# jcribeiro98/V-GAN

Measured on AMD Instinct MI355X. Metric: V-GAN train steps/sec (batch=1024, d=784), higher is better.
Workload: dtype f32; MMD contractions of `value`: split-bf16 x3 on the bf16 MFMA with fp32 accumulation (centred operand); the same step with the fp32 MFMA is timed in `fp32_mode`; 1 GPU; configs[2]: MNIST-pixels-as-features stand-in, d=784, batch=1024 (VGAN_no_kl step); global_batch=1024, features=784, latent=49, rows_per_gpu=1024, parallelism=dp1 (row-sharded Gram, replicated front), hip_graph=True, generator=collapsed, chain_association=depth, mmd_precision=bf16x3, gram_tile=64

## Files before the change

include/vgan_hip.h:

```cpp
#ifndef VGAN_HIP_H
#define VGAN_HIP_H

#include <stdint.h>

#ifdef __cplusplus
extern "C" {
#endif

#define VGAN_OK 0
#define VGAN_ERR_ARG 1
#define VGAN_ERR_HIP 2

#define VGAN_ABI_VERSION 11

typedef void* vgan_stream_t;

int vgan_abi_version(void);
const char* vgan_last_error(void);

int vgan_linear_forward(const float* x, int ldx, int x_nslabs, int64_t x_slab_stride, const float* W,
                        int ldw, const float* b, float* y, int ldy, int n, int in, int out,
                        vgan_stream_t stream);
int vgan_linear_backward_input(const float* dy, int lddy, const float* W, int ldw,
                               float* dx, int lddx, int n, int in, int out, vgan_stream_t stream);
int vgan_linear_backward_params(const float* dy, int lddy, const float* x, int ldx, int x_nslabs,
                                int64_t x_slab_stride, float* dW, int lddw, float* db, int n, int in,
                                int out, int splits, int64_t slab_stride, vgan_stream_t stream);
struct vgan_xx_job;
int vgan_linear_backward_params_xx_supported(int n, int in, int out);
int vgan_linear_backward_params_xx(const float* dy, int lddy, const float* x, int ldx, float* dW, int lddw, int n, int in,
                                   int out, const struct vgan_xx_job* xx, vgan_stream_t stream);
int64_t vgan_linear_backward_params_ksplit_ws_bytes(int in, int out, int parts);
int vgan_linear_backward_params_ksplit(const float* dy, int lddy, const float* x, int ldx, float* dW, int lddw, int n, int in,
                                       int out, int parts, void* ws, int64_t ws_bytes, vgan_stream_t stream);
enum vgan_linear_forward_path_code {
    VGAN_LINEAR_FORWARD_T64_V4 = 0,
    VGAN_LINEAR_FORWARD_T64_V1 = 1,
    VGAN_LINEAR_FORWARD_T64_V4_SLABS = 2,
    VGAN_LINEAR_FORWARD_T64_V1_SLABS = 3,
    VGAN_LINEAR_FORWARD_KS4_V4 = 4,
    VGAN_LINEAR_FORWARD_KS4_V1 = 5,
    VGAN_LINEAR_FORWARD_KS16_V4 = 6,
    VGAN_LINEAR_FORWARD_PATHS = 7
};
enum vgan_linear_backward_input_path_code {
    VGAN_LINEAR_BACKWARD_INPUT_T64_V4 = 0,
    VGAN_LINEAR_BACKWARD_INPUT_T64_V1 = 1,
    VGAN_LINEAR_BACKWARD_INPUT_KS4_V4 = 2,
    VGAN_LINEAR_BACKWARD_INPUT_KS4_V1 = 3,
    VGAN_LINEAR_BACKWARD_INPUT_PATHS = 4
};
enum vgan_linear_backward_params_path_code {
    VGAN_LINEAR_BACKWARD_PARAMS_T64_V4 = 0,
    VGAN_LINEAR_BACKWARD_PARAMS_T64_V1 = 1,
    VGAN_LINEAR_BACKWARD_PARAMS_T64_V4_SLABS = 2,
    VGAN_LINEAR_BACKWARD_PARAMS_T64_V1_SLABS = 3,
    VGAN_LINEAR_BACKWARD_PARAMS_KS4_V4 = 4,
    VGAN_LINEAR_BACKWARD_PARAMS_KS4_V1 = 5,
    VGAN_LINEAR_BACKWARD_PARAMS_KS16_V4 = 6,
    VGAN_LINEAR_BACKWARD_PARAMS_PATHS = 7
};
int vgan_linear_forward_path(const float* x, int ldx, int x_nslabs, int64_t x_slab_stride, const float* W, int ldw,
                             const float* b, const float* y, int ldy, int n, int in, int out);
int vgan_linear_backward_input_path(const float* dy, int lddy, const float* W, int ldw, const float* dx, int lddx, int n,
                                    int in, int out);
int vgan_linear_backward_params_path(const float* dy, int lddy, const float* x, int ldx, int x_nslabs, int64_t x_slab_stride,
                                     const float* dW, int lddw, const float* db, int n, int in, int out, int splits,
                                     int64_t slab_stride);
int vgan_reduce_slabs(const float* src, int64_t slab_stride, int nslabs, float* dst, int64_t count,
                      vgan_stream_t stream);

typedef struct vgan_logits_chain {
    const float* za;
    const float* At4;
    int32_t ldza, ldat, e0, pad;
} vgan_logits_chain;
int vgan_mask_project_forward(const float* logits, int ldl, const float* data, int ldd,
                              const int32_t* rows, const uint64_t* row_cursor, int row_batches,
                              int row_stride, int row_offset, float* S, float* U, float* Zx, float* Zy,
                              int ldz, float* sqx, float* sqy, int n, int d, const float* center,
                              int norm_split, const vgan_logits_chain* chain, vgan_stream_t stream);
int vgan_col_mean(const float* data, int ldd, int rows, int d, float* out, vgan_stream_t stream);
int vgan_gather_rows(const float* data, int ldd, const int32_t* rows, const uint64_t* row_cursor,
                     int row_batches, int row_stride, int row_offset, float* out, int ldo,
                     float* sq, int n, int d, vgan_stream_t stream);
int vgan_gather_rows_split(const float* data, int ldd, const int32_t* rows, const uint64_t* row_cursor,
                           int row_batches, int row_stride, int row_offset, const float* center, float* out,
                           int ldo, float* sq, int norm_split, uint16_t* Zh, uint16_t* Zl, int kp, int n, int d,
                           vgan_stream_t stream);
int vgan_mask_backward(const float* gU, int ldg, int nslabs, int64_t slab_stride, const float* S,
                       int lds, const uint64_t* colkey, float pen_weight, int row_offset,
                       float* dlogits, int ldo, int n, int d, vgan_stream_t stream);
int vgan_colmax_chunks(int n);
int vgan_colmax(const float* S, int lds, int from_softmax, int row_offset, uint64_t* part,
                uint64_t* colkey, int n, int d, vgan_stream_t stream);
int vgan_colmax_partial(const float* S, int lds, int from_softmax, int row_offset, uint64_t* part,
                        int n, int d, vgan_stream_t stream);
int vgan_mask_from_softmax(const float* S, int lds, float* U, int ldu, int n, int d, vgan_stream_t stream);
int vgan_upper_softmax_forward(const float* logits, int ldl, float* S, float* U, int n, int d,
                               vgan_stream_t stream);

#define VGAN_TILE 64
#define VGAN_TILE_INTS 8
#define VGAN_TF_SLOT_MASK 3
#define VGAN_TF_TWICE 4
#define VGAN_TF_STORE 8
#define VGAN_TF_MIRROR 16
#define VGAN_TF_NEG 32

int vgan_mmd_build_tiles(int n, int grad_mode, int rank, int world, int tile, int32_t* out, int cap);
int vgan_mmd_order_tiles(int32_t* tiles, int count, int tile);

int vgan_mmd_gram(const float* Z, int ldz, const float* sq, int n, int p, const float* bw,
                  const int32_t* tiles, int ntiles, int calibrate,
                  float* Wg, int ldw, int wrow0, float* partial, vgan_stream_t stream);
#define VGAN_RBF_MAX_KERNELS 8
int vgan_mmd_gram_general(const float* Z, int ldz, const float* sq, int n, int p, const float* bw,
                          const int32_t* tiles, int ntiles, const float* multipliers, int n_kernels,
                          float* Wg, int ldw, int wrow0, float* partial, vgan_stream_t stream);
int vgan_mmd_gram_colmax(const float* Z, int ldz, const float* sq, int n, int p, const float* bw,
                         const int32_t* tiles, int ntiles, float* Wg, int ldw, int wrow0, float* partial,
                         const float* S, int lds, int from_softmax, int row_offset, uint64_t* colpart,
                         int nrows, int d, vgan_stream_t stream);
int vgan_mmd_reduce(const float* partial, const int32_t* tiles, int ntiles, double* stats,
                    int zero_first, vgan_stream_t stream);
int vgan_mmd_set_bandwidth(const double* stats, int n, float* bw, vgan_stream_t stream);
int vgan_mmd_loss(const double* stats, const uint64_t* colkey, int n, int d, float weight,
                  float* loss, float* loss_accum, float accum_scale, uint64_t* step_counter,
                  vgan_stream_t stream);
int vgan_mmd_finalize(const float* partial, const int32_t* tiles, int ntiles, const uint64_t* colpart,
                      int chunks, uint64_t* colkey, int n, int d, float weight, double* stats,
                      float* loss, float* loss_accum, float accum_scale, uint64_t* step_counter,
                      vgan_stream_t stream);
typedef struct vgan_finalize_job {
    const float* partial;
    const int32_t* tiles;
    const uint64_t* colpart;
    uint64_t* colkey;
    double* stats;
    float* loss;
    float* loss_accum;
    uint64_t* step_counter;
    int32_t ntiles, chunks, n, d;
    float weight, accum_scale;
    int32_t mode, ntiles_main;
} vgan_finalize_job;
int vgan_mmd_backward(const float* Wg, int ldw, const float* Z, int ldz, int wrow0, int nr,
                      int ncols, int p, const float* mul, int ldmul, const float* mul_shift, float* out,
                      int ldo, int splits, int64_t slab_stride, const vgan_finalize_job* finalize,
                      vgan_stream_t stream);
int vgan_mmd_bf3_prepare(const float* Z, int ldz, int rows, int p, uint16_t* Zh, uint16_t* Zl, int kp,
                         uint16_t* ZTh, uint16_t* ZTl, int kn, vgan_stream_t stream);
int64_t vgan_mmd_gram_bf3_tail_ws_bytes(void);
int vgan_mmd_gram_bf3(const uint16_t* Zh, const uint16_t* Zl, int kp, const float* sq, int n, const float* bw,
                      const int32_t* tiles, int ntiles, int tile, uint16_t* Wh, uint16_t* Wl, int ldw,
                      int wrow0, float* partial, const float* S, int lds, int from_softmax, int row_offset,
                      uint64_t* colpart, int nrows, int d, void* tail_ws, int64_t tail_ws_bytes,
                      float* rs_part, int ldrs, vgan_stream_t stream);
int vgan_mmd_backward_bf3_tile(int nr, int p, int splits, int tile);
int vgan_mmd_backward_bf3(const uint16_t* Wh, const uint16_t* Wl, int ldw, const uint16_t* ZTh,
                          const uint16_t* ZTl, int kn, int kp, const float* Z, int ldz, int wrow0, int nr,
                          int p, const float* mul, int ldmul, const float* mul_shift, float* out, int ldo,
                          int splits, int64_t slab_stride, int tile, const vgan_finalize_job* finalize,
                          vgan_stream_t stream);
int vgan_mmd_backward_bf3_rm(const uint16_t* Wh, const uint16_t* Wl, int ldw, int kn, const uint16_t* Zh,
                             const uint16_t* Zl, int kp, int zrows, const float* Z, int ldz, int wrow0, int nr,
                             int p, const float* mul, int ldmul, const float* mul_shift, float* out, int ldo,
                             int splits, int64_t slab_stride, int tile, const vgan_finalize_job* finalize,
                             const float* rs_part, int ldrs, vgan_stream_t stream);
int vgan_mmd_backward_bf3_rm_xx(const uint16_t* Wh, const uint16_t* Wl, int ldw, int kn, const uint16_t* Zh,
                                const uint16_t* Zl, int kp, int zrows, const float* Z, int ldz, int wrow0, int nr,
                                int p, const float* mul, int ldmul, const float* mul_shift, float* out, int ldo,
                                int splits, int64_t slab_stride, const vgan_finalize_job* finalize,
                                const struct vgan_xx_job* xx, vgan_stream_t stream);
typedef struct vgan_bwd_rebuild {
    const float* data;
    const int32_t* xrow;
    const float* S;
    const float* center;
    int32_t ldd, lds;
} vgan_bwd_rebuild;
int vgan_mmd_backward_bf3_rm_rebuild(const uint16_t* Wh, const uint16_t* Wl, int ldw, int kn, const uint16_t* Zh,
                                     const uint16_t* Zl, int kp, int zrows, int nr, int p,
                                     const vgan_bwd_rebuild* rebuild, float* out, int ldo, int splits,
                                     int64_t slab_stride, const vgan_finalize_job* finalize,
                                     const struct vgan_xx_job* xx, vgan_stream_t stream);
#define VGAN_GEMM_MAX_GROUP 4
// ... 407 lines not shown
```

v-gan_amd/csrc/linear.hip:

```cpp
#include "gemm_core.hpp"
#include "mmd_xx.hpp"

namespace vgan {

constexpr int LBM = 64, LBN = 64, LBK = 32;

template <int VEC, bool XSL>
__global__ __launch_bounds__(kBlock, 2) void linear_fwd_kernel(const float* __restrict__ x, int ldx, const float* __restrict__ W,
                                                              int ldw, const float* __restrict__ b, float* __restrict__ y,
                                                              int ldy, int n, int in, int out, int x_nslabs, long x_slab_stride) {
    using G = GemmTile<LBM, LBN, LBK, KC, KC, VEC, XSL ? 1 : 0>;
    __shared__ __attribute__((aligned(16))) float lds[G::kLdsFloats];
    const int m0 = blockIdx.y * LBM, n0 = blockIdx.x * LBN;
    const int col = n0 + G::sub_col(0);
    const float bias = (b != nullptr) ? b[min(col, out - 1)] : 0.f;
    f32x16 acc[G::WM][G::WN];
    zero_acc(acc);
    G::template run<false>(x, ldx, W, ldw, m0, n0, n, out, in, lds, nullptr, acc, x_nslabs, x_slab_stride);
#pragma unroll
    for (int r = 0; r < 16; ++r) {
        const int row = m0 + G::sub_row(0, r);
        if (row < n && col < out) y[(long)row * ldy + col] = acc[0][0][r] + bias;
    }
}

template <int VEC>
__global__ __launch_bounds__(kBlock, 2) void linear_bwd_input_kernel(const float* __restrict__ dy, int lddy,
                                                                    const float* __restrict__ W, int ldw, float* __restrict__ dx,
                                                                    int lddx, int n, int in, int out) {
    using G = GemmTile<LBM, LBN, LBK, KC, MC, VEC>;
    __shared__ __attribute__((aligned(16))) float lds[G::kLdsFloats];
    const int m0 = blockIdx.y * LBM, n0 = blockIdx.x * LBN;
    f32x16 acc[G::WM][G::WN];
    zero_acc(acc);
    G::template run<false>(dy, lddy, W, ldw, m0, n0, n, in, out, lds, nullptr, acc);
    const int col = n0 + G::sub_col(0);
#pragma unroll
    for (int r = 0; r < 16; ++r) {
        const int row = m0 + G::sub_row(0, r);
        if (row < n && col < in) dx[(long)row * lddx + col] = acc[0][0][r];
    }
}

template <int VEC, bool XSL>
__global__ __launch_bounds__(kBlock, 2) void linear_bwd_params_kernel(const float* __restrict__ dy, int lddy,
                                                                     const float* __restrict__ x, int ldx, float* __restrict__ dW,
                                                                     int lddw, float* __restrict__ db, int n, int in, int out,
                                                                     int kchunk, long slab_stride, int x_nslabs, long x_slab_stride) {
    using G = GemmTile<LBM, LBN, LBK, MC, MC, VEC, XSL ? 2 : 0>;
    __shared__ __attribute__((aligned(16))) float lds[G::kLdsFloats];
    __shared__ float side[LBM];
    const int m0 = blockIdx.y * LBM, n0 = blockIdx.x * LBN;
    const int k0 = blockIdx.z * kchunk;
    const int klen = min(kchunk, n - k0);
    dy += (long)k0 * lddy;
    x += (long)k0 * ldx;
    dW += blockIdx.z * slab_stride;
    if (db != nullptr) db += blockIdx.z * slab_stride;
    n = klen;
    f32x16 acc[G::WM][G::WN];
    zero_acc(acc);
    const bool do_bias = (db != nullptr) && (blockIdx.x == 0);
    if (klen <= 0) {
        if (threadIdx.x < LBM) side[threadIdx.x] = 0.f;
        __syncthreads();
    } else if (do_bias)
        G::template run<true>(dy, lddy, x, ldx, m0, n0, out, in, n, lds, side, acc, x_nslabs, x_slab_stride);
    else
        G::template run<false>(dy, lddy, x, ldx, m0, n0, out, in, n, lds, side, acc, x_nslabs, x_slab_stride);
    const int col = n0 + G::sub_col(0);
#pragma unroll
    for (int r = 0; r < 16; ++r) {
        const int row = m0 + G::sub_row(0, r);
        if (row < out && col < in) dW[(long)row * lddw + col] = acc[0][0][r];
    }
    if (do_bias && threadIdx.x < LBM && m0 + threadIdx.x < out) db[m0 + threadIdx.x] = side[threadIdx.x];
}

constexpr int KSBK = 128;
template <int VEC, int NW>
__global__ __launch_bounds__(64 * NW, NW == 4 ? 2 : 1) void linear_fwd_ks_kernel(const float* __restrict__ x, int ldx,
                                                                               const float* __restrict__ W, int ldw,
                                                                               const float* __restrict__ b, float* __restrict__ y,
                                                                               int ldy, int n, int in, int out) {
    using G = GemmTileKS<KSBK, KC, KC, VEC, NW>;
    __shared__ __attribute__((aligned(16))) float lds[G::kLdsFloats];
    const int m0 = blockIdx.y * 32, n0 = blockIdx.x * 32;
    const int col = n0 + G::col_of();
    const float bias = (b != nullptr) ? b[min(col, out - 1)] : 0.f;
    float o[G::NR];
    G::run(x, ldx, W, ldw, m0, n0, n, out, in, lds, o);
#pragma unroll
    for (int rr = 0; rr < G::NR; ++rr) {
        const int row = m0 + G::row_of(rr);
        if (row < n && col < out) y[(long)row * ldy + col] = o[rr] + bias;
    }
}
template <int VEC>
__global__ __launch_bounds__(kBlock, 2) void linear_bwd_input_ks_kernel(const float* __restrict__ dy, int lddy,
                                                                       const float* __restrict__ W, int ldw, float* __restrict__ dx,
                                                                       int lddx, int n, int in, int out, int in_staged) {
    using G = GemmTileKS<KSBK, KC, MC, VEC>;
    __shared__ __attribute__((aligned(16))) float lds[G::kLdsFloats];
    const int m0 = blockIdx.y * 32, n0 = blockIdx.x * 32;
    float o[G::NR];
    G::run(dy, lddy, W, ldw, m0, n0, n, in_staged, out, lds, o);
    const int col = n0 + G::col_of();
#pragma unroll
    for (int rr = 0; rr < G::NR; ++rr) {
        const int row = m0 + G::row_of(rr);
        if (row < n && col < in) dx[(long)row * lddx + col] = o[rr];
    }
}
template <int VEC, int NW>
__global__ __launch_bounds__(64 * NW, NW == 4 ? 2 : 1) void linear_bwd_params_ks_kernel(const float* __restrict__ dy, int lddy,
                                                                                      const float* __restrict__ x, int ldx,
                                                                                      float* __restrict__ dW, int lddw, int n, int in,
                                                                                      int out) {
    using G = GemmTileKS<KSBK, MC, MC, VEC, NW>;
    __shared__ __attribute__((aligned(16))) float lds[G::kLdsFloats];
    const int m0 = blockIdx.y * 32, n0 = blockIdx.x * 32;
    float o[G::NR];
    G::run(dy, lddy, x, ldx, m0, n0, out, in, n, lds, o);
    const int col = n0 + G::col_of();
#pragma unroll
    for (int rr = 0; rr < G::NR; ++rr) {
        const int row = m0 + G::row_of(rr);
        if (row < out && col < in) dW[(long)row * lddw + col] = o[rr];
    }
}
__global__ __launch_bounds__(1024, 1) void linear_bwd_params_ks_split_kernel(const float* __restrict__ dy, int lddy,
                                                                            const float* __restrict__ x, int ldx, float* __restrict__ dW,
                                                                            int lddw, int n, int in, int out, int kchunk, KSplitWs ws) {
    using G = GemmTileKS<KSBK, MC, MC, 4, 16>;
    __shared__ __attribute__((aligned(16))) float lds[G::kLdsFloats];
    const int m0 = blockIdx.y * 32, n0 = blockIdx.x * 32;
    const int part = blockIdx.z, parts = gridDim.z;
    const int k0 = part * kchunk, klen = min(kchunk, n - k0);
    float o[G::NR];
    if (klen > 0) {
        G::run(dy + (long)k0 * lddy, lddy, x + (long)k0 * ldx, ldx, m0, n0, out, in, klen, lds, o);
    } else {
#pragma unroll
        for (int rr = 0; rr < G::NR; ++rr) o[rr] = 0.f;
    }
    const int tile = blockIdx.y * gridDim.x + blockIdx.x;
    if (!ksplit_finish<G::NR, G::NTH>(o, ws, tile, tile * parts * kKSplitSlabBytes, part, parts, lds)) return;
    const int col = n0 + G::col_of();
#pragma unroll
    for (int rr = 0; rr < G::NR; ++rr) {
        const int row = m0 + G::row_of(rr);
        if (row < out && col < in) dW[(long)row * lddw + col] = o[rr];
    }
}
__global__ __launch_bounds__(1024, 1) void linear_bwd_params_ks_xx_kernel(const float* __restrict__ dy, int lddy, const float* __restrict__ x,
                                                                         int ldx, float* __restrict__ dW, int lddw, int n, int in, int out,
                                                                         int gx, int ptiles, XXJob xx) {
    using G = GemmTileKS<KSBK, MC, MC, 4, 16>;
    constexpr int kBytes = G::kLdsFloats * 4 > GemmBF3<64>::kLdsBytes ? G::kLdsFloats * 4 : GemmBF3<64>::kLdsBytes;
    __shared__ __attribute__((aligned(16))) char raw[kBytes];
    __shared__ float xx_red[4];
    if ((int)blockIdx.x >= ptiles) {
        xx_tile_body(xx, blockIdx.x - ptiles, raw, xx_red);
        return;
    }
    float* lds = reinterpret_cast<float*>(raw);
    const int m0 = (blockIdx.x / gx) * 32, n0 = (blockIdx.x % gx) * 32;
    float o[G::NR];
    G::run(dy, lddy, x, ldx, m0, n0, out, in, n, lds, o);
    const int col = n0 + G::col_of();
#pragma unroll
    for (int rr = 0; rr < G::NR; ++rr) {
        const int row = m0 + G::row_of(rr);
        if (row < out && col < in) dW[(long)row * lddw + col] = o[rr];
    }
}

static inline bool use_ks(int rows, int cols, int k) {
    const long tiles64 = (long)((rows + 63) / 64) * ((cols + 63) / 64);
    return tiles64 <= 32 && k >= 128;
}

static inline bool use_ks_params(int rows, int cols, int k) {
    const long tiles64 = (long)((rows + 63) / 64) * ((cols + 63) / 64);
    return use_ks(rows, cols, k) || (tiles64 <= 512 && k >= 2048);
}

static inline dim3 grid_for(int rows, int cols) { return dim3((cols + LBN - 1) / LBN, (rows + LBM - 1) / LBM, 1); }

}

using namespace vgan;

#define VGAN_PLAN_CHECK(cond)                                                       \
    do {                                                                            \
        if (!(cond)) {                                                              \
            ::vgan::set_error("%s:%d: bad argument: %s", __FILE__, __LINE__, #cond); \
            return -VGAN_ERR_ARG;                                                   \
        }                                                                           \
    } while (0)

static int linear_forward_plan(const float* x, int ldx, int x_nslabs, int64_t x_slab_stride, const float* W, int ldw, const float* y,
                               int ldy, int n, int in, int out) {
    VGAN_PLAN_CHECK(x && W && y && n > 0 && in > 0 && out > 0 && ldx >= in && ldw >= in && ldy >= out && x_nslabs >= 1);
    const bool vec = (in % 4 == 0) && (ldx % 4 == 0) && (ldw % 4 == 0) && aligned16(x) && aligned16(W) && (x_slab_stride % 4 == 0);
    if (x_nslabs == 1 && use_ks(n, out, in))
        return vec && in >= 512 ? VGAN_LINEAR_FORWARD_KS16_V4 : vec ? VGAN_LINEAR_FORWARD_KS4_V4 : VGAN_LINEAR_FORWARD_KS4_V1;
    if (x_nslabs > 1) return vec ? VGAN_LINEAR_FORWARD_T64_V4_SLABS : VGAN_LINEAR_FORWARD_T64_V1_SLABS;
    return vec ? VGAN_LINEAR_FORWARD_T64_V4 : VGAN_LINEAR_FORWARD_T64_V1;
}

extern "C" int vgan_linear_forward_path(const float* x, int ldx, int x_nslabs, int64_t x_slab_stride, const float* W, int ldw,
                                        const float* b, const float* y, int ldy, int n, int in, int out) {
    (void)b;
    return linear_forward_plan(x, ldx, x_nslabs, x_slab_stride, W, ldw, y, ldy, n, in, out);
}

extern "C" int vgan_linear_forward(const float* x, int ldx, int x_nslabs, int64_t x_slab_stride, const float* W, int ldw,
                                   const float* b, float* y, int ldy, int n, int in, int out, vgan_stream_t stream) {
    const int path = linear_forward_plan(x, ldx, x_nslabs, x_slab_stride, W, ldw, y, ldy, n, in, out);
    if (path < 0) return VGAN_ERR_ARG;
    hipStream_t s = (hipStream_t)stream;
    const long xs = (long)x_slab_stride;
    const dim3 g((out + 31) / 32, (n + 31) / 32);
#define VGAN_FWD(V, S) hipLaunchKernelGGL((linear_fwd_kernel<V, S>), grid_for(n, out), dim3(kBlock), 0, s, x, ldx, W, ldw, b, y, ldy, n, in, out, x_nslabs, xs)
#define VGAN_FWD_KS(V, NW) hipLaunchKernelGGL((linear_fwd_ks_kernel<V, NW>), g, dim3(64 * NW), 0, s, x, ldx, W, ldw, b, y, ldy, n, in, out)
    switch (path) {
        case VGAN_LINEAR_FORWARD_KS16_V4: VGAN_FWD_KS(4, 16); break;
        case VGAN_LINEAR_FORWARD_KS4_V4: VGAN_FWD_KS(4, 4); break;
        case VGAN_LINEAR_FORWARD_KS4_V1: VGAN_FWD_KS(1, 4); break;
        case VGAN_LINEAR_FORWARD_T64_V4_SLABS: VGAN_FWD(4, true); break;
        case VGAN_LINEAR_FORWARD_T64_V1_SLABS: VGAN_FWD(1, true); break;
        case VGAN_LINEAR_FORWARD_T64_V4: VGAN_FWD(4, false); break;
        default: VGAN_FWD(1, false); break;
    }
#undef VGAN_FWD
#undef VGAN_FWD_KS
    VGAN_CHECK_LAUNCH();
    return VGAN_OK;
}

static int linear_backward_input_plan(const float* dy, int lddy, const float* W, int ldw, const float* dx, int lddx, int n, int in,
                                      int out) {
    VGAN_PLAN_CHECK(dy && W && dx && n > 0 && in > 0 && out > 0 && lddy >= out && ldw >= in && lddx >= in);
    const bool vec_but_in = (out % 4 == 0) && (lddy % 4 == 0) && (ldw % 4 == 0) && aligned16(dy) && aligned16(W);
    const bool vec = vec_but_in && (in % 4 == 0);
    if (use_ks(n, in, out)) {
        const int in4 = (in + 3) / 4 * 4;
        return vec_but_in && ldw >= in4 ? VGAN_LINEAR_BACKWARD_INPUT_KS4_V4 : VGAN_LINEAR_BACKWARD_INPUT_KS4_V1;
    }
    return vec ? VGAN_LINEAR_BACKWARD_INPUT_T64_V4 : VGAN_LINEAR_BACKWARD_INPUT_T64_V1;
}

extern "C" int vgan_linear_backward_input_path(const float* dy, int lddy, const float* W, int ldw, const float* dx, int lddx, int n,
                                               int in, int out) {
    return linear_backward_input_plan(dy, lddy, W, ldw, dx, lddx, n, in, out);
}

extern "C" int vgan_linear_backward_input(const float* dy, int lddy, const float* W, int ldw, float* dx, int lddx, int n, int in,
                                          int out, vgan_stream_t stream) {
    const int path = linear_backward_input_plan(dy, lddy, W, ldw, dx, lddx, n, in, out);
    if (path < 0) return VGAN_ERR_ARG;
    hipStream_t s = (hipStream_t)stream;
    const dim3 g((in + 31) / 32, (n + 31) / 32);
    const int in4 = (in + 3) / 4 * 4;
    switch (path) {
        case VGAN_LINEAR_BACKWARD_INPUT_KS4_V4:
            hipLaunchKernelGGL(linear_bwd_input_ks_kernel<4>, g, dim3(kBlock), 0, s, dy, lddy, W, ldw, dx, lddx, n, in, out, in4);
            break;
        case VGAN_LINEAR_BACKWARD_INPUT_KS4_V1:
            hipLaunchKernelGGL(linear_bwd_input_ks_kernel<1>, g, dim3(kBlock), 0, s, dy, lddy, W, ldw, dx, lddx, n, in, out, in);
            break;
        case VGAN_LINEAR_BACKWARD_INPUT_T64_V4:
            hipLaunchKernelGGL(linear_bwd_input_kernel<4>, grid_for(n, in), dim3(kBlock), 0, s, dy, lddy, W, ldw, dx, lddx, n, in, out);
            break;
        default:
            hipLaunchKernelGGL(linear_bwd_input_kernel<1>, grid_for(n, in), dim3(kBlock), 0, s, dy, lddy, W, ldw, dx, lddx, n, in, out);
            break;
    }
    VGAN_CHECK_LAUNCH();
    return VGAN_OK;
}

static int linear_backward_params_plan(const float* dy, int lddy, const float* x, int ldx, int x_nslabs, int64_t x_slab_stride,
                                       const float* dW, int lddw, const float* db, int n, int in, int out, int splits,
                                       int64_t slab_stride) {
    VGAN_PLAN_CHECK(dy && x && dW && n > 0 && in > 0 && out > 0 && lddy >= out && ldx >= in && lddw >= in && x_nslabs >= 1);
    VGAN_PLAN_CHECK(splits >= 1 && splits <= 64 && (splits == 1 || slab_stride > 0));
    const bool vec = (out % 4 == 0) && (lddy % 4 == 0) && (in % 4 == 0) && (ldx % 4 == 0) && aligned16(dy) && aligned16(x) &&
                     (x_slab_stride % 4 == 0);
    if (splits == 1 && x_nslabs == 1 && db == nullptr && use_ks_params(out, in, n))
        return vec && n >= 256 ? VGAN_LINEAR_BACKWARD_PARAMS_KS16_V4 : vec ? VGAN_LINEAR_BACKWARD_PARAMS_KS4_V4 : VGAN_LINEAR_BACKWARD_PARAMS_KS4_V1;
    if (x_nslabs > 1) return vec ? VGAN_LINEAR_BACKWARD_PARAMS_T64_V4_SLABS : VGAN_LINEAR_BACKWARD_PARAMS_T64_V1_SLABS;
    return vec ? VGAN_LINEAR_BACKWARD_PARAMS_T64_V4 : VGAN_LINEAR_BACKWARD_PARAMS_T64_V1;
}

extern "C" int vgan_linear_backward_params_path(const float* dy, int lddy, const float* x, int ldx, int x_nslabs, int64_t x_slab_stride,
                                                const float* dW, int lddw, const float* db, int n, int in, int out, int splits,
                                                int64_t slab_stride) {
    return linear_backward_params_plan(dy, lddy, x, ldx, x_nslabs, x_slab_stride, dW, lddw, db, n, in, out, splits, slab_stride);
}

extern "C" int vgan_linear_backward_params(const float* dy, int lddy, const float* x, int ldx, int x_nslabs, int64_t x_slab_stride,
                                           float* dW, int lddw, float* db, int n, int in, int out, int splits, int64_t slab_stride,
                                           vgan_stream_t stream) {
    const int path = linear_backward_params_plan(dy, lddy, x, ldx, x_nslabs, x_slab_stride, dW, lddw, db, n, in, out, splits, slab_stride);
    if (path < 0) return VGAN_ERR_ARG;
    hipStream_t s = (hipStream_t)stream;
    int kchunk = (n + splits - 1) / splits;
    kchunk = (kchunk + 3) / 4 * 4;
    dim3 grid = grid_for(out, in);
    grid.z = splits;
    const long xs = (long)x_slab_stride;
    const dim3 g((in + 31) / 32, (out + 31) / 32);
#define VGAN_BWP(V, S) hipLaunchKernelGGL((linear_bwd_params_kernel<V, S>), grid, dim3(kBlock), 0, s, dy, lddy, x, ldx, dW, lddw, db, n, in, out, kchunk, (long)slab_stride, x_nslabs, xs)
#define VGAN_BWP_KS(V, NW) hipLaunchKernelGGL((linear_bwd_params_ks_kernel<V, NW>), g, dim3(64 * NW), 0, s, dy, lddy, x, ldx, dW, lddw, n, in, out)
    switch (path) {
        case VGAN_LINEAR_BACKWARD_PARAMS_KS16_V4: VGAN_BWP_KS(4, 16); break;
        case VGAN_LINEAR_BACKWARD_PARAMS_KS4_V4: VGAN_BWP_KS(4, 4); break;
        case VGAN_LINEAR_BACKWARD_PARAMS_KS4_V1: VGAN_BWP_KS(1, 4); break;
        case VGAN_LINEAR_BACKWARD_PARAMS_T64_V4_SLABS: VGAN_BWP(4, true); break;
        case VGAN_LINEAR_BACKWARD_PARAMS_T64_V1_SLABS: VGAN_BWP(1, true); break;
        case VGAN_LINEAR_BACKWARD_PARAMS_T64_V4: VGAN_BWP(4, false); break;
        default: VGAN_BWP(1, false); break;
    }
#undef VGAN_BWP
#undef VGAN_BWP_KS
    VGAN_CHECK_LAUNCH();
    return VGAN_OK;
}

extern "C" int64_t vgan_linear_backward_params_ksplit_ws_bytes(int in, int out, int parts) {
    if (in <= 0 || out <= 0 || parts <= 1 || parts > kKSplitMaxParts) return 0;
    const long tiles = (long)((in + 31) / 32) * ((out + 31) / 32);
    return ksplit_ticket_bytes(tiles) + tiles * parts * kKSplitSlabBytes;
}

extern "C" int vgan_linear_backward_params_ksplit(const float* dy, int lddy, const float* x, int ldx, float* dW, int lddw, int n, int in,
                                                  int out, int parts, void* ws, int64_t ws_bytes, vgan_stream_t stream) {
    VGAN_CHECK_ARG(parts >= 1 && parts <= kKSplitMaxParts);
    if (parts == 1) return vgan_linear_backward_params(dy, lddy, x, ldx, 1, 0, dW, lddw, nullptr, n, in, out, 1, 0, stream);
    VGAN_CHECK_ARG(dy && x && dW && n > 0 && in > 0 && out > 0 && lddy >= out && ldx >= in && lddw >= in);
    VGAN_CHECK_ARG((out % 4 == 0) && (lddy % 4 == 0) && (in % 4 == 0) && (ldx % 4 == 0) && aligned16(dy) && aligned16(x));
    const int64_t need = vgan_linear_backward_params_ksplit_ws_bytes(in, out, parts);
    VGAN_CHECK_ARG(ws != nullptr && aligned16(ws) && ws_bytes >= need && need < (1ll << 31));
    const int gx = (in + 31) / 32, gy = (out + 31) / 32;
    VGAN_CHECK_ARG(gy <= 65535);
    const long tb = ksplit_ticket_bytes((long)gx * gy);
    const KSplitWs k{reinterpret_cast<float*>(static_cast<char*>(ws) + tb), static_cast<int*>(ws), (int)(need - tb)};
    hipLaunchKernelGGL(linear_bwd_params_ks_split_kernel, dim3(gx, gy, parts), dim3(1024), 0, (hipStream_t)stream, dy, lddy, x, ldx, dW, lddw, n,
                       in, out, ksplit_kchunk(n, parts, KSBK), k);
    VGAN_CHECK_LAUNCH();
    return VGAN_OK;
}

extern "C" int vgan_linear_backward_params_xx_supported(int n, int in, int out) {
    return (n >= 256 && in > 0 && out > 0 && in % 4 == 0 && out % 4 == 0 && use_ks(out, in, n)) ? 1 : 0;
}

extern "C" int vgan_linear_backward_params_xx(const float* dy, int lddy, const float* x, int ldx, float* dW, int lddw, int n, int in,
                                              int out, const vgan_xx_job* xxjob, vgan_stream_t stream) {
    VGAN_CHECK_ARG(dy && x && dW && xxjob && n > 0 && in > 0 && out > 0 && lddy >= out && ldx >= in && lddw >= in);
    const vgan_xx_job& j = *xxjob;
    VGAN_CHECK_ARG(j.Dh && j.Dl && j.dsq && j.tiles && j.bw && j.partial && j.ntiles > 0 && j.ldd % 64 == 0 && aligned16(j.Dh) && aligned16(j.Dl) &&
                   (reinterpret_cast<uintptr_t>(j.partial) & 15) == 0);
    VGAN_CHECK_ARG((out % 4 == 0) && (lddy % 4 == 0) && (in % 4 == 0) && (ldx % 4 == 0) && aligned16(dy) && aligned16(x) && n >= 256 &&
                   use_ks(out, in, n));
    const int gx = (in + 31) / 32, gy = (out + 31) / 32;
    const XXJob xx{j.Dh, j.Dl, j.dsq, nullptr, nullptr, reinterpret_cast<const TileDesc*>(j.tiles), j.bw, j.partial, j.ldd, 1, 0, j.ntiles, 0};
    hipLaunchKernelGGL(linear_bwd_params_ks_xx_kernel, dim3(gx * gy + j.ntiles), dim3(1024), 0, (hipStream_t)stream, dy, lddy, x, ldx, dW, lddw, n,
                       in, out, gx, gx * gy, xx);
    VGAN_CHECK_LAUNCH();
    return VGAN_OK;
}
```

v-gan_amd/csrc/rows.hip:

```cpp
#include "mmd_xx.hpp"
#include "vgan_common.hpp"

namespace vgan {

constexpr int kRowsPerBlock = kBlock / kWave;

struct RowSel {
    const int* rows;
    const unsigned long long* cursor;
    int row_batches, row_stride, row_offset;
    __device__ __forceinline__ long operator()(int i) const {
        if (rows == nullptr) return (long)(row_offset + i);
        const long b = cursor ? (long)(cursor[0] % (unsigned long long)row_batches) : 0l;
        return (long)rows[b * row_stride + row_offset + i];
    }
};


template <bool PROJECT>
__global__ __launch_bounds__(kBlock) void mask_forward_kernel(const float* __restrict__ logits, int ldl, const float* __restrict__ data,
                                                             int ldd, RowSel rows, float* __restrict__ S,
                                                             float* __restrict__ U, float* __restrict__ Zx, float* __restrict__ Zy,
                                                             int ldz, float* __restrict__ sqx, float* __restrict__ sqy, int n, int d,
                                                             const float* __restrict__ center, int norm_split) {
    const int lane = threadIdx.x & 63;
    const int i = blockIdx.x * kRowsPerBlock + (threadIdx.x >> 6);
    if (i >= n) return;
    const float* x = logits + (long)i * ldl;
    float m = -INFINITY;
    for (int j = lane; j < d; j += 64) m = fmaxf(m, x[j]);
    m = wave_max(m);
    float sum = 0.f;
    for (int j = lane; j < d; j += 64) sum += expf(x[j] - m);
    sum = wave_sum(sum);
    const float tau = 1.0f / (float)d;
    const float* xr = nullptr;
    float *zx = nullptr, *zy = nullptr;
    if constexpr (PROJECT) {
        const long src = rows(i);
        xr = data + src * ldd;
        zx = Zx ? Zx + (long)i * ldz : nullptr;
        zy = Zy + (long)i * ldz;
    }
    float nx = 0.f, ny = 0.f;
    for (int j = lane; j < d; j += 64) {
        const float s = expf(x[j] - m) / sum;
        const float u = s < tau ? s : 1.0f;
        S[(long)i * d + j] = s;
        if (U) U[(long)i * d + j] = u;
        if constexpr (PROJECT) {
            const float c = center ? center[j] : 0.f;
            const float xv = xr[j] - c;
            const float yv = project_centred(u, xr[j], c);
            if (zx) zx[j] = xv;
            zy[j] = yv;
            const float xn = norm_split ? split_value(xv) : xv, yn = norm_split ? split_value(yv) : yv;
            nx = fmaf(xn, xn, nx);
            ny = fmaf(yn, yn, ny);
        }
    }
    if constexpr (PROJECT) {
        nx = wave_sum(nx);
        ny = wave_sum(ny);
        if (lane == 0) {
            if (sqx) sqx[i] = nx;
            sqy[i] = ny;
        }
    }
}


struct LogitsChain {
    const float* za;
    const float* At4;
    int ldza, ldat, e0;
};
constexpr int kChainK = 16;
__host__ __device__ constexpr int chain_pitch(int d) { return ((d + 3) / 4) * 4 + 4; }

template <int NT>
__device__ __forceinline__ void chain_logits(const LogitsChain& ch, float* __restrict__ lds_at, int d, int row, bool row_ok, float4 (&v)[NT]) {
    const int lane = threadIdx.x & 63, nq = d >> 2, pitch = chain_pitch(d);
#pragma unroll
    for (int t = 0; t < NT; ++t) v[t] = make_float4(0.f, 0.f, 0.f, 0.f);
    const float* zr = ch.za + (long)(row_ok ? row : 0) * ch.ldza;
    for (int kc = 0; kc < ch.e0; kc += kChainK) {
        __syncthreads();
        for (int idx = threadIdx.x; idx < d * (kChainK / 4); idx += blockDim.x) {
            const int col = idx / (kChainK / 4), kq = idx % (kChainK / 4), k = kc + 4 * kq;
            const float4 a = k < ch.e0 ? *reinterpret_cast<const float4*>(ch.At4 + (long)col * ch.ldat + k) : make_float4(0.f, 0.f, 0.f, 0.f);
            lds_at[(4 * kq + 0) * pitch + col] = a.x;
            lds_at[(4 * kq + 1) * pitch + col] = a.y;
            lds_at[(4 * kq + 2) * pitch + col] = a.z;
            lds_at[(4 * kq + 3) * pitch + col] = a.w;
        }
        __syncthreads();
        const int kw = min(kChainK, ch.e0 - kc);
        for (int k = 0; k < kw; ++k) {
            const float z = zr[kc + k];
#pragma unroll
            for (int t = 0; t < NT; ++t) {
                const int q = min(lane + 64 * t, nq - 1);
                const float4 a = *reinterpret_cast<const float4*>(lds_at + k * pitch + 4 * q);
                v[t].x = fmaf(z, a.x, v[t].x);
                v[t].y = fmaf(z, a.y, v[t].y);
                v[t].z = fmaf(z, a.z, v[t].z);
                v[t].w = fmaf(z, a.w, v[t].w);
            }
        }
    }
#pragma unroll
    for (int t = 0; t < NT; ++t)
        if (lane + 64 * t >= nq) v[t] = make_float4(-INFINITY, -INFINITY, -INFINITY, -INFINITY);
}

template <int NT, bool CHAIN>
__global__ __launch_bounds__(kBlock) void mask_forward_vec_kernel(const float* __restrict__ logits, int ldl, const float* __restrict__ data,
                                                                 int ldd, RowSel rows, float* __restrict__ S, float* __restrict__ U,
                                                                 float* __restrict__ Zx, float* __restrict__ Zy, int ldz,
                                                                 float* __restrict__ sqx, float* __restrict__ sqy, int n, int d,
                                                                 const float* __restrict__ center, int norm_split, LogitsChain ch) {
    extern __shared__ __attribute__((aligned(16))) float chain_lds[];
    const int lane = threadIdx.x & 63;
    const int i = blockIdx.x * kRowsPerBlock + (threadIdx.x >> 6);
    const int nq = d >> 2;
    float4 v[NT], xv[NT], cv[NT];
    if constexpr (CHAIN) chain_logits<NT>(ch, chain_lds, d, i, i < n, v);
    if (i >= n) return;
    const float4* x4 = reinterpret_cast<const float4*>(logits + (long)i * ldl);
    const float4* xr4 = reinterpret_cast<const float4*>(data + rows(i) * ldd);
#pragma unroll
    for (int t = 0; t < NT; ++t) {
        const int q = lane + 64 * t;
        const bool ok = q < nq;
        if constexpr (!CHAIN) v[t] = ok ? x4[min(q, nq - 1)] : make_float4(-INFINITY, -INFINITY, -INFINITY, -INFINITY);
        xv[t] = xr4[min(q, nq - 1)];
        cv[t] = center ? reinterpret_cast<const float4*>(center)[min(q, nq - 1)] : make_float4(0.f, 0.f, 0.f, 0.f);
    }
    float m = -INFINITY;
#pragma unroll
    for (int t = 0; t < NT; ++t) m = fmaxf(m, fmaxf(fmaxf(v[t].x, v[t].y), fmaxf(v[t].z, v[t].w)));
    m = wave_max(m);
    float sum = 0.f;
#pragma unroll
    for (int t = 0; t < NT; ++t) {
        v[t].x = expf(v[t].x - m); v[t].y = expf(v[t].y - m); v[t].z = expf(v[t].z - m); v[t].w = expf(v[t].w - m);
        sum += (v[t].x + v[t].y) + (v[t].z + v[t].w);
    }
    sum = wave_sum(sum);
    const float tau = 1.0f / (float)d;
    float nx = 0.f, ny = 0.f;
#pragma unroll
    for (int t = 0; t < NT; ++t) {
        const int q = lane + 64 * t;
        if (q < nq) {
            float4 s4 = make_float4(v[t].x / sum, v[t].y / sum, v[t].z / sum, v[t].w / sum);
            float4 u4 = make_float4(s4.x < tau ? s4.x : 1.f, s4.y < tau ? s4.y : 1.f, s4.z < tau ? s4.z : 1.f, s4.w < tau ? s4.w : 1.f);
            const float4 x4c = make_float4(xv[t].x - cv[t].x, xv[t].y - cv[t].y, xv[t].z - cv[t].z, xv[t].w - cv[t].w);
            const float4 y4 = make_float4(project_centred(u4.x, xv[t].x, cv[t].x), project_centred(u4.y, xv[t].y, cv[t].y), project_centred(u4.z, xv[t].z, cv[t].z),
                                              project_centred(u4.w, xv[t].w, cv[t].w));
            reinterpret_cast<float4*>(S + (long)i * d)[q] = s4;
            if (U) reinterpret_cast<float4*>(U + (long)i * d)[q] = u4;
            if (Zx) reinterpret_cast<float4*>(Zx + (long)i * ldz)[q] = x4c;
            reinterpret_cast<float4*>(Zy + (long)i * ldz)[q] = y4;
            const float xs[4] = {x4c.x, x4c.y, x4c.z, x4c.w}, ys[4] = {y4.x, y4.y, y4.z, y4.w};
            float xn[4], yn[4];
#pragma unroll
            for (int e = 0; e < 4; ++e) {
                xn[e] = norm_split ? split_value(xs[e]) : xs[e];
                yn[e] = norm_split ? split_value(ys[e]) : ys[e];
            }
            nx += (xn[0] * xn[0] + xn[1] * xn[1]) + (xn[2] * xn[2] + xn[3] * xn[3]);
            ny += (yn[0] * yn[0] + yn[1] * yn[1]) + (yn[2] * yn[2] + yn[3] * yn[3]);
        }
    }
    nx = wave_sum(nx);
    ny = wave_sum(ny);
    if (lane == 0) {
        if (sqx) sqx[i] = nx;
        sqy[i] = ny;
    }
}

__device__ __forceinline__ float norm_term4(const float (&z)[4]) { return (z[0] * z[0] + z[1] * z[1]) + (z[2] * z[2] + z[3] * z[3]); }

template <int NT, bool XX, bool CHAIN>
__global__ __launch_bounds__(512) void mask_forward_bf3_kernel(const float* __restrict__ logits, int ldl, const float* __restrict__ data,
                                                                 int ldd, RowSel rows, float* __restrict__ S, float* __restrict__ Z,
                                                                 int ldz, float* __restrict__ sq, unsigned short* __restrict__ Zh,
                                                                 unsigned short* __restrict__ Zl, int kp, unsigned short* __restrict__ ZTh,
                                                                 unsigned short* __restrict__ ZTl, int kn, int n, int d,
                                                                 const float* __restrict__ center, int write_x, int mask_blocks,
                                                                 XXJob xx, LogitsChain ch, int write_z, int* __restrict__ xrow) {
    constexpr int R = 8;
    if constexpr (XX) {
        __shared__ __attribute__((aligned(16))) char xx_lds[GemmBF3<64>::kLdsBytes];
        __shared__ float xx_red[4];
        if ((int)blockIdx.x >= mask_blocks) {
            xx_tile_body(xx, blockIdx.x - mask_blocks, xx_lds, xx_red);
            return;
        }
    }
    extern __shared__ __attribute__((aligned(16))) unsigned short tile[];
    const int ldt = 4 * (d >> 2) + 8;
    const int lane = threadIdx.x & 63, wave = threadIdx.x >> 6;
    const int nq = d >> 2;
    const int groups = n / R, C = (groups + 7) / 8;
    const int grp = (blockIdx.x % 8) * C + blockIdx.x / 8;
    if (grp >= groups) return;
    const int i0 = grp * R;
    const float tau = 1.0f / (float)d;
    {
        const int lr = wave, i = i0 + lr;
        float4 v[NT];
        if constexpr (CHAIN) chain_logits<NT>(ch, reinterpret_cast<float*>(tile), d, i, i < n, v);
        if (i < n) {
            const float4* x4 = reinterpret_cast<const float4*>(logits + (long)i * ldl);
            const long src = rows(i);
            const float4* xr4 = reinterpret_cast<const float4*>(data + src * ldd);
            if (xrow != nullptr && lane == 0) xrow[i] = (int)src;
            float4 xv[NT], cv[NT];
#pragma unroll
            for (int t = 0; t < NT; ++t) {
                const int q = lane + 64 * t;
                const bool ok = q < nq;
                if constexpr (!CHAIN) v[t] = ok ? x4[min(q, nq - 1)] : make_float4(-INFINITY, -INFINITY, -INFINITY, -INFINITY);
                xv[t] = xr4[min(q, nq - 1)];
                cv[t] = center ? reinterpret_cast<const float4*>(center)[min(q, nq - 1)] : make_float4(0.f, 0.f, 0.f, 0.f);
            }
            float m = -INFINITY;
#pragma unroll
            for (int t = 0; t < NT; ++t) m = fmaxf(m, fmaxf(fmaxf(v[t].x, v[t].y), fmaxf(v[t].z, v[t].w)));
            m = wave_max(m);
            float sum = 0.f;
#pragma unroll
            for (int t = 0; t < NT; ++t) {
                v[t].x = expf(v[t].x - m); v[t].y = expf(v[t].y - m); v[t].z = expf(v[t].z - m); v[t].w = expf(v[t].w - m);
                sum += (v[t].x + v[t].y) + (v[t].z + v[t].w);
            }
            sum = wave_sum(sum);
            float nx = 0.f, ny = 0.f;
#pragma unroll
            for (int t = 0; t < NT; ++t) {
                const int q = lane + 64 * t;
                if (q < nq) {
                    const float4 s4 = make_float4(v[t].x / sum, v[t].y / sum, v[t].z / sum, v[t].w / sum);
                    const float4 u4 = make_float4(upper_mask(s4.x, tau), upper_mask(s4.y, tau), upper_mask(s4.z, tau), upper_mask(s4.w, tau));
                    const float4 x4c = make_float4(centred_x(xv[t].x, cv[t].x), centred_x(xv[t].y, cv[t].y), centred_x(xv[t].z, cv[t].z),
                                                   centred_x(xv[t].w, cv[t].w));
                    const float4 y4 = make_float4(project_centred(u4.x, xv[t].x, cv[t].x), project_centred(u4.y, xv[t].y, cv[t].y), project_centred(u4.z, xv[t].z, cv[t].z),
                                              project_centred(u4.w, xv[t].w, cv[t].w));
                    reinterpret_cast<float4*>(S + (long)i * d)[q] = s4;
                    if (write_z) {
                        if (write_x) reinterpret_cast<float4*>(Z + (long)i * ldz)[q] = x4c;
                        reinterpret_cast<float4*>(Z + (long)(n + i) * ldz)[q] = y4;
                    }
                    const float xs[4] = {x4c.x, x4c.y, x4c.z, x4c.w}, ys[4] = {y4.x, y4.y, y4.z, y4.w};
                    unsigned short h[2][4], l[2][4];
                    float xn[4], yn[4];
#pragma unroll
                    for (int e = 0; e < 4; ++e) {
                        split_bf16(xs[e], h[0][e], l[0][e]);
                        split_bf16(ys[e], h[1][e], l[1][e]);
                        xn[e] = bf16_val(h[0][e]) + bf16_val(l[0][e]);
                        yn[e] = bf16_val(h[1][e]) + bf16_val(l[1][e]);
                    }
                    nx += norm_term4(xn);
                    ny += norm_term4(yn);
#pragma unroll
                    for (int im = 0; im < 2; ++im) {
                        const uint2 ph = make_uint2((unsigned)h[im][0] | ((unsigned)h[im][1] << 16), (unsigned)h[im][2] | ((unsigned)h[im][3] << 16));
                        const uint2 pl = make_uint2((unsigned)l[im][0] | ((unsigned)l[im][1] << 16), (unsigned)l[im][2] | ((unsigned)l[im][3] << 16));
                        const long grow = (long)(im * n + i) * kp + 4 * q;
                        if (im == 1 || write_x) {
                            *reinterpret_cast<uint2*>(Zh + grow) = ph;
                            *reinterpret_cast<uint2*>(Zl + grow) = pl;
                        }
                        if (ZTh != nullptr) {
                            *reinterpret_cast<uint2*>(tile + ((2 * im) * R + lr) * ldt + 4 * q) = ph;
                            *reinterpret_cast<uint2*>(tile + ((2 * im + 1) * R + lr) * ldt + 4 * q) = pl;
                        }
                    }
                }
            }
            nx = wave_sum(nx);
            ny = wave_sum(ny);
            if (lane == 0) {
                if (write_x) sq[i] = nx;
                sq[n + i] = ny;
            }
        } else if (ZTh != nullptr) {
            for (int c = lane; c < ldt; c += 64)
#pragma unroll
                for (int im = 0; im < 4; ++im) tile[(im * R + lr) * ldt + c] = 0;
        }
    }
    if (ZTh == nullptr) return;
    __syncthreads();
    const int npairs = d >> 1;
    for (int item = threadIdx.x; item < 4 * npairs; item += 512) {
        const int im = item / npairs, j = 2 * (item - im * npairs);
        unsigned w0[4], w1[4];
#pragma unroll
        for (int e = 0; e < 4; ++e) {
            const unsigned a = *reinterpret_cast<const unsigned*>(tile + (im * R + 2 * e) * ldt + j);
            const unsigned c = *reinterpret_cast<const unsigned*>(tile + (im * R + 2 * e + 1) * ldt + j);
            w0[e] = (a & 0xFFFFu) | (c << 16);
            w1[e] = (a >> 16) | (c & 0xFFFF0000u);
        }
        unsigned short* dst = ((im & 1) ? ZTl : ZTh) + (long)j * kn + (im >> 1) * n + i0;
        *reinterpret_cast<uint4*>(dst) = make_uint4(w0[0], w0[1], w0[2], w0[3]);
        *reinterpret_cast<uint4*>(dst + kn) = make_uint4(w1[0], w1[1], w1[2], w1[3]);
    }
}

#ifndef VGAN_MASK_FWD_SPLIT
#define VGAN_MASK_FWD_SPLIT 1
#endif
template <int NT>
__global__ __launch_bounds__(64 * NT) void mask_forward_bf3_split_kernel(const float* __restrict__ logits, int ldl, const float* __restrict__ data,
                                                                         int ldd, RowSel rows, float* __restrict__ S, float* __restrict__ Z,
                                                                         int ldz, float* __restrict__ sq, unsigned short* __restrict__ Zh,
                                                                         unsigned short* __restrict__ Zl, int kp, int n, int d,
                                                                         const float* __restrict__ center, int write_x, int write_z,
                                                                         int* __restrict__ xrow) {
    __shared__ float red_m[NT][64], red_nx[NT][64], red_s[NT][64], red_ny[NT][64];
    const int lane = threadIdx.x & 63, wave = threadIdx.x >> 6;
    const int nq = d >> 2;
    const int i = blockIdx.x;
    const int q = lane + 64 * wave, qc = min(q, nq - 1);
    const bool ok = q < nq;
    const float tau = 1.0f / (float)d;
    float4 v = reinterpret_cast<const float4*>(logits + (long)i * ldl)[qc];
    const float4 cv = center ? reinterpret_cast<const float4*>(center)[qc] : make_float4(0.f, 0.f, 0.f, 0.f);
    const long src = rows(i);
    const float4 xv = reinterpret_cast<const float4*>(data + src * ldd)[qc];
    if (xrow != nullptr && threadIdx.x == 0) xrow[i] = (int)src;
    if (!ok) v = make_float4(-INFINITY, -INFINITY, -INFINITY, -INFINITY);
    const float4 x4c = make_float4(centred_x(xv.x, cv.x), centred_x(xv.y, cv.y), centred_x(xv.z, cv.z), centred_x(xv.w, cv.w));
    const float xs[4] = {x4c.x, x4c.y, x4c.z, x4c.w};
    unsigned short h[4], l[4];
    float xn[4];
#pragma unroll
    for (int e = 0; e < 4; ++e) {
        split_bf16(xs[e], h[e], l[e]);
        xn[e] = bf16_val(h[e]) + bf16_val(l[e]);
    }
    if (ok && write_x) {
        if (write_z) reinterpret_cast<float4*>(Z + (long)i * ldz)[q] = x4c;
        const long grow = (long)i * kp + 4 * q;
        *reinterpret_cast<uint2*>(Zh + grow) = make_uint2((unsigned)h[0] | ((unsigned)h[1] << 16), (unsigned)h[2] | ((unsigned)h[3] << 16));
        *reinterpret_cast<uint2*>(Zl + grow) = make_uint2((unsigned)l[0] | ((unsigned)l[1] << 16), (unsigned)l[2] | ((unsigned)l[3] << 16));
    }
    red_m[wave][lane] = fmaxf(fmaxf(v.x, v.y), fmaxf(v.z, v.w));
    red_nx[wave][lane] = ok ? norm_term4(xn) : 0.f;
    __syncthreads();
    float m = -INFINITY;
#pragma unroll
    for (int t = 0; t < NT; ++t) m = fmaxf(m, red_m[t][lane]);
    m = wave_max(m);
    v.x = expf(v.x - m); v.y = expf(v.y - m); v.z = expf(v.z - m); v.w = expf(v.w - m);
    red_s[wave][lane] = (v.x + v.y) + (v.z + v.w);
    __syncthreads();
    float sum = 0.f;
#pragma unroll
    for (int t = 0; t < NT; ++t) sum += red_s[t][lane];
    sum = wave_sum(sum);
    const float4 s4 = make_float4(v.x / sum, v.y / sum, v.z / sum, v.w / sum);
    const float4 u4 = make_float4(upper_mask(s4.x, tau), upper_mask(s4.y, tau), upper_mask(s4.z, tau), upper_mask(s4.w, tau));
    const float4 y4 = make_float4(project_centred(u4.x, xv.x, cv.x), project_centred(u4.y, xv.y, cv.y), project_centred(u4.z, xv.z, cv.z),
                                  project_centred(u4.w, xv.w, cv.w));
    const float ys[4] = {y4.x, y4.y, y4.z, y4.w};
    float yn[4];
#pragma unroll
    for (int e = 0; e < 4; ++e) {
        split_bf16(ys[e], h[e], l[e]);
        yn[e] = bf16_val(h[e]) + bf16_val(l[e]);
    }
    if (ok) {
        reinterpret_cast<float4*>(S + (long)i * d)[q] = s4;
        if (write_z) reinterpret_cast<float4*>(Z + (long)(n + i) * ldz)[q] = y4;
        const long grow = (long)(n + i) * kp + 4 * q;
        *reinterpret_cast<uint2*>(Zh + grow) = make_uint2((unsigned)h[0] | ((unsigned)h[1] << 16), (unsigned)h[2] | ((unsigned)h[3] << 16));
        *reinterpret_cast<uint2*>(Zl + grow) = make_uint2((unsigned)l[0] | ((unsigned)l[1] << 16), (unsigned)l[2] | ((unsigned)l[3] << 16));
    }
    red_ny[wave][lane] = ok ? norm_term4(yn) : 0.f;
    __syncthreads();
    if (wave == 0) {
        float nx = 0.f, ny = 0.f;
#pragma unroll
        for (int t = 0; t < NT; ++t) {
            nx += red_nx[t][lane];
            ny += red_ny[t][lane];
        }
        nx = wave_sum(nx);
        ny = wave_sum(ny);
        if (lane == 0) {
            if (write_x) sq[i] = nx;
            sq[n + i] = ny;
        }
    }
}

template <int NT>
__global__ __launch_bounds__(kBlock) void mask_backward_vec_kernel(const float* __restrict__ gU, int ldg, const float* __restrict__ S,
                                                                  int lds, const unsigned long long* __restrict__ colkey,
                                                                  float pen_weight, int row_offset, float* __restrict__ dlogits,
                                                                  int ldo, int n, int d, int nslabs, long slab_stride) {
    const int lane = threadIdx.x & 63;
    const int i = blockIdx.x * kRowsPerBlock + (threadIdx.x >> 6);
    if (i >= n) return;
    const int nq = d >> 2;
    const float tau = 1.0f / (float)d;
    const float pg = -pen_weight / (float)d;
    const unsigned me = (unsigned)(row_offset + i);
    float4 sv[NT], gs[NT];
    float dot = 0.f;
#pragma unroll
    for (int t = 0; t < NT; ++t) {
        const int q = min(lane + 64 * t, nq - 1);
        const bool ok = lane + 64 * t < nq;
        sv[t] = reinterpret_cast<const float4*>(S + (long)i * lds)[q];
        float4 g = reinterpret_cast<const float4*>(gU + (long)i * ldg)[q];
        for (int sl = 1; sl < nslabs; ++sl) {
            const float4 b = reinterpret_cast<const float4*>(gU + sl * slab_stride + (long)i * ldg)[q];
            g.x += b.x; g.y += b.y; g.z += b.z; g.w += b.w;
        }
        if (colkey != nullptr) {
            const ulonglong2 k0 = reinterpret_cast<const ulonglong2*>(colkey)[2 * q], k1 = reinterpret_cast<const ulonglong2*>(colkey)[2 * q + 1];
            if (colkey_row(k0.x) == me) g.x += pg;
            if (colkey_row(k0.y) == me) g.y += pg;
            if (colkey_row(k1.x) == me) g.z += pg;
            if (colkey_row(k1.y) == me) g.w += pg;
        }
        gs[t] = make_float4(ok && sv[t].x < tau ? g.x : 0.f, ok && sv[t].y < tau ? g.y : 0.f, ok && sv[t].z < tau ? g.z : 0.f,
                            ok && sv[t].w < tau ? g.w : 0.f);
        dot += (gs[t].x * sv[t].x + gs[t].y * sv[t].y) + (gs[t].z * sv[t].z + gs[t].w * sv[t].w);
    }
    dot = wave_sum(dot);
#pragma unroll
    for (int t = 0; t < NT; ++t) {
        const int q = lane + 64 * t;
        if (q < nq)
            reinterpret_cast<float4*>(dlogits + (long)i * ldo)[q] =
                make_float4(sv[t].x * (gs[t].x - dot), sv[t].y * (gs[t].y - dot), sv[t].z * (gs[t].z - dot), sv[t].w * (gs[t].w - dot));
    }
}

__global__ __launch_bounds__(kBlock) void mask_backward_kernel(const float* __restrict__ gU, int ldg, const float* __restrict__ S,
                                                              int lds, const unsigned long long* __restrict__ colkey,
                                                              float pen_weight, int row_offset, float* __restrict__ dlogits,
                                                              int ldo, int n, int d, int nslabs, long slab_stride) {
    const int lane = threadIdx.x & 63;
    const int i = blockIdx.x * kRowsPerBlock + (threadIdx.x >> 6);
    if (i >= n) return;
    const float tau = 1.0f / (float)d;
    const float pg = -pen_weight / (float)d;
    const float* g = gU + (long)i * ldg;
    const float* s = S + (long)i * lds;
    const unsigned me = (unsigned)(row_offset + i);
    auto grad = [&](int j) {
        float gv = g[j];
        for (int q = 1; q < nslabs; ++q) gv += g[q * slab_stride + j];
        if (colkey != nullptr && colkey_row(colkey[j]) == me) gv += pg;
        return gv;
    };
    float dot = 0.f;
    for (int j = lane; j < d; j += 64) {
        const float sv = s[j];
        dot = fmaf(sv < tau ? grad(j) : 0.f, sv, dot);
    }
    dot = wave_sum(dot);
    for (int j = lane; j < d; j += 64) {
        const float sv = s[j];
        dlogits[(long)i * ldo + j] = sv * ((sv < tau ? grad(j) : 0.f) - dot);
    }
}

__global__ __launch_bounds__(kBlock) void colmax_partial_kernel(const float* __restrict__ S, int lds, int row_offset,
                                                               unsigned long long* __restrict__ part, int n, int d, int from_softmax) {
    colmax_partial_body<4>(S, lds, row_offset, part, n, d, from_softmax, blockIdx.x, blockIdx.y);
}
__global__ void colmax_final_kernel(const unsigned long long* __restrict__ part, int chunks, unsigned long long* __restrict__ colkey,
                                    int d) {
    const int j = blockIdx.x * blockDim.x + threadIdx.x;
    if (j >= d) return;
    unsigned long long b = 0ull;
    for (int c = 0; c < chunks; ++c) {
        const unsigned long long k = part[(long)c * d + j];
        b = k > b ? k : b;
    }
    colkey[j] = b;
}

__global__ __launch_bounds__(kBlock) void gather_rows_kernel(const float* __restrict__ data, int ldd, RowSel rows,
                                                            float* __restrict__ out, int ldo, float* __restrict__ sq, int n, int d) {
    const int lane = threadIdx.x & 63;
    const int i = blockIdx.x * kRowsPerBlock + (threadIdx.x >> 6);
    if (i >= n) return;
    const float* x = data + rows(i) * ldd;
    float* o = out + (long)i * ldo;
    float nx = 0.f;
    for (int j = lane; j < d; j += 64) {
        const float v = x[j];
        o[j] = v;
        nx = fmaf(v, v, nx);
    }
    nx = wave_sum(nx);
    if (lane == 0 && sq) sq[i] = nx;
}

__global__ __launch_bounds__(kBlock) void gather_center_split_kernel(const float* __restrict__ data, int ldd, RowSel rows,
                                                                    const float* __restrict__ center, float* __restrict__ out, int ldo,
                                                                    float* __restrict__ sq, int norm_split,
                                                                    unsigned short* __restrict__ Zh, unsigned short* __restrict__ Zl,
                                                                    int kp, int n, int d) {
    const int lane = threadIdx.x & 63;
    const int i = blockIdx.x * kRowsPerBlock + (threadIdx.x >> 6);
    if (i >= n) return;
    const float* x = data + rows(i) * ldd;
    float nx = 0.f;
    for (int j = lane; j < d; j += 64) {
        const float v = x[j] - (center ? center[j] : 0.f);
        if (out) out[(long)i * ldo + j] = v;
        unsigned short hi, lo;
        split_bf16(v, hi, lo);
        if (Zh) {
            Zh[(long)i * kp + j] = hi;
            Zl[(long)i * kp + j] = lo;
        }
        const float vn = norm_split ? bf16_val(hi) + bf16_val(lo) : v;
        nx = fmaf(vn, vn, nx);
    }
    nx = wave_sum(nx);
    if (lane == 0 && sq) sq[i] = nx;
}

__global__ __launch_bounds__(kBlock) void gather_center_split_vec_kernel(const float* __restrict__ data, int ldd, RowSel rows,
                                                                        const float* __restrict__ center, float* __restrict__ out, int ldo,
                                                                        float* __restrict__ sq, int norm_split,
                                                                        unsigned short* __restrict__ Zh, unsigned short* __restrict__ Zl,
                                                                        int kp, int n, int d) {
    const int lane = threadIdx.x & 63;
    const int i = blockIdx.x * kRowsPerBlock + (threadIdx.x >> 6);
    if (i >= n) return;
    const float4* x4 = reinterpret_cast<const float4*>(data + rows(i) * ldd);
    const int nq = d >> 2;
    float nx = 0.f;
    for (int q = lane; q < nq; q += 64) {
        float4 v = x4[q];
        if (center) {
            const float4 c = reinterpret_cast<const float4*>(center)[q];
            v.x -= c.x; v.y -= c.y; v.z -= c.z; v.w -= c.w;
        }
        if (out) reinterpret_cast<float4*>(out + (long)i * ldo)[q] = v;
        const float vs[4] = {v.x, v.y, v.z, v.w};
        unsigned short h[4], l[4];
        float vn[4];
#pragma unroll
        for (int e = 0; e < 4; ++e) {
            split_bf16(vs[e], h[e], l[e]);
            vn[e] = norm_split ? bf16_val(h[e]) + bf16_val(l[e]) : vs[e];
        }
        if (Zh) {
            *reinterpret_cast<uint2*>(Zh + (long)i * kp + 4 * q) = make_uint2((unsigned)h[0] | ((unsigned)h[1] << 16), (unsigned)h[2] | ((unsigned)h[3] << 16));
            *reinterpret_cast<uint2*>(Zl + (long)i * kp + 4 * q) = make_uint2((unsigned)l[0] | ((unsigned)l[1] << 16), (unsigned)l[2] | ((unsigned)l[3] << 16));
        }
        nx += (vn[0] * vn[0] + vn[1] * vn[1]) + (vn[2] * vn[2] + vn[3] * vn[3]);
    }
    nx = wave_sum(nx);
    if (lane == 0 && sq) sq[i] = nx;
}

__global__ void mask_from_softmax_kernel(const float* __restrict__ S, int lds, float* __restrict__ U, int ldu, int n, int d) {
    const long idx = (long)blockIdx.x * blockDim.x + threadIdx.x;
    if (idx >= (long)n * d) return;
    const int i = (int)(idx / d), j = (int)(idx % d);
    const float sv = S[(long)i * lds + j];
    U[(long)i * ldu + j] = sv < 1.0f / (float)d ? sv : 1.0f;
}

}

using namespace vgan;

extern "C" int vgan_mask_project_forward(const float* logits, int ldl, const float* data, int ldd, const int32_t* rows,
                                         const uint64_t* row_cursor, int row_batches, int row_stride, int row_offset, float* S,
                                         float* U, float* Zx, float* Zy, int ldz, float* sqx, float* sqy, int n, int d,
                                         const float* center, int norm_split, const vgan_logits_chain* chain, vgan_stream_t stream) {
    VGAN_CHECK_ARG((logits || chain) && data && S && Zy && sqy && n > 0 && d > 0 && (logits == nullptr || ldl >= d) && ldd >= d && ldz >= d);
    VGAN_CHECK_ARG(row_batches >= 1 && row_stride >= 0 && row_offset >= 0);
    LogitsChain ch{};
    if (chain != nullptr) {
        VGAN_CHECK_ARG(chain->za && chain->At4 && chain->e0 > 0 && chain->e0 % 4 == 0 && chain->ldza >= chain->e0 && chain->ldat >= chain->e0 &&
                       chain->ldat % 4 == 0 && aligned16(chain->At4));
        ch = LogitsChain{chain->za, chain->At4, chain->ldza, chain->ldat, chain->e0};
        if (logits == nullptr) { logits = chain->za; ldl = 4; }
    }
    const RowSel sel{rows, reinterpret_cast<const unsigned long long*>(row_cursor), row_batches, row_stride, row_offset};
    const dim3 grid((n + kRowsPerBlock - 1) / kRowsPerBlock), block(kBlock);
    hipStream_t st = (hipStream_t)stream;
    const bool vec = (d % 4 == 0) && (d <= (chain != nullptr ? 1024 : 4096)) && (ldl % 4 == 0) && (ldd % 4 == 0) && (ldz % 4 == 0) && aligned16(logits) &&
                     aligned16(data) && aligned16(S) && (U == nullptr || aligned16(U)) && (Zx == nullptr || aligned16(Zx)) && aligned16(Zy) && (center == nullptr || aligned16(center));
    if (vec) {
        const int nt = (d / 4 + 63) / 64;
        const size_t chain_bytes = (size_t)kChainK * chain_pitch(d) * sizeof(float);
#define VGAN_LAUNCH_FWD(NT)                                                                                                               \
    do {                                                                                                                                  \
        if (chain != nullptr) {                                                                                                           \
            if (chain_bytes > 64 * 1024)                                                                                                  \
                (void)hipFuncSetAttribute(reinterpret_cast<const void*>(&mask_forward_vec_kernel<NT, true>),                                \
                                          hipFuncAttributeMaxDynamicSharedMemorySize, (int)chain_bytes);                                  \
            hipLaunchKernelGGL((mask_forward_vec_kernel<NT, true>), grid, block, chain_bytes, st, logits, ldl, data, ldd, sel, S, U, Zx, Zy, ldz, \
                               sqx, sqy, n, d, center, norm_split, ch);                                                                   \
        } else                                                                                                                            \
            hipLaunchKernelGGL((mask_forward_vec_kernel<NT, false>), grid, block, 0, st, logits, ldl, data, ldd, sel, S, U, Zx, Zy, ldz, sqx, \
                               sqy, n, d, center, norm_split, ch);                                                                        \
    } while (0)
        if (nt == 1) VGAN_LAUNCH_FWD(1); else if (nt == 2) VGAN_LAUNCH_FWD(2); else if (nt == 3) VGAN_LAUNCH_FWD(3); else if (nt == 4) VGAN_LAUNCH_FWD(4);
        else if (nt <= 8)
            hipLaunchKernelGGL((mask_forward_vec_kernel<8, false>), grid, block, 0, st, logits, ldl, data, ldd, sel, S, U, Zx, Zy, ldz, sqx, sqy, n, d,
                               center, norm_split, ch);
        else
            hipLaunchKernelGGL((mask_forward_vec_kernel<16, false>), grid, block, 0, st, logits, ldl, data, ldd, sel, S, U, Zx, Zy, ldz, sqx, sqy, n, d,
                               center, norm_split, ch);
#undef VGAN_LAUNCH_FWD
    } else {
        VGAN_CHECK_ARG(chain == nullptr);
        hipLaunchKernelGGL(mask_forward_kernel<true>, grid, block, 0, st, logits, ldl, data, ldd, sel, S, U, Zx, Zy, ldz, sqx, sqy, n, d, center,
                           norm_split);
    }
    VGAN_CHECK_LAUNCH();
    return VGAN_OK;
}

extern "C" int vgan_mask_project_forward_bf3(const float* logits, int ldl, const float* data, int ldd, const int32_t* rows,
                                             const uint64_t* row_cursor, int row_batches, int row_stride, float* S, float* Z, int ldz,
                                             float* sq, uint16_t* Zh, uint16_t* Zl, int kp, uint16_t* ZTh, uint16_t* ZTl, int kn,
                                             int n, int d, const float* center, int write_x, const vgan_xx_job* xxjob,
                                             const vgan_logits_chain* chain, vgan_stream_t stream) {
    VGAN_CHECK_ARG(Z != nullptr);
    return vgan_mask_project_forward_bf3_ex(logits, ldl, data, ldd, rows, row_cursor, row_batches, row_stride, S, Z, ldz, sq, Zh, Zl, kp, ZTh,
                                            ZTl, kn, n, d, center, write_x, xxjob, chain, 1, nullptr, stream);
}

extern "C" int vgan_mask_project_forward_bf3_ex(const float* logits, int ldl, const float* data, int ldd, const int32_t* rows,
                                                const uint64_t* row_cursor, int row_batches, int row_stride, float* S, float* Z, int ldz,
                                                float* sq, uint16_t* Zh, uint16_t* Zl, int kp, uint16_t* ZTh, uint16_t* ZTl, int kn,
                                                int n, int d, const float* center, int write_x, const vgan_xx_job* xxjob,
                                                const vgan_logits_chain* chain, int write_z, int32_t* xrow, vgan_stream_t stream) {
    VGAN_CHECK_ARG((logits || chain) && data && S && (Z || !write_z) && sq && Zh && Zl && n > 0 && d > 0 && (logits == nullptr || ldl >= d) &&
                   ldd >= d && (!write_z || ldz >= d));
    LogitsChain ch{};
    if (chain != nullptr) {
        VGAN_CHECK_ARG(ZTh == nullptr && chain->za && chain->At4 && chain->e0 > 0 && chain->e0 % 4 == 0 && chain->ldza >= chain->e0 &&
                       chain->ldat >= chain->e0 && chain->ldat % 4 == 0 && aligned16(chain->At4));
        ch = LogitsChain{chain->za, chain->At4, chain->ldza, chain->ldat, chain->e0};
        if (logits == nullptr) { logits = chain->za; ldl = 4; }
    }
    VGAN_CHECK_ARG((ZTh == nullptr) == (ZTl == nullptr));
    VGAN_CHECK_ARG(row_batches >= 1 && row_stride >= 0 && kp >= d && kp % 64 == 0 && (ZTh == nullptr || (kn >= 2 * n && kn % 64 == 0)));
    VGAN_CHECK_ARG(write_x || ZTh == nullptr);
    VGAN_CHECK_ARG(d % 4 == 0 && d <= 1024 && n % 8 == 0 && ldl % 4 == 0 && ldd % 4 == 0 && (!write_z || ldz % 4 == 0));
    VGAN_CHECK_ARG(aligned16(logits) && aligned16(data) && aligned16(S) && (!write_z || aligned16(Z)) && aligned16(Zh) && aligned16(Zl) &&
                   (ZTh == nullptr || (aligned16(ZTh) && aligned16(ZTl))) && (center == nullptr || aligned16(center)));
    const RowSel sel{rows, reinterpret_cast<const unsigned long long*>(row_cursor), row_batches, row_stride, 0};
    const int mask_blocks = 8 * ((n / 8 + 7) / 8);
    XXJob xx{};
    int xx_blocks = 0;
    if (xxjob != nullptr) {
        const vgan_xx_job& j = *xxjob;
        VGAN_CHECK_ARG(ZTh == nullptr && j.Dh && j.Dl && j.dsq && j.tiles && j.bw && j.partial && j.ntiles > 0 && j.ldd >= d && j.ldd % 64 == 0);
        VGAN_CHECK_ARG(aligned16(j.Dh) && aligned16(j.Dl) && (reinterpret_cast<uintptr_t>(j.partial) & 15) == 0);
        xx = XXJob{j.Dh, j.Dl, j.dsq, rows, reinterpret_cast<const unsigned long long*>(row_cursor), reinterpret_cast<const TileDesc*>(j.tiles),
                   j.bw, j.partial, j.ldd, row_batches, row_stride, j.ntiles, n};
        xx_blocks = j.ntiles;
    }
    const dim3 grid(mask_blocks + xx_blocks), block(512);
    const size_t shmem = ZTh != nullptr ? (size_t)4 * 8 * (d + 8) * sizeof(unsigned short)
                                        : (chain != nullptr ? (size_t)kChainK * chain_pitch(d) * sizeof(float) : 0);
    hipStream_t st = (hipStream_t)stream;
    const int nt = (d / 4 + 63) / 64;
#if VGAN_MASK_FWD_SPLIT
    if (ZTh == nullptr && xxjob == nullptr && chain == nullptr && nt >= 2) {
#define VGAN_LAUNCH_SPLIT(NT)                                                                                                       \
    hipLaunchKernelGGL((mask_forward_bf3_split_kernel<NT>), dim3(n), dim3(64 * NT), 0, st, logits, ldl, data, ldd, sel, S, Z, ldz, sq, \
                       Zh, Zl, kp, n, d, center, write_x, write_z, xrow)
        if (nt == 2) VGAN_LAUNCH_SPLIT(2); else if (nt == 3) VGAN_LAUNCH_SPLIT(3); else VGAN_LAUNCH_SPLIT(4);
#undef VGAN_LAUNCH_SPLIT
        VGAN_CHECK_LAUNCH();
        return VGAN_OK;
    }
#endif
#define VGAN_LAUNCH_K3(NT, XXF, CHF)                                                                                                \
    do {                                                                                                                            \
        if (shmem > 64 * 1024)                                                                                                      \
            (void)hipFuncSetAttribute(reinterpret_cast<const void*>(&mask_forward_bf3_kernel<NT, XXF, CHF>),                          \
                                      hipFuncAttributeMaxDynamicSharedMemorySize, (int)shmem);                                      \
        hipLaunchKernelGGL((mask_forward_bf3_kernel<NT, XXF, CHF>), grid, block, shmem, st, logits, ldl, data, ldd, sel, S, Z, ldz, sq, \
                           Zh, Zl, kp, ZTh, ZTl, kn, n, d, center, write_x, mask_blocks, xx, ch, write_z, xrow);                     \
    } while (0)
#define VGAN_LAUNCH_FWD3(NT)                                                                                                        \
    do {                                                                                                                            \
        if (xx_blocks > 0 && chain != nullptr) VGAN_LAUNCH_K3(NT, true, true);                                                      \
        else if (xx_blocks > 0) VGAN_LAUNCH_K3(NT, true, false);                                                                    \
        else if (chain != nullptr) VGAN_LAUNCH_K3(NT, false, true);                                                                 \
        else VGAN_LAUNCH_K3(NT, false, false);                                                                                      \
    } while (0)
    if (nt == 1) VGAN_LAUNCH_FWD3(1); else if (nt == 2) VGAN_LAUNCH_FWD3(2); else if (nt == 3) VGAN_LAUNCH_FWD3(3); else VGAN_LAUNCH_FWD3(4);
#undef VGAN_LAUNCH_FWD3
#undef VGAN_LAUNCH_K3
    VGAN_CHECK_LAUNCH();
    return VGAN_OK;
}

extern "C" int vgan_upper_softmax_forward(const float* logits, int ldl, float* S, float* U, int n, int d, vgan_stream_t stream) {
    VGAN_CHECK_ARG(logits && S && n > 0 && d > 0 && ldl >= d);
    hipLaunchKernelGGL(mask_forward_kernel<false>, dim3((n + kRowsPerBlock - 1) / kRowsPerBlock), dim3(kBlock), 0,
                       (hipStream_t)stream, logits, ldl, nullptr, 0, RowSel{nullptr, nullptr, 1, 0, 0}, S, U, nullptr, nullptr, 0, nullptr, nullptr, n, d, nullptr, 0);
    VGAN_CHECK_LAUNCH();
    return VGAN_OK;
// ... 86 lines not shown
```

v-gan_amd/lib.py:

```python
import ctypes
import os

_HERE = os.path.dirname(os.path.abspath(__file__))
LIB_PATH = os.path.join(_HERE, "libvgan_hip.so")

_p = ctypes.c_void_p
_i = ctypes.c_int
_f = ctypes.c_float
_i64 = ctypes.c_int64
_d = ctypes.c_double
_u64 = ctypes.c_uint64

class FinalizeJob(ctypes.Structure):
    _fields_ = [("partial", _p), ("tiles", _p), ("colpart", _p), ("colkey", _p), ("stats", _p), ("loss", _p), ("loss_accum", _p),
                ("step_counter", _p), ("ntiles", ctypes.c_int32), ("chunks", ctypes.c_int32), ("n", ctypes.c_int32),
                ("d", ctypes.c_int32), ("weight", _f), ("accum_scale", _f), ("mode", ctypes.c_int32), ("ntiles_main", ctypes.c_int32)]


class GemmProblem(ctypes.Structure):
    _fields_ = [("a", _p), ("b", _p), ("c", _p), ("kind", ctypes.c_int32), ("m", ctypes.c_int32), ("n", ctypes.c_int32),
                ("k", ctypes.c_int32), ("lda", ctypes.c_int32), ("ldb", ctypes.c_int32), ("ldc", ctypes.c_int32), ("splitk", ctypes.c_int32),
                ("d", _p), ("scratch", _p), ("ldd", ctypes.c_int32), ("k2", ctypes.c_int32)]


class LogitsChain(ctypes.Structure):
    _fields_ = [("za", _p), ("At4", _p), ("ldza", ctypes.c_int32), ("ldat", ctypes.c_int32), ("e0", ctypes.c_int32), ("pad", ctypes.c_int32)]


class XXJob(ctypes.Structure):
    _fields_ = [("Dh", _p), ("Dl", _p), ("dsq", _p), ("tiles", _p), ("bw", _p), ("partial", _p), ("ldd", ctypes.c_int32),
                ("ntiles", ctypes.c_int32)]


class BwdRebuild(ctypes.Structure):
    _fields_ = [("data", _p), ("xrow", _p), ("S", _p), ("center", _p), ("ldd", ctypes.c_int32), ("lds", ctypes.c_int32)]


class AdadeltaLayer(ctypes.Structure):
    _fields_ = [("w_packed", _p), ("off_w", _i64), ("off_b", _i64), ("ldp", ctypes.c_int32), ("out", ctypes.c_int32),
                ("inp", ctypes.c_int32), ("pad", ctypes.c_int32)]


class GroupedExtras(ctypes.Structure):
    _fields_ = [("copy_src", _p), ("copy_dst", _p), ("copy_count", _i64), ("adadelta", ctypes.c_int32), ("pad", ctypes.c_int32),
                ("p", _p), ("sq_avg", _p), ("acc_delta", _p), ("lr", _f), ("rho", _f), ("eps", _f), ("weight_decay", _f),
                ("grad_scale", _f), ("ld_extra", ctypes.c_int32), ("layer", AdadeltaLayer * 5), ("g_extra", _p), ("next_noise", _p),
                ("noise_rows", ctypes.c_int32), ("noise_cols", ctypes.c_int32), ("noise_ld", ctypes.c_int32),
                ("noise_ones_col", ctypes.c_int32), ("seed", _u64), ("step_counter", _p), ("fold", _p)]


GEMM_NN, GEMM_NT, GEMM_TN, GEMM_NT_NT = 0, 1, 2, 3
GEMM_MAX_GROUP = 4

LINEAR_FORWARD_PATHS = ("T64_V4", "T64_V1", "T64_V4_SLABS", "T64_V1_SLABS", "KS4_V4", "KS4_V1", "KS16_V4")
LINEAR_BACKWARD_INPUT_PATHS = ("T64_V4", "T64_V1", "KS4_V4", "KS4_V1")
LINEAR_BACKWARD_PARAMS_PATHS = ("T64_V4", "T64_V1", "T64_V4_SLABS", "T64_V1_SLABS", "KS4_V4", "KS4_V1", "KS16_V4")
GEMM_GROUPED_PATHS = ("T256_V4", "T256_V4_EPI", "T256_V1", "T256_V1_EPI", "KS16", "KS16_SPLIT")
GEMM_ENGINES = ("T64", "KS4", "KS16")

SIGNATURES = {
    "vgan_abi_version": (_i, []),
    "vgan_last_error": (ctypes.c_char_p, []),
    "vgan_linear_forward": (_i, [_p, _i, _i, _i64, _p, _i, _p, _p, _i, _i, _i, _i, _p]),
    "vgan_linear_backward_input": (_i, [_p, _i, _p, _i, _p, _i, _i, _i, _i, _p]),
    "vgan_linear_backward_params": (_i, [_p, _i, _p, _i, _i, _i64, _p, _i, _p, _i, _i, _i, _i, _i64, _p]),
    "vgan_linear_backward_params_ksplit_ws_bytes": (_i64, [_i, _i, _i]),
    "vgan_linear_backward_params_ksplit": (_i, [_p, _i, _p, _i, _p, _i, _i, _i, _i, _i, _p, _i64, _p]),
    "vgan_linear_backward_params_xx_supported": (_i, [_i, _i, _i]),
    "vgan_linear_backward_params_xx": (_i, [_p, _i, _p, _i, _p, _i, _i, _i, _i, _p, _p]),
    "vgan_linear_forward_path": (_i, [_p, _i, _i, _i64, _p, _i, _p, _p, _i, _i, _i, _i]),
    "vgan_linear_backward_input_path": (_i, [_p, _i, _p, _i, _p, _i, _i, _i, _i]),
    "vgan_linear_backward_params_path": (_i, [_p, _i, _p, _i, _i, _i64, _p, _i, _p, _i, _i, _i, _i, _i64]),
    "vgan_reduce_slabs": (_i, [_p, _i64, _i, _p, _i64, _p]),
    "vgan_mask_project_forward": (_i, [_p, _i, _p, _i, _p, _p, _i, _i, _i, _p, _p, _p, _p, _i, _p, _p, _i, _i, _p, _i, _p, _p]),
    "vgan_col_mean": (_i, [_p, _i, _i, _i, _p, _p]),
    "vgan_gather_rows": (_i, [_p, _i, _p, _p, _i, _i, _i, _p, _i, _p, _i, _i, _p]),
    "vgan_gather_rows_split": (_i, [_p, _i, _p, _p, _i, _i, _i, _p, _p, _i, _p, _i, _p, _p, _i, _i, _i, _p]),
    "vgan_mask_backward": (_i, [_p, _i, _i, _i64, _p, _i, _p, _f, _i, _p, _i, _i, _i, _p]),
    "vgan_colmax_partial": (_i, [_p, _i, _i, _i, _p, _i, _i, _p]),
    "vgan_mmd_finalize": (_i, [_p, _p, _i, _p, _i, _p, _i, _i, _f, _p, _p, _p, _f, _p, _p]),
    "vgan_colmax_chunks": (_i, [_i]),
    "vgan_colmax": (_i, [_p, _i, _i, _i, _p, _p, _i, _i, _p]),
    "vgan_mask_from_softmax": (_i, [_p, _i, _p, _i, _i, _i, _p]),
    "vgan_upper_softmax_forward": (_i, [_p, _i, _p, _p, _i, _i, _p]),
    "vgan_mmd_build_tiles": (_i, [_i, _i, _i, _i, _i, _p, _i]),
    "vgan_mmd_order_tiles": (_i, [_p, _i, _i]),
    "vgan_mmd_gram": (_i, [_p, _i, _p, _i, _i, _p, _p, _i, _i, _p, _i, _i, _p, _p]),
    "vgan_mmd_gram_general": (_i, [_p, _i, _p, _i, _i, _p, _p, _i, _p, _i, _p, _i, _i, _p, _p]),
    "vgan_mmd_gram_colmax": (_i, [_p, _i, _p, _i, _i, _p, _p, _i, _p, _i, _i, _p, _p, _i, _i, _i, _p, _i, _i, _p]),
    "vgan_mmd_reduce": (_i, [_p, _p, _i, _p, _i, _p]),
    "vgan_mmd_set_bandwidth": (_i, [_p, _i, _p, _p]),
    "vgan_mmd_loss": (_i, [_p, _p, _i, _i, _f, _p, _p, _f, _p, _p]),
    "vgan_mmd_backward": (_i, [_p, _i, _p, _i, _i, _i, _i, _i, _p, _i, _p, _p, _i, _i, _i64, _p, _p]),
    "vgan_mmd_bf3_prepare": (_i, [_p, _i, _i, _i, _p, _p, _i, _p, _p, _i, _p]),
    "vgan_mmd_gram_bf3": (_i, [_p, _p, _i, _p, _i, _p, _p, _i, _i, _p, _p, _i, _i, _p, _p, _i, _i, _i, _p, _i, _i, _p, _i64, _p, _i, _p]),
    "vgan_mmd_gram_bf3_tail_ws_bytes": (_i64, []),
    "vgan_mmd_backward_bf3": (_i, [_p, _p, _i, _p, _p, _i, _i, _p, _i, _i, _i, _i, _p, _i, _p, _p, _i, _i, _i64, _i, _p, _p]),
    "vgan_mmd_backward_bf3_tile": (_i, [_i, _i, _i, _i]),
    "vgan_mmd_backward_bf3_rm": (_i, [_p, _p, _i, _i, _p, _p, _i, _i, _p, _i, _i, _i, _i, _p, _i, _p, _p, _i, _i, _i64, _i, _p, _p, _i, _p]),
    "vgan_mmd_backward_bf3_rm_xx": (_i, [_p, _p, _i, _i, _p, _p, _i, _i, _p, _i, _i, _i, _i, _p, _i, _p, _p, _i, _i, _i64, _p, _p, _p]),
    "vgan_mmd_backward_bf3_rm_rebuild": (_i, [_p, _p, _i, _i, _p, _p, _i, _i, _i, _i, _p, _p, _i, _i, _i64, _p, _p, _p]),
    "vgan_row_sqnorm": (_i, [_p, _i, _p, _i, _i, _p]),
    "vgan_adadelta_step": (_i, [_p, _p, _i, _i64, _p, _p, _i64, _f, _f, _f, _f, _f, _p]),
    "vgan_noise_normal": (_i, [_p, _i, _i, _i, _i, _u64, _p, _u64, _p]),
    "vgan_homogeneous_pack": (_i, [_p, _i, _i, _i, _p]),
    "vgan_adadelta_step_packed": (_i, [_p, _p, _p, _p, _p, _p, _i64, _f, _f, _f, _f, _f, _p, _i, _i, _i, _i, _u64, _p, _p]),
    "vgan_gemm_grouped": (_i, [_p, _i, _p]),
    "vgan_gemm_grouped_ex": (_i, [_p, _i, _p, _p]),
    "vgan_gemm_grouped_path": (_i, [_p, _i, _p, _p, _p]),
    "vgan_gemm_grouped_ksplit_ws_bytes": (_i64, [_p, _i, _p]),
    "vgan_gemm_grouped_ksplit": (_i, [_p, _i, _p, _p, _p, _i64, _p]),
    "vgan_mask_project_forward_bf3": (_i, [_p, _i, _p, _i, _p, _p, _i, _i, _p, _p, _i, _p, _p, _p, _i, _p, _p, _i, _i, _i, _p, _i, _p, _p, _p]),
    "vgan_mask_project_forward_bf3_ex": (_i, [_p, _i, _p, _i, _p, _p, _i, _i, _p, _p, _i, _p, _p, _p, _i, _p, _p, _i, _i, _i, _p, _i, _p, _p, _i, _p,
                                              _p]),
    "vgan_mse_grad": (_i, [_p, _i, _p, _i, _i, _i, _f, _p, _p, _i, _p]),
    "vgan_sum_f64": (_i, [_p, _i, ctypes.c_double, _p, _i, _p]),
    "vgan_rbf_kernel_matrix": (_i, [_p, _i, _i, _i, _p, _f, _p, _i, _p]),
    "vgan_rbf_multi_kernel_matrix": (_i, [_p, _i, _i, _i, _p, _p, _p, _i, _p, _i, _p, _i, _p]),
    "vgan_rows_dot": (_i, [_p, _i, _p, _i, _p, _i, _i, _p]),
    "vgan_shuffle_epoch": (_i, [_p, _i64, _i64, _u64, _u64, _p]),
    "vgan_shuffle_index": (_i64, [_i64, _i64, _u64, _u64]),
    "vgan_mask_unique": (_i, [_p, _i, _i, _i, _p, _p, _p, _p, _p]),
    "vgan_dp_unique_id": (_i, [_p]),
    "vgan_dp_comm_create": (_i, [_p, _i, _p, _i]),
    "vgan_dp_allreduce_sum": (_i, [_p, _p, _i64, _p]),
    "vgan_dp_allgather": (_i, [_p, _p, _i64, _p]),
    "vgan_dp_comm_destroy": (_i, [_p]),
    "vgan_mse": (_i, [_p, _i, _p, _i, _i, _i, _f, _p, _i, _p]),
    "vgan_outlier_pack": (_i, [_p, _i, _i, _i, _p, _p, _p, _p, _i, _i, _p, _p, _p]),
    "vgan_outlier_knn": (_i, [_p, _p, _i, _p, _p, _i, _p, _p, _i, _i, _i, _i, _i, _i, _p, _p, _p, _p]),
    "vgan_outlier_refine": (_i, [_p, _i, _i, _p, _i, _i, _i, _p, _p, _i, _i, _p, _i, _p, _p, _p, _p]),
    "vgan_outlier_score": (_i, [_p, _p, _i, _i, _i, _i, _p, _p, _i, _p, _p, _i, _p, _p]),
    "vgan_outlier_kde": (_i, [_p, _p, _i, _p, _p, _i, _p, _p, _i, _i, _p, _i, _i, _i, _p, _p, _p, _p, _i, _p]),
    "vgan_outlier_combine": (_i, [_p, _i, _i, _i, _p, _p, _p]),
    "vgan_outlier_abod": (_i, [_p, _i, _i, _p, _i, _i, _i, _p, _p, _i, _i, _p, _i, _p, _p, _i, _p]),
    "vgan_outlier_abod_floor": (_i, [_p, _i, _i, _i, _i, _p, _p, _p]),
    "vgan_outlier_cof_chain": (_i, [_p, _i, _i, _p, _i, _i, _i, _p, _p, _i, _i, _p, _i, _i, _p, _p]),
    "vgan_outlier_cof_score": (_i, [_p, _i, _p, _i, _p, _i, _i, _p, _p, _i, _p]),
    "vgan_outlier_cof_ceiling": (_i, [_p, _i, _i, _i, _i, _p, _p, _p]),
    "vgan_outlier_score_stats_ws_bytes": (_i64, [_i, _i, _i]),
    "vgan_outlier_score_stats": (_i, [_p, _i, _i, _i, _i, _p, _p, _p, _i64, _p]),
    "vgan_outlier_combine_normalized": (_i, [_p, _i, _i, _i, _p, _p, _p, _i, _p, _p]),
    "vgan_cluster_lloyd_ws_bytes": (_i64, [_i, _i, _i, _i]),
    "vgan_cluster_image": (_i, [_p, _i, _p, _p, _p, _i, _i, _p, _p, _p, _p]),
    "vgan_cluster_lloyd": (_i, [_p, _p, _p, _i, _i, _i, _p, _p, _p, _i, _i, _i, _i, _i, _i, _p, _p, _p, _p, _p, _p, _p, _p, _p,
                                _p, _i64, _i, _p]),
    "vgan_cluster_final": (_i, [_p, _i, _i, _i, _p, _p, _i, _i, _p, _p, _p, _i, _p, _p, _p, _p, _p, _i, _p]),
    "vgan_ecod_sort_columns": (_i, [_p, _i, _i, _i, _p, _i64, _p]),
    "vgan_ecod_skew_sign": (_i, [_p, _i64, _i, _i, _p, _p]),
    "vgan_ecod_tail_counts": (_i, [_p, _i, _i, _i, _p, _i64, _i, _p, _p, _p]),
    "vgan_ecod_scores": (_i, [_p, _p, _i, _i, _p, _i, _i, _i, _p, _i, _i, _p, _p, _i64, _p]),
    "vgan_hist_column_range": (_i, [_p, _i, _i, _i, _p, _p]),
    "vgan_hist_edges": (_i, [_p, _i64, _i, _p, _p]),
    "vgan_hist_column_counts": (_i, [_p, _i, _i, _i, _p, _i, _p, _p]),
    "vgan_hbos_scores": (_i, [_p, _i, _i, _i, _p, _i, _p, _p, _p, _i, _i, _p, _p, _i64, _p]),
    "vgan_hist_reset": (_i, [_p, _i64, _p, _i64, _p]),
    "vgan_loda_range": (_i, [_p, _i, _p, _p, _i, _i, _i, _p, _p, _p, _i, _p, _p]),
    "vgan_loda_counts": (_i, [_p, _i, _p, _p, _i, _i, _i, _p, _p, _p, _i, _p, _i, _p, _p]),
    "vgan_loda_scores": (_i, [_p, _i, _p, _p, _i, _i, _i, _p, _p, _p, _i, _p, _i, _p, _p, _i64, _p]),
    "vgan_iforest_build": (_i, [_p, _i, _i64, _i, _p, _p, _i, _i, _i, _i, _i, _i, _u64, _p, _p]),
    "vgan_iforest_path_sums": (_i, [_p, _i, _i, _i, _p, _i, _i, _i, _i, _i, _p, _p, _i64, _p]),
    "vgan_iforest_scores": (_i, [_p, _i64, _i, _i, _i64, _p, _i64, _p]),
    "vgan_iforest_build_blocks": (_i, [_p, _i64, _i64, _i, _i, _i, _i, _i, _i, _u64, _p, _p]),
    "vgan_iforest_path_sums_blocks": (_i, [_p, _i64, _i, _i, _p, _i, _i, _i, _i, _i, _p, _p, _i64, _p]),
    "vgan_dif_weights": (_i, [_p, _i, _i, _i, _i, _p, _i, _p, _u64, _p, _p, _i64, _p]),
    "vgan_dif_represent": (_i, [_p, _i, _i, _i, _p, _p, _p, _p, _i, _i, _i, _i, _p, _i, _i, _p, _p, _p, _p]),
    "vgan_ae_init": (_i, [_p, _i, _i, _i, _p, _p, _u64, _p, _p, _i64, _p]),
    "vgan_ae_train": (_i, [_p, _i, _i, _i, _p, _p, _p, _p, _p, _i, _i, _i, _i, _p, _i, _i, _u64, _i64, _i, _p, _d, _d, _d, _d, _d, _p, _p,
                           _p, _i64, _p, _i64, _p]),
    "vgan_ae_scores": (_i, [_p, _i, _i, _i, _p, _p, _p, _p, _p, _i, _i, _i, _i, _p, _i, _p, _p, _p, _i64, _p, _p, _i64, _p]),
    "vgan_inne_build": (_i, [_p, _i, _i64, _i, _p, _p, _i, _i, _i, _i, _i, _i, _u64, _p, _p, _p, _p, _p]),
    "vgan_inne_scores": (_i, [_p, _i, _i, _i, _p, _i, _i64, _p, _p, _i, _i, _i, _i, _i, _p, _p, _p, _p, _i64, _p]),
    "vgan_maha_moments": (_i, [_p, _i, _i, _i, _p, _p, _p, _i, _i, _i, _i, _p, _i, _p, _i64, _p, _p, _p, _p, _i64, _p]),
    "vgan_maha_factor": (_i, [_p, _p, _p, _i, _i, _i, _p, ctypes.c_double, _p, _p, _p, _p, _p]),
    "vgan_maha_scores": (_i, [_p, _i, _i, _i, _p, _p, _p, _i, _i, _i, _p, _p, _p, _i64, _p]),
    "vgan_maha_select": (_i, [_p, _i64, _i, _i, _i, _p, _p, _i64, _p, _p]),
    "vgan_pca_eigen": (_i, [_p, _p, _p, _i, _i, _i, _i, _i, _p, _p, _p, _p, _p, _p]),
    "vgan_pca_scores": (_i, [_p, _i, _i, _i, _p, _p, _p, _i, _i, _i, _p, _p, _p, _p, _p, _i64, _p]),
    "vgan_gmm_moments": (_i, [_p, _i, _i, _i, _p, _p, _p, _i, _i, _i, _i, _i, _p, _i, _p, _p, ctypes.c_double, _p, _p, _p, _p, _p, _p,
                              _i64, _p]),
    "vgan_gmm_logdet": (_i, [_p, _p, _p, _i, _i, _i, _p, _p]),
    "vgan_gmm_estep": (_i, [_p, _i, _i, _i, _p, _p, _p, _i, _i, _i, _i, _p, _p, _p, _p, _p, _p, _p, _p, _i64, _p]),
    "vgan_gmm_converge": (_i, [_p, _i, _i, _i, _i, _p, ctypes.c_double, _i, _p, _p, _p, _p, _p]),
    "vgan_ocsvm_kernel_matrix": (_i, [_p, _p, _i, _p, _p, _i, _i, _p, _i, _i, _p, _p]),
    "vgan_ocsvm_init": (_i, [_p, _i, _i, _i, ctypes.c_double, _p, _p, _p, _p, _p]),
    "vgan_ocsvm_smo": (_i, [_p, _i, _i, ctypes.c_double, _i, _i, _i, _p, _p, _p, _p, _p]),
    "vgan_ocsvm_rho": (_i, [_p, _p, _i, _i, _p, _p]),
    "vgan_ocsvm_scores": (_i, [_p, _p, _i, _p, _p, _i, _p, _p, _i, _i, _p, _p, _p, _i, _i, _p, _p, _p, _i64, _p]),
    "vgan_sos_distance_matrix": (_i, [_p, _p, _i, _p, _p, _i, _i, _i, _i, _i, _p, _p]),
    "vgan_sos_fit": (_i, [_p, _i, _i, ctypes.c_double, ctypes.c_double, _i, _i, _p, _p, _p, _p, _p, _p]),
    "vgan_sos_fit_scores": (_i, [_p, _i, _i, _p, _p, _p, _p, _p, _i64, _p]),
    "vgan_sos_scores": (_i, [_p, _p, _i, _p, _p, _i, _p, _p, _i, _i, _i, _p, _p, _p, _i, _i, _p, _p, _p, _i64, _p]),
    "vgan_sod_reverse_lists": (_i, [_p, _i, _i, _i, _p, _p, _p, _p]),
    "vgan_sod_reference_sets": (_i, [_p, _i, _p, _p, _i, _i, _i, _i, _i, _p, _p, _p]),
    "vgan_sod_score": (_i, [_p, _i, _i, _p, _i, _i, _i, _p, _p, _i, _i, _p, _i, ctypes.c_double, _i, _p, _p, _i, _p, _p, _i, _p]),
    "vgan_kpca_center": (_i, [_p, _i, _i, _p, _p, _p, _p]),
    "vgan_kpca_kernel_rows": (_i, [_p, _p, _i, _p, _p, _i, _p, _p, _i, _i, _p, _i, _i, _p, _p]),
    "vgan_kpca_row_means": (_i, [_p, _i64, _i, _p, _p]),
    "vgan_kpca_scores": (_i, [_p, _i, _i, _i, _i, _p, _p, _p, _p, _p, _p, _p, _i64, _p]),
}

ABI_VERSION = 11
_lib = None


class VganHipError(RuntimeError):
    pass


def load():
    global _lib
    if _lib is not None:
        return _lib
    if not os.path.exists(LIB_PATH):
        raise VganHipError(
            f"{LIB_PATH} is missing: build it with `python -c 'import __graft_entry__ as g; g.build()'` "
            "(or `make -C v-gan_amd/csrc`).  vgan_amd has no CPU fallback.")
    lib = ctypes.CDLL(LIB_PATH)
    for name, (res, args) in SIGNATURES.items():
        fn = getattr(lib, name)
# ... 48 lines not shown
```

v-gan_amd/ops.py:

```python
import ctypes

import torch

from . import lib as _lib

_f32 = torch.float32


def _round4(v):
    return (int(v) + 3) // 4 * 4


def _ptr(t):
    return ctypes.c_void_p(t.data_ptr()) if t is not None else None


def _mat(t, name):
    if not (t.is_cuda and t.dtype == _f32 and t.dim() == 2 and t.stride(1) == 1):
        raise ValueError(f"{name}: need a float32 HIP matrix with unit inner stride, got "
                         f"{t.dtype} {tuple(t.shape)} strides {t.stride()} on {t.device}")
    return t


def _vec(t, name, dtype=_f32):
    if not (t.is_cuda and t.dtype == dtype and t.is_contiguous()):
        raise ValueError(f"{name}: need a contiguous {dtype} HIP tensor, got {t.dtype} on {t.device}")
    return t


class HipOps:

    name = "hip"

    def __init__(self):
        self.lib = _lib.load()
        if not torch.cuda.is_available():
            raise _lib.VganHipError("vgan_amd needs a HIP device (torch.cuda.is_available() is False); "
                                    "there is no CPU fallback")

    @staticmethod
    def _stream():
        return ctypes.c_void_p(torch.cuda.current_stream().cuda_stream)

    def build_tiles(self, n, grad_mode, rank=0, world=1, device=None, tile=64, split_xx=False, split=None):
        flat, cnt = _lib.build_tiles(n, grad_mode, rank, world, tile)
        table = torch.tensor(flat, dtype=torch.int32).view(cnt, 8)
        if split_xx or split:
            first, second = _lib.split_tiles(table, tile, yy_last=(split == "yy_last"))
            return torch.cat([first, second]).to(device or "cuda"), first.shape[0]
        return table.to(device or "cuda")

    def colmax_chunks(self, n):
        return self.lib.vgan_colmax_chunks(n)

    def linear_forward(self, x, W, b, y, x_nslabs=1, x_slab_stride=0):
        _mat(x, "x"), _mat(W, "W"), _mat(y, "y")
        n, kin = x.shape
        out = W.shape[0]
        assert W.shape[1] == kin and y.shape == (n, out)
        _lib.check(self.lib.vgan_linear_forward(_ptr(x), x.stride(0), int(x_nslabs), int(x_slab_stride), _ptr(W), W.stride(0),
                                                _ptr(b), _ptr(y), y.stride(0), n, kin, out, self._stream()), "vgan_linear_forward")

    def linear_forward_path(self, x, W, b, y, x_nslabs=1, x_slab_stride=0):
        n, kin = x.shape
        return _lib.path_name(_lib.LINEAR_FORWARD_PATHS, self.lib.vgan_linear_forward_path(
            _ptr(x), x.stride(0), int(x_nslabs), int(x_slab_stride), _ptr(W), W.stride(0), _ptr(b), _ptr(y), y.stride(0), n, kin,
            W.shape[0]), "vgan_linear_forward_path")

    def linear_backward_input(self, dy, W, dx):
        _mat(dy, "dy"), _mat(W, "W"), _mat(dx, "dx")
        n, out = dy.shape
        kin = W.shape[1]
        assert W.shape[0] == out and dx.shape == (n, kin)
        _lib.check(self.lib.vgan_linear_backward_input(_ptr(dy), dy.stride(0), _ptr(W), W.stride(0), _ptr(dx), dx.stride(0),
                                                       n, kin, out, self._stream()), "vgan_linear_backward_input")

    def linear_backward_input_path(self, dy, W, dx):
        n, out = dy.shape
        return _lib.path_name(_lib.LINEAR_BACKWARD_INPUT_PATHS, self.lib.vgan_linear_backward_input_path(
            _ptr(dy), dy.stride(0), _ptr(W), W.stride(0), _ptr(dx), dx.stride(0), n, W.shape[1], out), "vgan_linear_backward_input_path")

    def linear_backward_params(self, dy, x, dW, db, splits=1, slab_stride=0, x_nslabs=1, x_slab_stride=0):
        _mat(dy, "dy"), _mat(x, "x"), _mat(dW, "dW")
        n, out = dy.shape
        kin = x.shape[1]
        assert x.shape[0] == n and dW.shape == (out, kin)
        _lib.check(self.lib.vgan_linear_backward_params(_ptr(dy), dy.stride(0), _ptr(x), x.stride(0), int(x_nslabs), int(x_slab_stride),
                                                        _ptr(dW), dW.stride(0), _ptr(db), n, kin, out, int(splits), int(slab_stride),
                                                        self._stream()), "vgan_linear_backward_params")

    def linear_backward_params_path(self, dy, x, dW, db, splits=1, slab_stride=0, x_nslabs=1, x_slab_stride=0):
        n, out = dy.shape
        return _lib.path_name(_lib.LINEAR_BACKWARD_PARAMS_PATHS, self.lib.vgan_linear_backward_params_path(
            _ptr(dy), dy.stride(0), _ptr(x), x.stride(0), int(x_nslabs), int(x_slab_stride), _ptr(dW), dW.stride(0), _ptr(db), n,
            x.shape[1], out, int(splits), int(slab_stride)), "vgan_linear_backward_params_path")

    def linear_backward_params_ksplit_ws_bytes(self, kin, out, parts):
        return int(self.lib.vgan_linear_backward_params_ksplit_ws_bytes(int(kin), int(out), int(parts)))

    def ksplit_workspace(self, nbytes, device=None):
        return torch.zeros(max(int(nbytes), 16) // 4 + 4, dtype=torch.int32, device=device or "cuda")

    def linear_backward_params_ksplit(self, dy, x, dW, parts, ws):
        _mat(dy, "dy"), _mat(x, "x"), _mat(dW, "dW")
        n, out = dy.shape
        kin = x.shape[1]
        assert x.shape[0] == n and dW.shape == (out, kin)
        _lib.check(self.lib.vgan_linear_backward_params_ksplit(_ptr(dy), dy.stride(0), _ptr(x), x.stride(0), _ptr(dW), dW.stride(0), n, kin, out,
                                                               int(parts), _ptr(ws), 0 if ws is None else ws.numel() * ws.element_size(),
                                                               self._stream()), "vgan_linear_backward_params_ksplit")

    def linear_backward_params_xx_supported(self, n, kin, out):
        return bool(self.lib.vgan_linear_backward_params_xx_supported(int(n), int(kin), int(out)))

    def linear_backward_params_xx(self, dy, x, dW, xx):
        _mat(dy, "dy"), _mat(x, "x"), _mat(dW, "dW")
        n, out = dy.shape
        kin = x.shape[1]
        assert x.shape[0] == n and dW.shape == (out, kin)
        _lib.check(self.lib.vgan_linear_backward_params_xx(_ptr(dy), dy.stride(0), _ptr(x), x.stride(0), _ptr(dW), dW.stride(0), n, kin, out,
                                                           ctypes.byref(xx), self._stream()), "vgan_linear_backward_params_xx")

    def reduce_slabs(self, src, slab_stride, nslabs, dst):
        _vec(dst, "dst")
        _lib.check(self.lib.vgan_reduce_slabs(_ptr(src), int(slab_stride), int(nslabs), _ptr(dst), dst.numel(), self._stream()),
                   "vgan_reduce_slabs")

    def col_mean(self, data, out):
        _mat(data, "data"), _vec(out, "out")
        rows, d = data.shape
        assert out.numel() >= d
        _lib.check(self.lib.vgan_col_mean(_ptr(data), data.stride(0), rows, d, _ptr(out), self._stream()), "vgan_col_mean")

    @staticmethod
    def logits_chain(za, At4):
        _mat(za, "za"), _mat(At4, "At4")
        assert za.shape[1] == At4.shape[1]
        return _lib.LogitsChain(_ptr(za), _ptr(At4), za.stride(0), At4.stride(0), za.shape[1], 0)

    @staticmethod
    def chain_fusable(n, d, *lds):
        return d % 4 == 0 and d <= 1024 and all(int(v) % 4 == 0 for v in lds)

    def mask_project_forward(self, logits, data, rows, S, U, Zx, Zy, sqx, sqy, row_cursor=None, row_batches=1, row_stride=0,
                             row_offset=0, center=None, norm_split=False, chain=None):
        _mat(data, "data"), _mat(Zy, "Zy"), _mat(S, "S")
        n, d = S.shape
        if logits is not None:
            _mat(logits, "logits")
            assert tuple(logits.shape) == (n, d)
        assert S.is_contiguous() and S.shape == (n, d) and (U is None or (U.is_contiguous() and U.shape == (n, d)))
        assert Zx is None or Zx.stride(0) == Zy.stride(0)
        if rows is not None:
            _vec(rows, "rows", torch.int32)
        _lib.check(self.lib.vgan_mask_project_forward(_ptr(logits), logits.stride(0) if logits is not None else 0, _ptr(data), data.stride(0), _ptr(rows),
                                                      _ptr(row_cursor), int(row_batches), int(row_stride), int(row_offset), _ptr(S), _ptr(U), _ptr(Zx), _ptr(Zy), Zy.stride(0), _ptr(sqx), _ptr(sqy),
                                                      n, d, _ptr(center), int(bool(norm_split)),
                                                      ctypes.byref(chain) if chain is not None else None, self._stream()), "vgan_mask_project_forward")

    bf3_rebuild = True
    chain_ksplit = True

    def xx_job(self, Dh, Dl, dsq, tiles, bw, partial):
        assert tiles.is_contiguous() and partial.is_contiguous() and Dh.stride(0) == Dl.stride(0)
        return _lib.XXJob(_ptr(Dh), _ptr(Dl), _ptr(dsq), _ptr(tiles), _ptr(bw), _ptr(partial), Dh.stride(0), tiles.shape[0])

    def bwd_rebuild(self, data, xrow, S, center):
        _mat(data, "data"), _mat(S, "S")
        assert xrow.dtype == torch.int32 and xrow.is_contiguous() and center.is_contiguous()
        return _lib.BwdRebuild(_ptr(data), _ptr(xrow), _ptr(S), _ptr(center), data.stride(0), S.stride(0))

    def mask_project_forward_bf3(self, logits, data, rows, S, Z, sq, Zh, Zl, ZTh, ZTl, row_cursor=None, row_batches=1, row_stride=0,
                                 center=None, write_x=True, xx=None, chain=None, write_z=True, xrow=None):
        _mat(data, "data"), _mat(Z, "Z"), _mat(S, "S")
        n, d = S.shape
        if logits is not None:
            _mat(logits, "logits")
        if not write_z or xrow is not None:
            _lib.check(self.lib.vgan_mask_project_forward_bf3_ex(_ptr(logits), logits.stride(0) if logits is not None else 0, _ptr(data),
                                                                 data.stride(0), _ptr(rows), _ptr(row_cursor), int(row_batches),
                                                                 int(row_stride), _ptr(S), _ptr(Z), Z.stride(0), _ptr(sq), _ptr(Zh), _ptr(Zl),
                                                                 Zh.stride(0), _ptr(ZTh), _ptr(ZTl), ZTh.stride(0) if ZTh is not None else 0,
                                                                 n, d, _ptr(center), int(bool(write_x)),
                                                                 ctypes.byref(xx) if xx is not None else None,
                                                                 ctypes.byref(chain) if chain is not None else None, int(bool(write_z)),
                                                                 _ptr(xrow), self._stream()), "vgan_mask_project_forward_bf3_ex")
            return
        _lib.check(self.lib.vgan_mask_project_forward_bf3(_ptr(logits), logits.stride(0) if logits is not None else 0, _ptr(data), data.stride(0), _ptr(rows),
                                                          _ptr(row_cursor), int(row_batches), int(row_stride), _ptr(S), _ptr(Z), Z.stride(0),
                                                          _ptr(sq), _ptr(Zh), _ptr(Zl), Zh.stride(0), _ptr(ZTh), _ptr(ZTl),
                                                          ZTh.stride(0) if ZTh is not None else 0,
                                                          n, d, _ptr(center), int(bool(write_x)),
                                                          ctypes.byref(xx) if xx is not None else None,
                                                          ctypes.byref(chain) if chain is not None else None, self._stream()),
                   "vgan_mask_project_forward_bf3")

    @staticmethod
    def bf3_fusable(n, d, *lds):
        return d % 4 == 0 and d <= 1024 and n % 8 == 0 and all(int(v) % 4 == 0 for v in lds)

    def gather_rows(self, data, rows, out, sq, row_cursor=None, row_batches=1, row_stride=0, row_offset=0):
        _mat(data, "data"), _mat(out, "out")
        n, d = out.shape[0], data.shape[1]
        _lib.check(self.lib.vgan_gather_rows(_ptr(data), data.stride(0), _ptr(rows), _ptr(row_cursor), int(row_batches),
                                             int(row_stride), int(row_offset), _ptr(out), out.stride(0), _ptr(sq), n, d,
                                             self._stream()), "vgan_gather_rows")

    def gather_rows_split(self, data, rows, center, out, sq, norm_split=False, Zh=None, Zl=None, row_cursor=None, row_batches=1,
                          row_stride=0, row_offset=0, n=None):
        _mat(data, "data")
        d = data.shape[1]
        n = int(n if n is not None else (out.shape[0] if out is not None else sq.numel()))
        _lib.check(self.lib.vgan_gather_rows_split(_ptr(data), data.stride(0), _ptr(rows), _ptr(row_cursor), int(row_batches),
                                                   int(row_stride), int(row_offset), _ptr(center), _ptr(out),
                                                   out.stride(0) if out is not None else 0, _ptr(sq), int(bool(norm_split)), _ptr(Zh),
                                                   _ptr(Zl), Zh.stride(0) if Zh is not None else 0, n, d, self._stream()),
                   "vgan_gather_rows_split")

    def upper_softmax_forward(self, logits, S, U):
        _mat(logits, "logits")
        n, d = logits.shape
        assert S.is_contiguous() and (U is None or U.is_contiguous())
        _lib.check(self.lib.vgan_upper_softmax_forward(_ptr(logits), logits.stride(0), _ptr(S), _ptr(U), n, d, self._stream()),
                   "vgan_upper_softmax_forward")

    def mask_backward(self, gU, S, colkey, pen_weight, row_offset, dlogits, nslabs=1, slab_stride=0):
        _mat(gU, "gU"), _mat(S, "S"), _mat(dlogits, "dlogits")
        n, d = S.shape
        _lib.check(self.lib.vgan_mask_backward(_ptr(gU), gU.stride(0), int(nslabs), int(slab_stride), _ptr(S), S.stride(0),
                                               _ptr(colkey), float(pen_weight),
                                               int(row_offset), _ptr(dlogits), dlogits.stride(0), n, d, self._stream()),
                   "vgan_mask_backward")

    def colmax(self, S, row_offset, part, colkey, from_softmax=True):
        _mat(S, "S")
        n, d = S.shape
        assert part.dtype == torch.int64 and colkey.dtype == torch.int64 and part.numel() >= self.colmax_chunks(n) * d
        _lib.check(self.lib.vgan_colmax(_ptr(S), S.stride(0), int(bool(from_softmax)), int(row_offset), _ptr(part), _ptr(colkey), n, d, self._stream()),
                   "vgan_colmax")

    def colmax_partial(self, S, row_offset, part, from_softmax=True):
        _mat(S, "S")
        n, d = S.shape
        assert part.dtype == torch.int64 and part.numel() >= self.colmax_chunks(n) * d
        _lib.check(self.lib.vgan_colmax_partial(_ptr(S), S.stride(0), int(bool(from_softmax)), int(row_offset), _ptr(part), n, d,
                                                self._stream()), "vgan_colmax_partial")

    def mmd_finalize(self, partial, tiles, colpart, chunks, colkey, n, d, weight, stats, loss, loss_accum=None, accum_scale=1.0,
                     step_counter=None):
        _lib.check(self.lib.vgan_mmd_finalize(_ptr(partial), _ptr(tiles), tiles.shape[0], _ptr(colpart), int(chunks), _ptr(colkey),
                                              int(n), int(d), float(weight), _ptr(stats), _ptr(loss), _ptr(loss_accum),
                                              float(accum_scale), _ptr(step_counter), self._stream()), "vgan_mmd_finalize")

    def finalize_job(self, partial, tiles, colpart, chunks, colkey, n, d, weight, stats, loss, loss_accum=None, accum_scale=1.0,
                     step_counter=None, mode=0, ntiles_main=0):
        return _lib.FinalizeJob(_ptr(partial), _ptr(tiles), _ptr(colpart), _ptr(colkey), _ptr(stats), _ptr(loss), _ptr(loss_accum),
                                _ptr(step_counter), tiles.shape[0], int(chunks), int(n), int(d), float(weight), float(accum_scale),
                                int(mode), int(ntiles_main))

    def mask_from_softmax(self, S, U):
        _mat(S, "S"), _mat(U, "U")
        n, d = S.shape
        _lib.check(self.lib.vgan_mask_from_softmax(_ptr(S), S.stride(0), _ptr(U), U.stride(0), n, d, self._stream()),
# ... 1047 lines not shown
```

v-gan_amd/step_plan.py:

```python
import dataclasses
import os
from typing import Optional, Union


def _round4(v):
    return (v + 3) // 4 * 4


def _launch_rounds(tiles, slots, can_split):
    if tiles <= 0:
        return 0.0
    full, r = divmod(tiles, slots)
    if r == 0:
        return float(full)
    x = r / slots
    last = 0.55 if x <= 0.5 else 0.55 + 0.9 * (x - 0.5)
    if can_split and x <= 0.125:
        last = 0.25
    elif can_split and x <= 0.25:
        last = 0.4
    elif can_split and x <= 0.5:
        last = 0.5
    return full + last


def _best_boundary(n_main, total, slots, can_split):
    cost = lambda k: _launch_rounds(k, slots, can_split) + _launch_rounds(total - k, slots, can_split)
    best, best_cost = n_main, cost(n_main)
    for k in range(n_main - 1, max(n_main - slots, 0), -1):
        c = cost(k)
        if c < best_cost - 1e-9 and c <= cost(n_main) - 0.15:
            best, best_cost = k, c
    return best


CHAIN_KPARTS_AUTO = 4


def chain_kparts(want, tiles, k, chain_flops=False):
    if want != "auto":
        parts = int(want)
        if parts not in (1, 2, 4, 8):
            raise ValueError(f"VGAN_CHAIN_KPARTS must be auto, 1, 2, 4 or 8, got {want!r}")
        return parts
    if chain_flops or not (32 <= tiles <= 64 and k >= 768):
        return 1
    return CHAIN_KPARTS_AUTO


def _knob(var, default, parse=str):
    return dataclasses.field(default=None if default is None else parse(default), metadata=dict(var=var, default=default, parse=parse))


_is_1 = lambda v: v == "1"
_not_0 = lambda v: v != "0"


@dataclasses.dataclass(frozen=True)
class Knobs:
    generator: str = _knob("VGAN_GENERATOR", "collapsed")
    fuse_update: bool = _knob("VGAN_FUSE_UPDATE", "0", _is_1)
    dp_front: str = _knob("VGAN_DP_FRONT", "auto")
    chain_assoc: str = _knob("VGAN_CHAIN_ASSOC", "auto")
    chain_splitk: bool = _knob("VGAN_CHAIN_SPLITK", "1", _is_1)
    mmd_precision: str = _knob("VGAN_MMD_PRECISION", "auto")
    bwd_tile: int = _knob("VGAN_BWD_TILE", "0", int)
    bwd_transposed: bool = _knob("VGAN_BWD_OPERAND", "rowmajor", lambda v: v == "transposed")
    bwd_splits: Optional[int] = _knob("VGAN_BWD_SPLITS", None, lambda v: None if v is None else int(v))
    fused_prepare: bool = _knob("VGAN_FUSED_PREPARE", "1", _is_1)
    chain_in_mask: bool = _knob("VGAN_CHAIN_IN_MASK", "0", _is_1)
    logits_2stage: bool = _knob("VGAN_LOGITS_2STAGE", "0", _is_1)
    gram_tile: str = _knob("VGAN_GRAM_TILE", "auto")
    gram_tail: bool = _knob("VGAN_GRAM_TAIL", "1", _not_0)
    rs_from_gram: bool = _knob("VGAN_RS_FROM_GRAM", "1", _not_0)
    overlap: Union[None, bool, str] = _knob("VGAN_OVERLAP", None, lambda v: {"1": True, "0": False}.get(v, v))
    xx_ride: bool = _knob("VGAN_XX_RIDE", "0", _is_1)
    xx_in_m4: bool = _knob("VGAN_XX_IN_M4", "1", _is_1)
    gram_slots: int = _knob("VGAN_GRAM_SLOTS", "512", int)
    xx_late_in_backward: bool = _knob("VGAN_XX_LATE", "backward", lambda v: v == "backward")
    chain_kparts: str = _knob("VGAN_CHAIN_KPARTS", "auto")
    z_fp32: bool = _knob("VGAN_Z_FP32", "0", _is_1)

    @classmethod
    def from_env(cls, environ=os.environ):
        return cls(**{f.name: f.metadata["parse"](environ.get(f.metadata["var"], f.metadata["default"])) for f in dataclasses.fields(cls)})


@dataclasses.dataclass(frozen=True)
class StepPlan:
    mode: str
    exchange: bool
    front_sharded: bool
    fuse_update: bool
    chain_flops: bool
    fwd_split: Optional[dict]
    bwd_split: Optional[dict]
    precision: str
    bf3: bool
    bwd_tile: int
    splits: int
    bsplits: int
    rm_backward: bool
    fused_prepare: bool
    chain_in_mask: bool
    two_stage_logits: bool
    gram_tile: int
    gram_tail: bool
    rs_from_gram: bool
    overlap: bool
    side_stream: bool
    x_ahead: bool
    xx_ride: bool
    xx_in_m4: bool
    xx_late_in_backward: bool
    tile_split: Optional[str]
    n_tiles: int
    n_main: int
    cal_shares_tiles: bool
    m4_kparts: int
    tn_kparts: int
    lean: bool
    col_chunks: int
    nl: int
    lo: int
    dp: int
    e: list
    kp: int
    kn: int


def plan_step(ops, *, n, d, data_stride, latent, widths, world, rank, force_exchange, generator_mode, mmd_precision,
              overlap_exchange, fuse_update, front, chain_assoc, knobs, host_tables=None):
    assert widths[0] == latent and len(widths) == 5
    exchange = world > 1 or bool(force_exchange)
    if n % world != 0:
        raise ValueError(f"global batch {n} must be divisible by the number of ranks {world}")
    nl = n // world
    lo, dp = rank * nl, _round4(d)
    mode = generator_mode or knobs.generator
    if mode not in ("collapsed", "layered"):
        raise ValueError(f"generator_mode must be 'collapsed' or 'layered', got {mode!r}")
    collapsed = mode == "collapsed"
    fuse_update = knobs.fuse_update if fuse_update is None else bool(fuse_update)
    want_front = front or knobs.dp_front
    if want_front not in ("auto", "replicated", "sharded"):
        raise ValueError(f"front must be 'auto', 'replicated' or 'sharded', got {want_front!r}")
    if want_front == "sharded" and not (exchange and collapsed):
        raise ValueError("front='sharded' needs a data-parallel engine (world > 1 or force_exchange) with the collapsed generator")
    front_sharded = exchange and collapsed and (want_front == "sharded" or (want_front == "auto" and n * d >= (1 << 22)))

    splits = max(1, min(8, nl // 128))
    e = [_round4(w + 1) for w in widths]
    chain_flops, fwd_split, bwd_split = False, None, None
    if collapsed:
        want_assoc = chain_assoc or knobs.chain_assoc
        if want_assoc not in ("auto", "depth", "flops"):
            raise ValueError(f"chain_assoc must be 'auto', 'depth' or 'flops', got {want_assoc!r}")
        chain_flops = want_assoc == "flops" or (want_assoc == "auto" and 2.0 * e[4] * e[3] * e[2] >= 1e9)
    if chain_flops:
        fuse_update = False
        def split_of(m, n_, k):
            t64 = ((m + 63) // 64) * ((n_ + 63) // 64)
            return 1 if (2.0 * m * n_ * k < 2.5e8 or not knobs.chain_splitk) else max(1, min(8, 1024 // t64, k // 256))
        fwd_split = {k: split_of(e[k], e[0], e[k - 1]) for k in (2, 3, 4)}
        bwd_split = {k: split_of(e[k - 1], e[0], e[k]) for k in (4, 3, 2)}

    precision = mmd_precision or knobs.mmd_precision
    if precision not in ("auto", "fp32", "bf16x3"):
        raise ValueError(f"mmd_precision must be 'auto', 'fp32' or 'bf16x3', got {precision!r}")
    if precision == "auto":
        precision = "bf16x3" if 2 * n * d >= (1 << 20) else "fp32"
    bf3 = precision == "bf16x3"
    bwd_tile = knobs.bwd_tile
    rm_backward = not bf3 or front_sharded or not knobs.bwd_transposed
    out_tiles = ((nl + 63) // 64) * ((d + 63) // 64)
    auto_splits = max(2 if bf3 else 1, min(4, 256 // max(out_tiles, 1), max(1, (2 * n) // 64)))
    if bf3 and rm_backward and bwd_tile in (0, 256) and ops.mmd_backward_bf3_tile(nl, d, 1, bwd_tile) == 256:
        auto_splits = 1
    bsplits = max(1, auto_splits if knobs.bwd_splits is None else knobs.bwd_splits)
    bwd_edge = ops.mmd_backward_bf3_tile(nl, d, bsplits, bwd_tile) if bf3 else 0
    fused_prepare = bf3 and not front_sharded and ops.bf3_fusable(n, d, d, data_stride, dp) and knobs.fused_prepare
    chain_in_mask = (collapsed and not front_sharded and ops.chain_fusable(n, d, data_stride, dp) and
                     (not bf3 or fused_prepare) and knobs.chain_in_mask)
    two_stage_logits = collapsed and not chain_flops and not chain_in_mask and not front_sharded and knobs.logits_2stage

    def count_tiles(tile, split=None):
        table = ops.build_tiles(n, 1, rank, world, device="cpu", tile=tile, split=split)
        if host_tables is not None:
            host_tables[tile, split] = table
        return (table[0].shape[0], table[1]) if split else (len(table), len(table))

    gram_tile = 64
    for edge in (128, 256):
        if bf3 and nl % edge == 0 and knobs.gram_tile in ("auto", str(edge)):
            if knobs.gram_tile == str(edge) or count_tiles(edge)[0] >= 512:
                gram_tile = edge
    small_tiles = gram_tile == 64
    gram_tail = gram_tile == 256 and knobs.gram_tail
    rs_from_gram = gram_tile == 256 and rm_backward and n % 128 == 0 and knobs.rs_from_gram and bwd_edge == 256

    if overlap_exchange is None:
        overlap_exchange = knobs.overlap
    overlap = False if overlap_exchange is None else bool(overlap_exchange)
    if front_sharded and overlap:
        raise ValueError("overlap_exchange and front='sharded' are two schedules of the same exchange: choose one")
    side_stream = overlap and overlap_exchange != "serial"
    x_ahead = overlap and rm_backward
    plain_schedule = not overlap and not front_sharded

    xx_ride = False
    if fused_prepare and small_tiles and plain_schedule and rm_backward and knobs.xx_ride:
        total, first = count_tiles(64, "xx_last")
        xx_tiles = total - first
        xx_ride = xx_tiles > 0 and 8 * ((n // 8 + 7) // 8) + xx_tiles <= 512
    xx_in_m4 = (bf3 and collapsed and small_tiles and plain_schedule and not xx_ride and
                ops.linear_backward_params_xx_supported(nl, e[0], dp) and knobs.xx_in_m4)
    if front_sharded:
        tile_split = "yy_last"
        n_tiles, n_main = count_tiles(gram_tile, tile_split)
        slots = 256 if gram_tile >= 128 else (512 if bf3 else 1024)
        n_main = _best_boundary(n_main, n_tiles, slots, gram_tail)
    elif overlap or xx_ride or xx_in_m4:
        tile_split = "xx_last"
        n_tiles, n_main = count_tiles(gram_tile, tile_split)
        if xx_in_m4:
            n_main = min(n_tiles, max(n_main, knobs.gram_slots))
            xx_in_m4 = n_main < n_tiles
    else:
        tile_split = None
        n_tiles, n_main = count_tiles(gram_tile)
    bwd_wgs = ((d + 63) // 64) * ((nl + 63) // 64) * bsplits + 1
    xx_late_in_backward = (xx_in_m4 and rm_backward and knobs.xx_late_in_backward and bwd_edge == 64 and
                           n_tiles - n_main <= 512 - bwd_wgs)
    cal_shares_tiles = world == 1 and small_tiles and plain_schedule and not xx_ride and not xx_in_m4

    m4_kparts = tn_kparts = 1
    if collapsed and getattr(ops, "chain_ksplit", False):
        t32 = lambda rows, cols: ((rows + 31) // 32) * ((cols + 31) // 32)
        if not (xx_in_m4 and not xx_late_in_backward):
            m4_kparts = chain_kparts(knobs.chain_kparts, t32(dp, e[0]), nl, chain_flops)
        tn_tiles = sum(t32(e[k], e[0]) for k in (3, 2, 1))
        if not chain_flops and e[4] >= 96 and tn_tiles <= 256:
            tn_kparts = chain_kparts(knobs.chain_kparts, tn_tiles, e[4])
    lean = (getattr(ops, "bf3_rebuild", False) and fused_prepare and small_tiles and rm_backward and world == 1 and
            plain_schedule and bwd_edge == 64 and not knobs.z_fp32)
    col_chunks = (world * ops.colmax_chunks(nl)) if front_sharded else ops.colmax_chunks(n)
    return StepPlan(mode=mode, exchange=exchange, front_sharded=front_sharded, fuse_update=fuse_update, chain_flops=chain_flops,
                    fwd_split=fwd_split, bwd_split=bwd_split, precision=precision, bf3=bf3, bwd_tile=bwd_tile, splits=splits,
                    bsplits=bsplits, rm_backward=rm_backward, fused_prepare=fused_prepare, chain_in_mask=chain_in_mask,
                    two_stage_logits=two_stage_logits, gram_tile=gram_tile, gram_tail=gram_tail, rs_from_gram=rs_from_gram,
                    overlap=overlap, side_stream=side_stream, x_ahead=x_ahead, xx_ride=xx_ride, xx_in_m4=xx_in_m4,
                    xx_late_in_backward=xx_late_in_backward, tile_split=tile_split, n_tiles=n_tiles, n_main=n_main,
                    cal_shares_tiles=cal_shares_tiles, m4_kparts=m4_kparts, tn_kparts=tn_kparts, lean=lean, col_chunks=col_chunks,
                    nl=nl, lo=lo, dp=dp, e=e, kp=(d + 63) // 64 * 64, kn=(2 * n + 63) // 64 * 64)
```

v-gan_amd/trainer.py:

```python
import contextlib
import gc
import os

import torch

from .step_plan import CHAIN_KPARTS_AUTO, Knobs, _best_boundary, _launch_rounds, _round4, chain_kparts, plan_step

ADADELTA_RHO = 0.9
ADADELTA_EPS = 1e-6


@contextlib.contextmanager
def no_gc_while_capturing():
    was_enabled = gc.isenabled()
    gc.collect()
    gc.disable()
    try:
        yield
    finally:
        if was_enabled:
            gc.enable()


class FlatParams:

    def __init__(self, params, device):
        self.shapes = [tuple(p.shape) for p in params]
        self.offsets = []
        off = 0
        for p in params:
            self.offsets.append(off)
            off += _round4(p.numel())
        self.total = off
        self.flat = torch.zeros(off, dtype=torch.float32, device=device)
        self.grad = torch.zeros_like(self.flat)
        self.sq = torch.zeros_like(self.flat)
        self.acc = torch.zeros_like(self.flat)
        for k, (p, o) in enumerate(zip(params, self.offsets)):
            self.flat[o:o + p.numel()].copy_(p.detach().reshape(-1).to(device=device, dtype=torch.float32))
            p.data = self.view(self.flat, k)

    def view(self, buf, k):
        o, shp = self.offsets[k], self.shapes[k]
        numel = 1
        for s in shp:
            numel *= s
        return buf[o:o + numel].view(shp)


class NoKLStepEngine:
    def __init__(self, ops, generator, data, batch_size, batches_per_epoch, lr=0.007, weight_decay=0.04, penalty_weight=10.0,
                 seed=777, noise="device", rank=0, world=1, group=None, use_graph=True, loss_accum_scale=None,
                 generator_mode=None, force_exchange=False, mmd_precision=None, center_operand=True, overlap_exchange=None,
                 fuse_update=None, front=None, chain_assoc=None):
        self.ops = ops
        self.dev = data.device
        self.rank, self.world, self.group = rank, world, group
        n = self.n = int(batch_size)
        self.data = data
        d = self.d = data.shape[1]
        self.nb = int(batches_per_epoch)
        self.lr, self.wd, self.pen = float(lr), float(weight_decay), float(penalty_weight)
        self.seed = int(seed)
        self.noise_mode = noise
        self.use_graph = bool(use_graph) and data.is_cuda
        self.graph = None
        self.graph_multi = None
        self.graph_blocks = {}
        self.steps_per_graph = max(1, min(16, int(batches_per_epoch)))
        self.steps_done = 0
        self._xx_primed = False
        self._coalesce = None
        lin = [m for m in generator.main if isinstance(m, torch.nn.Linear)]
        assert len(lin) == 4
        L = self.L = lin[0].in_features
        self.widths = [L] + [m.out_features for m in lin]
        tables = {}
        self.plan = plan_step(ops, n=n, d=d, data_stride=data.stride(0), latent=L, widths=self.widths, world=world, rank=rank,
                              force_exchange=force_exchange, generator_mode=generator_mode, mmd_precision=mmd_precision,
                              overlap_exchange=overlap_exchange, fuse_update=fuse_update, front=front, chain_assoc=chain_assoc,
                              knobs=Knobs.from_env(), host_tables=tables)
        vars(self).update(vars(self.plan))
        self._alloc_generator([q for m in lin for q in (m.weight, m.bias)])
        self._alloc_mmd(center_operand)
        self.perm = torch.zeros(self.nb, n, dtype=torch.int32, device=self.dev)
        self.perm_next = torch.zeros_like(self.perm)
        self.epoch_staged = False
        self._alloc_carriers()
        self._alloc_tiles(tables[self.gram_tile, self.tile_split])
        self._hist, self._hist_n, self._hist_events = None, 0, []
        self._read_stream, self._loss_host = None, None
        self.accum_scale = (1.0 / self.nb) if loss_accum_scale is None else float(loss_accum_scale)
        if self.front_sharded and data.is_cuda and self._collect().is_initialized():
            self._coalesce = self._probe_coalescing(self._collect())

    def _alloc_generator(self, params):
        ops, n, nl, d, L, e = self.ops, self.n, self.nl, self.d, self.L, self.e
        f32 = dict(dtype=torch.float32, device=self.dev)
        self.fp = FlatParams(params, self.dev)
        self.W = [self.fp.view(self.fp.flat, 2 * k) for k in range(4)]
        self.b = [self.fp.view(self.fp.flat, 2 * k + 1) for k in range(4)]
        self.za = torch.zeros(n, e[0], **f32)
        self.za[:, L] = 1.0
        self.z_own = self.za[self.lo:self.lo + nl]
        self.logits = torch.zeros(n, d, **f32)
        self._chain = None
        if self.mode == "layered":
            self.gslab = torch.zeros(self.splits, self.fp.total, **f32) if self.splits > 1 else None
            gbase = self.gslab[0] if self.splits > 1 else self.fp.grad
            self.dW = [self.fp.view(gbase, 2 * k) for k in range(4)]
            self.db = [self.fp.view(gbase, 2 * k + 1) for k in range(4)]
            self.acts = [self.za[:, :L]] + [torch.zeros(n, w, **f32) for w in self.widths[1:4]] + [self.logits]
            self.acts_own = [a[self.lo:self.lo + nl] for a in self.acts]
            self.dacts = [None] + [torch.zeros(nl, w, **f32) for w in self.widths[1:4]]
            return
        poff = [0]
        for k in range(1, 5):
            poff.append(poff[-1] + e[k] * e[k - 1])
        self.Wt_all = torch.zeros(poff[-1], **f32)
        self.Gt_all = torch.zeros(poff[-1], **f32)
        self.Wt = [None] + [self.Wt_all[poff[k - 1]:poff[k]].view(e[k], e[k - 1]) for k in range(1, 5)]
        self.Gt = [None] + [self.Gt_all[poff[k - 1]:poff[k]].view(e[k], e[k - 1]) for k in range(1, 5)]
        self.At = [None, self.Wt[1]] + [torch.zeros(e[k], e[0], **f32) for k in range(2, 5)]
        self.M = [None, self.Gt[1]] + [torch.zeros(e[k], e[0], **f32) for k in range(2, 5)]
        self.B3 = torch.zeros(e[4], e[2], **f32)
        self.B2 = torch.zeros(e[4], e[1], **f32)
        self.At1s = torch.zeros(e[1], e[0], **f32)
        if self.chain_flops:
            need = max([self.fwd_split[k] * e[k] * e[0] for k in (2, 3, 4)] + [self.bwd_split[k] * e[k - 1] * e[0] for k in (4, 3, 2)])
            self.chain_ws = torch.zeros(need, **f32)
        pmap = torch.full((self.fp.total,), -1, dtype=torch.int32)
        for k in range(1, 5):
            wk, wk1 = self.widths[k], self.widths[k - 1]
            r = torch.arange(wk, dtype=torch.int32)[:, None] * e[k - 1]
            ow, ob = self.fp.offsets[2 * (k - 1)], self.fp.offsets[2 * (k - 1) + 1]
            pmap[ow:ow + wk * wk1] = (poff[k - 1] + r + torch.arange(wk1, dtype=torch.int32)[None, :]).reshape(-1)
            pmap[ob:ob + wk] = (poff[k - 1] + r + wk1).reshape(-1)
        self.pmap = pmap.to(self.dev)
        self.pack_layers = [(self.W[k - 1], self.b[k - 1], self.Wt[k]) for k in range(1, 5)]
        self.unpack_layers = [(self.fp.view(self.fp.grad, 2 * (k - 1)), self.fp.view(self.fp.grad, 2 * (k - 1) + 1), self.Gt[k])
                              for k in range(1, 5)]
        ops.homogeneous_pack(self.pack_layers, unpack=False)

    def _alloc_mmd(self, center_operand):
        n, nl, d, dp = self.n, self.nl, self.d, self.dp
        f32, i16 = dict(dtype=torch.float32, device=self.dev), dict(dtype=torch.int16, device=self.dev)
        self.center = torch.zeros(dp, **f32)
        if center_operand:
            self.ops.col_mean(self.data, self.center)
        self.S = torch.zeros(n, d, **f32)
        self.S_own = self.S[self.lo:self.lo + nl]
        self.Z = torch.zeros(2 * n, dp, **f32)
        self.sqn = torch.zeros(2 * n, **f32)
        self.sq_cal = torch.zeros(2 * n, **f32) if self.bf3 else self.sqn
        self.Wg = torch.zeros(nl, 2 * n, **f32)
        self.gU_slabs = torch.zeros(self.bsplits, nl, dp, **f32)
        self.gU = self.gU_slabs[0]
        self.dlogits_pad = torch.zeros(nl, dp, **f32)
        self.dlogits = self.dlogits_pad[:, :d]
        if self.bf3:
            self.Zh, self.Zl = torch.zeros(2 * n, self.kp, **i16), torch.zeros(2 * n, self.kp, **i16)
            if self.rm_backward:
                self.ZTh = self.ZTl = None
            else:
                self.ZTh, self.ZTl = torch.zeros(self.kp, self.kn, **i16), torch.zeros(self.kp, self.kn, **i16)
            self.Wh, self.Wl = torch.zeros(nl, self.kn, **i16), torch.zeros(nl, self.kn, **i16)

    def _alloc_tiles(self, host_table):
        ops, n, nl, d, rank = self.ops, self.n, self.nl, self.d, self.rank
        f32 = dict(dtype=torch.float32, device=self.dev)
        self.tiles = (host_table[0] if self.tile_split else host_table).to(self.dev)
        self.tiles_cal = self.tiles if self.cal_shares_tiles else ops.build_tiles(n, 0, 0, 1, device=self.dev)
        self.partial = torch.zeros(max(self.tiles.shape[0], self.tiles_cal.shape[0]), 4, **f32)
        self.stats = torch.zeros(4, dtype=torch.float64, device=self.dev)
        self.bw = torch.zeros(1, **f32)
        self.has_bw = False
        self.loss = torch.zeros(1, **f32)
        self.loss_accum = torch.zeros(1, **f32)
        self.step_counter = torch.zeros(1, dtype=torch.int64, device=self.dev)
        self.colpart = torch.zeros(self.col_chunks * d, dtype=torch.int64, device=self.dev)
        own = ops.colmax_chunks(nl) * d
        self.colpart_own = self.colpart[rank * own:(rank + 1) * own] if self.front_sharded else self.colpart
        self.colkey = torch.zeros(d, dtype=torch.int64, device=self.dev)
        self._fin = self._fold = None

    def _alloc_carriers(self):
        ops, n, nl, dp, e = self.ops, self.n, self.nl, self.dp, self.e
        f32 = dict(dtype=torch.float32, device=self.dev)
        if self.two_stage_logits:
            self.T = torch.zeros(n, e[2], **f32)
            self.T_ws = torch.zeros(((n + 63) // 64) * ((e[2] + 63) // 64) * 64 * _round4(e[1]), **f32)
        self.gram_tail_ws = ops.gram_tail_workspace(self.dev) if self.gram_tail else None
        self.rs_part = torch.zeros((2 * n + 127) // 128, nl, **f32) if self.rs_from_gram else None
        self._side = torch.cuda.Stream(device=self.dev) if (self.side_stream and self.data.is_cuda) else None
        self._xx = self._xx_m4 = self._rebuild = None
        if self.xx_ride:
            i16 = dict(dtype=torch.int16, device=self.dev)
            rows_total = self.data.shape[0]
            self.Dh, self.Dl = torch.zeros(rows_total, self.kp, **i16), torch.zeros(rows_total, self.kp, **i16)
            self.dsq = torch.zeros(rows_total, **f32)
            ops.gather_rows_split(self.data, None, self.center, None, self.dsq, True, self.Dh, self.Dl, n=rows_total)
        self.m4_ws = self.tn_ws = None
        if self.m4_kparts > 1:
            self.m4_ws = ops.ksplit_workspace(ops.linear_backward_params_ksplit_ws_bytes(e[0], dp, self.m4_kparts), self.dev)
        if self.tn_kparts > 1:
            tn = [("TN", self.Wt[4], self.M[4], self.M[3]), ("TN", self.B3, self.M[4], self.M[2]), ("TN", self.B2, self.M[4], self.M[1])]
            self.tn_ws = ops.ksplit_workspace(ops.gemm_grouped_ksplit_ws_bytes(tn, [self.tn_kparts] * 3), self.dev)
        self.xrow = torch.zeros(n, dtype=torch.int32, device=self.dev) if self.lean else None

    def set_epoch_batches(self, idx):
        if os.environ.get("VGAN_FEED_DIRECT") == "1":
            self.perm.copy_(idx.to(dtype=torch.int32), non_blocking=True)
            self._after_new_epoch_table()
            return
        self.stage_epoch_batches(idx)
        self.begin_epoch()

    def stage_epoch_batches(self, idx):
        self.perm_next.copy_(idx.to(dtype=torch.int32).view(self.nb, self.n), non_blocking=True)
        self.epoch_staged = True

    def begin_epoch(self):
        if not self.epoch_staged:
            raise RuntimeError("begin_epoch without a staged table (stage_epoch_batches)")
        self.perm.copy_(self.perm_next)
        self.epoch_staged = False
        self._after_new_epoch_table()

    def _after_new_epoch_table(self):
        if self.overlap and self.has_bw:
            self._prefetch_xx()

    def _prefetch_xx(self):
        self._prefetch_x_operand()
        self._xx_tiles()
        self._xx_primed = True

    def _prefetch_x_operand(self):
        ops, n = self.ops, self.n
        rowsel = dict(row_cursor=self.step_counter, row_batches=self.nb, row_stride=n)
        if self.bf3:
            ops.gather_rows_split(self.data, self.perm, self.center, self.Z[:n], self.sqn[:n], True, self.Zh[:n], self.Zl[:n], **rowsel)
        else:
            ops.gather_rows_split(self.data, self.perm, self.center, self.Z[:n], self.sqn[:n], False, **rowsel)

    def _xx_tiles(self):
        ops, n = self.ops, self.n
        ntx = self.tiles.shape[0] - self.n_main
        if ntx == 0:
            return
        tx, px = self.tiles[self.n_main:], self.partial[self.n_main:self.n_main + ntx]
        if self.bf3:
            ops.mmd_gram_bf3(self.Zh, self.Zl, self.sqn, n, self.bw, tx, None, None, 0, px, tile=self.gram_tile)
        else:
            ops.mmd_gram(self.Z, self.sqn, n, self.dp, self.bw, tx, False, None, 0, px)

    def _fork_prefetch(self):
        if not self.overlap:
            return
        if self._side is None:
            self._prefetch_xx()
            return
        self._side.wait_stream(torch.cuda.current_stream())
        with torch.cuda.stream(self._side):
            self._prefetch_xx()

    def _join_prefetch(self):
        if self.overlap and self._side is not None:
            torch.cuda.current_stream().wait_stream(self._side)

    def shuffle_epoch(self, epoch):
        self.ops.shuffle_epoch(self.perm, self.data.shape[0], self.seed, int(epoch))
        self._after_new_epoch_table()

    def set_bandwidth(self, value):
        self.bw.fill_(float(value))
        self.has_bw = True

    def set_noise(self, z):
        self.za[:, :self.L].copy_(z.to(dtype=torch.float32), non_blocking=True)

    def epoch_loss(self):
        v = float(self._sum_over_ranks(self.loss_accum).item())
        self.loss_accum.zero_()
        return v

    def close_epoch(self):
        if self._hist is None or self._hist_n == self._hist.numel():
            grown = torch.zeros(max(64, 2 * self._hist_n), dtype=torch.float32, device=self.dev)
            if self._hist is not None:
                grown[:self._hist_n].copy_(self._hist)
            self._hist = grown
        slot = self._hist_n
        cell = self._hist[slot:slot + 1]
        cell.copy_(self.loss_accum)
        self.loss_accum.zero_()
        if self.exchange:
            self._collect().all_reduce(cell, group=self.group)
        ev = None
        if self.data.is_cuda:
            ev = torch.cuda.Event()
            ev.record()
        self._hist_events.append(ev)
        self._hist_n += 1
        return slot

    def read_epoch_loss(self, slot):
        ev = self._hist_events[slot]
        if ev is None:
            return float(self._hist[slot])
        if self._read_stream is None:
            self._read_stream = torch.cuda.Stream(self.dev)
            self._loss_host = torch.zeros(1, dtype=torch.float32).pin_memory()
        self._read_stream.wait_event(ev)
        with torch.cuda.stream(self._read_stream):
            self._loss_host.copy_(self._hist[slot:slot + 1], non_blocking=True)
        self._read_stream.synchronize()
        return float(self._loss_host[0])

    def step_loss(self):
        return float(self._sum_over_ranks(self.loss).item())

    def _sum_over_ranks(self, t):
        if not self.exchange:
            return t
        t = t.clone()
        self._collect().all_reduce(t, group=self.group)
        return t

    def grad_view(self, k):
        if self.mode == "collapsed":
            self.ops.homogeneous_pack(self.unpack_layers, unpack=True)
        elif not self.exchange and self.splits > 1:
            return sum(self.fp.view(self.gslab[sl], k) for sl in range(self.splits))
        return self.fp.view(self.fp.grad, k)

    def _generator_forward(self, own_rows=False):
        ops = self.ops
        if self.mode == "layered":
            for k in range(4):
                ops.linear_forward(self.acts[k], self.W[k], self.b[k], self.acts[k + 1])
            return
        Wt, At = self.Wt, self.At
        if self.chain_flops:
            for k in (2, 3, 4):
                sp = self.fwd_split[k]
                if sp > 1:
                    ops.gemm_grouped([("NN", Wt[k], At[k - 1], self._slabs(sp, At[k]), sp)])
                    ops.reduce_slabs(self.chain_ws, At[k].numel(), sp, At[k])
                else:
                    ops.gemm_grouped([("NN", Wt[k], At[k - 1], At[k])])
        elif self.two_stage_logits:
            ops.gemm_grouped([("NN", Wt[2], At[1], At[2]), ("NN", Wt[4], Wt[3], self.B3), ("NT2", self.za, Wt[1], self.T, Wt[2], self.T_ws)])
            ops.gemm_grouped([("NN", Wt[3], At[2], At[3]), ("NN", self.B3, Wt[2], self.B2), ("NT", self.T, self.B3[:self.d], self.logits)])
            return
        else:
            ops.gemm_grouped([("NN", Wt[2], At[1], At[2]), ("NN", Wt[4], Wt[3], self.B3)])
            ops.gemm_grouped([("NN", Wt[3], At[2], At[3]), ("NN", self.B3, At[2], At[4]), ("NN", self.B3, Wt[2], self.B2)])
        if own_rows:
            ops.linear_forward(self.z_own, At[4][:self.d], None, self.logits[self.lo:self.lo + self.nl])
        elif not self.chain_in_mask:
            ops.linear_forward(self.za, At[4][:self.d], None, self.logits)

    def _slabs(self, splits, like):
        return self.chain_ws[:splits * like.numel()].view(splits, like.shape[0], like.shape[1])

    def _generator_backward_update(self, dist):
        ops = self.ops
        adadelta = dict(lr=self.lr, rho=ADADELTA_RHO, eps=ADADELTA_EPS, weight_decay=self.wd, grad_scale=1.0)
        if self.mode == "layered":
            g = self.dlogits
            for k in (3, 2, 1, 0):
                ops.linear_backward_params(g, self.acts_own[k], self.dW[k], self.db[k], self.splits, self.fp.total)
                if k:
                    ops.linear_backward_input(g, self.W[k], self.dacts[k])
                    g = self.dacts[k]
            if dist:
                if self.splits > 1:
                    ops.reduce_slabs(self.gslab, self.fp.total, self.splits, self.fp.grad)
                dist.all_reduce(self.fp.grad, group=self.group)
                ops.adadelta_step(self.fp.flat, self.fp.grad, self.fp.sq, self.fp.acc, **adadelta)
            elif self.splits > 1:
                ops.adadelta_step(self.fp.flat, self.gslab[0], self.fp.sq, self.fp.acc, nslabs=self.splits, slab_stride=self.fp.total,
                                  **adadelta)
            else:
                ops.adadelta_step(self.fp.flat, self.fp.grad, self.fp.sq, self.fp.acc, **adadelta)
            return
        e, d = self.e, self.d
        if self.xx_in_m4 and not self.xx_late_in_backward:
            ops.linear_backward_params_xx(self.dlogits_pad, self.z_own, self.M[4][:self.dp], self._late_xx_job())
        elif self.m4_kparts > 1:
            ops.linear_backward_params_ksplit(self.dlogits_pad, self.z_own, self.M[4][:self.dp], self.m4_kparts, self.m4_ws)
        else:
            ops.linear_backward_params(self.dlogits_pad, self.z_own, self.M[4][:self.dp], None)
        if dist:
            dist.all_reduce(self.M[4], group=self.group)
        M, Gt, At = self.M, self.Gt, self.At
        fused_noise = dict(next_noise=self.za, noise_cols=self.L, noise_ones_col=self.L, seed=self.seed,
                           step_counter=self.step_counter) if self.noise_mode == "device" else {}
        if self.chain_flops:
            Wt = self.Wt
            for k in (4, 3, 2):
                sp = self.bwd_split[k]
                probs = [("TN", Wt[k], M[k], self._slabs(sp, M[k - 1]), sp) if sp > 1 else ("TN", Wt[k], M[k], M[k - 1])]
                if k < 4:
                    probs.append(("NT", M[k + 1], At[k], Gt[k + 1]))
                ops.gemm_grouped(probs, fold=self._fold if (self.xx_in_m4 and k == 4) else None)
                if sp > 1:
                    ops.reduce_slabs(self.chain_ws, M[k - 1].numel(), sp, M[k - 1])
            ops.gemm_grouped([("NT", M[2], At[1], Gt[2])])
            ops.adadelta_step_packed(self.fp.flat, self.pmap, self.Gt_all, self.Wt_all, self.fp.sq, self.fp.acc, **adadelta, **fused_noise)
            return
        tn_split = dict(kparts=[self.tn_kparts] * 3, ksplit_ws=self.tn_ws) if self.tn_kparts > 1 else {}
        if not self.fuse_update:
            ops.gemm_grouped([("TN", self.Wt[4], M[4], M[3]), ("TN", self.B3, M[4], M[2]), ("TN", self.B2, M[4], M[1])],
                             fold=self._fold if self.xx_in_m4 else None, **tn_split)
            ops.gemm_grouped([("NT", M[4], At[3], Gt[4]), ("NT", M[3], At[2], Gt[3]), ("NT", M[2], At[1], Gt[2])])
            ops.adadelta_step_packed(self.fp.flat, self.pmap, self.Gt_all, self.Wt_all, self.fp.sq, self.fp.acc, **adadelta, **fused_noise)
            return
        ops.gemm_grouped([("TN", self.Wt[4], M[4], M[3]), ("TN", self.B3, M[4], M[2]), ("TN", self.B2, M[4], M[1])],
                         copy=(self.Wt[1], self.At1s), fold=self._fold if self.xx_in_m4 else None, **tn_split)
        w, off = self.widths, self.fp.offsets
        layers = [(self.Wt[k], off[2 * (k - 1)], off[2 * (k - 1) + 1], w[k], w[k - 1]) for k in (4, 3, 2, 1)]
        ops.gemm_grouped([("NT", M[4], At[3], Gt[4]), ("NT", M[3], At[2], Gt[3]), ("NT", M[2], self.At1s, Gt[2])],
                         adadelta=dict(p=self.fp.flat, sq=self.fp.sq, acc=self.fp.acc, layers=layers, extra_grad=Gt[1], **adadelta),
                         noise=fused_noise or None)

    def _collect(self):
        import torch.distributed as dist
        return dist

    def _forward(self):
        ops, n, nl, lo = self.ops, self.n, self.nl, self.lo
        if self.noise_mode == "device" and (self.mode == "layered" or self.steps_done == 0):
            ops.noise_normal(self.za, self.seed, self.step_counter, 0, cols=self.L, ones_col=self.L)
        self._generator_forward()
        rowsel = dict(row_cursor=self.step_counter, row_batches=self.nb, row_stride=n)
        logits = self.logits
        if self.chain_in_mask:
            if self._chain is None:
                self._chain = ops.logits_chain(self.za, self.At[4][:self.d])
            rowsel["chain"] = self._chain
            logits = None
        if self.fused_prepare:
            xx = None
            if self.xx_ride and self.has_bw:
                if self._xx is None:
                    ntx = self.tiles.shape[0] - self.n_main
                    self._xx = ops.xx_job(self.Dh, self.Dl, self.dsq, self.tiles[self.n_main:], self.bw, self.partial[self.n_main:self.n_main + ntx])
                xx = self._xx
            if self.lean:
                ops.mask_project_forward_bf3(logits, self.data, self.perm, self.S, self.Z, self.sqn, self.Zh, self.Zl, None, None,
                                             center=self.center, xx=xx, write_z=not self.has_bw, xrow=self.xrow, **rowsel)
            else:
                ops.mask_project_forward_bf3(logits, self.data, self.perm, self.S, self.Z, self.sqn, self.Zh, self.Zl, self.ZTh, self.ZTl,
                                             center=self.center, write_x=not self.x_ahead, xx=xx, **rowsel)
            return
        if self.x_ahead:
            ops.mask_project_forward(logits, self.data, self.perm, self.S, None, None, self.Z[n:], None, self.sqn[n:],
                                     row_offset=0, center=self.center, norm_split=self.bf3, **rowsel)
        else:
            ops.mask_project_forward(logits, self.data, self.perm, self.S, None, self.Z[:n], self.Z[n:], self.sqn[:n], self.sqn[n:],
                                     row_offset=0, center=self.center, norm_split=self.bf3, **rowsel)

    def _calibrate(self):
        ops = self.ops
        if self.bf3:
            ops.row_sqnorm(self.Z, self.sq_cal, self.dp)
        ops.mmd_gram(self.Z, self.sq_cal, self.n, self.dp, None, self.tiles_cal, True, None, 0, self.partial)
        ops.mmd_reduce(self.partial, self.tiles_cal, self.stats, True)
        ops.mmd_set_bandwidth(self.stats, self.n, self.bw)
        self.has_bw = True

    def _loss_backward_update(self):
        ops, n, nl, lo, d = self.ops, self.n, self.nl, self.lo, self.d
        dist = self._collect() if self.exchange else None
        gstride = nl * self.dp
        if self.bf3 and not self.fused_prepare:
            if self.x_ahead:
                ops.mmd_bf3_prepare(self.Z[n:], n, d, self.Zh[n:], self.Zl[n:])
            else:
                ops.mmd_bf3_prepare(self.Z, 2 * n, d, self.Zh, self.Zl, self.ZTh, self.ZTl)
        if self.bf3:
            ops.mmd_gram_bf3(self.Zh, self.Zl, self.sqn, n, self.bw, self.tiles[:self.n_main], self.Wh, self.Wl, n + lo, self.partial, self.S, 0,
                             self.colpart, True, tile=self.gram_tile, tail_ws=self.gram_tail_ws, rs_part=self.rs_part)
        else:
            ops.mmd_gram_colmax(self.Z, self.sqn, n, self.dp, self.bw, self.tiles[:self.n_main], self.Wg, n + lo, self.partial, self.S, 0,
                                self.colpart, True)
        if self._fin is None:
            fin_args = (self.partial, self.tiles, self.colpart, ops.colmax_chunks(n), self.colkey, n, d, self.pen if self.rank == 0 else 0.0,
                        self.stats, self.loss, self.loss_accum, self.accum_scale, self.step_counter)
            if self.xx_in_m4:
                self._fin = ops.finalize_job(*fin_args, mode=1, ntiles_main=self.n_main)
                self._fold = ops.finalize_job(*fin_args, mode=2, ntiles_main=self.n_main)
            else:
                self._fin = ops.finalize_job(*fin_args)
        fin = self._fin
        if self.bf3:
            if self.lean:
                if self._rebuild is None:
                    self._rebuild = ops.bwd_rebuild(self.data, self.xrow, self.S, self.center)
                ops.mmd_backward_bf3_rm_rebuild(self.Wh, self.Wl, self.Zh, self.Zl, 2 * n, nl, d, self._rebuild, self.gU, self.bsplits, gstride,
                                                fin, xx=self._late_xx_job() if self.xx_late_in_backward else None)
            elif self.rm_backward:
                ops.mmd_backward_bf3_rm(self.Wh, self.Wl, self.Zh, self.Zl, 2 * n, self.Z, n + lo, nl, d, self.Z[lo:lo + nl], self.gU,
                                        self.bsplits, gstride, fin, mul_shift=self.center, tile=self.bwd_tile,
                                        xx=self._late_xx_job() if self.xx_late_in_backward else None, rs_part=self.rs_part)
            else:
                ops.mmd_backward_bf3(self.Wh, self.Wl, self.ZTh, self.ZTl, self.Z, n + lo, nl, d, self.Z[lo:lo + nl], self.gU, self.bsplits,
                                     gstride, fin, mul_shift=self.center, tile=self.bwd_tile)
        else:
            ops.mmd_backward(self.Wg, self.Z, n + lo, nl, 2 * n, self.dp, self.Z[lo:lo + nl], self.gU, self.bsplits, gstride, fin,
                             mul_shift=self.center)
        self._fork_prefetch()
        ops.mask_backward(self.gU, self.S_own, self.colkey, self.pen, lo, self.dlogits, self.bsplits, gstride)
        self._generator_backward_update(dist)
        self._join_prefetch()

    def _forward_sharded(self):
        ops, n, nl, lo, d = self.ops, self.n, self.nl, self.lo, self.d
        if self.noise_mode == "device" and self.steps_done == 0:
            ops.noise_normal(self.za, self.seed, self.step_counter, 0, cols=self.L, ones_col=self.L)
        self._generator_forward(own_rows=True)
        rowsel = dict(row_cursor=self.step_counter, row_batches=self.nb, row_stride=n)
        own, yown = slice(lo, lo + nl), slice(n + lo, n + lo + nl)
        if self.bf3:
            ops.gather_rows_split(self.data, self.perm, self.center, None, self.sqn[:n], True, self.Zh[:n], self.Zl[:n], **rowsel)
        else:
            ops.gather_rows_split(self.data, self.perm, self.center, self.Z[:n], self.sqn[:n], False, **rowsel)
        ops.mask_project_forward(self.logits[own], self.data, self.perm, self.S_own, None, self.Z[own] if self.bf3 else None, self.Z[yown],
                                 None, self.sqn[yown], row_offset=lo, center=self.center, norm_split=self.bf3, **rowsel)
        if self.bf3:
            ops.mmd_bf3_prepare(self.Z[yown], nl, d, self.Zh[yown], self.Zl[yown])
        ops.colmax_partial(self.S_own, lo, self.colpart_own)

    def _all_gather(self, dist, out, own):
        size = dist.get_world_size(self.group) if dist.is_initialized() else 1
        if size != self.world:
            out = own
        if own.is_cuda and dist.get_backend(self.group) == "gloo":
            host = out.cpu()
            dist.all_gather_into_tensor(host, own.cpu(), group=self.group)
            out.copy_(host)
            return None
        return dist.all_gather_into_tensor(out, own, group=self.group, async_op=True)

    def _exchange_front(self, dist):
        n, nl, lo = self.n, self.nl, self.lo
        yown = slice(n + lo, n + lo + nl)
        pairs = []
        if self.bf3:
            pairs += [(img[n:2 * n].view(torch.int32), img[yown].view(torch.int32)) for img in (self.Zh, self.Zl)]
        else:
            pairs.append((self.Z[n:], self.Z[yown]))
        pairs += [(self.sqn[n:], self.sqn[yown]), (self.colpart, self.colpart_own)]
        if self._coalesce is None:
            self._coalesce = self._probe_coalescing(dist)
        if self._coalesce:
            emulated = dist.get_world_size(self.group) != self.world
            with dist._coalescing_manager(group=self.group, device=self.dev, async_ops=True) as cm:
                for out, own in pairs:
                    dist.all_gather_into_tensor(own if emulated else out, own, group=self.group)
            return [cm]
        return [self._all_gather(dist, out, own) for out, own in pairs]

    def _probe_coalescing(self, dist):
        if os.environ.get("VGAN_DP_COALESCE", "0") != "1" or not self.data.is_cuda or torch.cuda.is_current_stream_capturing():
            return False
        try:
            if dist.get_backend(self.group) != "nccl" or not hasattr(dist, "_coalescing_manager"):
                return False
            size = dist.get_world_size(self.group)
            a, b = torch.zeros(size * 4, device=self.dev), torch.zeros(size * 2, dtype=torch.int64, device=self.dev)
            r = dist.get_rank(self.group)
            with dist._coalescing_manager(group=self.group, device=self.dev, async_ops=True) as cm:
                dist.all_gather_into_tensor(a, a[4 * r:4 * r + 4], group=self.group)
                dist.all_gather_into_tensor(b, b[2 * r:2 * r + 2], group=self.group)
            cm.wait()
            torch.cuda.synchronize()
            return True
        except Exception as e:
            import warnings
            warnings.warn(f"vgan_amd: coalesced all-gather is not available on this stack ({type(e).__name__}: {e}); one launch per gather")
            return False

    def _loss_backward_update_sharded(self, all_rows_here=False):
        ops, n, nl, lo, d = self.ops, self.n, self.nl, self.lo, self.d
        dist = self._collect()
        works = []
        if all_rows_here:
            if self.bf3:
                ops.mmd_bf3_prepare(self.Z, 2 * n, d, self.Zh, self.Zl)
            self.colpart.zero_()
            ops.colmax_partial(self.S, 0, self.colpart[:ops.colmax_chunks(n) * d])
        else:
            works = self._exchange_front(dist)
        na = self.n_main

        def gram(t0, t1):
            if t1 <= t0:
                return
            if self.bf3:
                ops.mmd_gram_bf3(self.Zh, self.Zl, self.sqn, n, self.bw, self.tiles[t0:t1], self.Wh, self.Wl, n + lo, self.partial[t0:t1],
                                 tile=self.gram_tile, tail_ws=self.gram_tail_ws, rs_part=self.rs_part)
            else:
                ops.mmd_gram(self.Z, self.sqn, n, self.dp, self.bw, self.tiles[t0:t1], False, self.Wg, n + lo, self.partial[t0:t1])

        gram(0, na)
        for w in works:
            if w is not None:
                w.wait()
        gram(na, self.tiles.shape[0])
        if self._fin is None:
            self._fin = ops.finalize_job(self.partial, self.tiles, self.colpart, self.col_chunks, self.colkey, n, d,
                                         self.pen if self.rank == 0 else 0.0, self.stats, self.loss, self.loss_accum, self.accum_scale,
                                         self.step_counter)
        gstride = nl * self.dp
        if self.bf3:
            ops.mmd_backward_bf3_rm(self.Wh, self.Wl, self.Zh, self.Zl, 2 * n, self.Z, n + lo, nl, d, self.Z[lo:lo + nl], self.gU,
                                    self.bsplits, gstride, self._fin, mul_shift=self.center, tile=self.bwd_tile, rs_part=self.rs_part)
        else:
            ops.mmd_backward(self.Wg, self.Z, n + lo, nl, 2 * n, self.dp, self.Z[lo:lo + nl], self.gU, self.bsplits, gstride, self._fin,
                             mul_shift=self.center)
        ops.mask_backward(self.gU, self.S_own, self.colkey, self.pen, lo, self.dlogits, self.bsplits, gstride)
        self._generator_backward_update(dist)

    def _late_xx_job(self):
        if self._xx_m4 is None:
            ntx = self.tiles.shape[0] - self.n_main
            self._xx_m4 = self.ops.xx_job(self.Zh, self.Zl, self.sqn, self.tiles[self.n_main:], self.bw,
                                          self.partial[self.n_main:self.n_main + ntx])
        return self._xx_m4

    def _step_body(self):
        if self.front_sharded:
            self._forward_sharded()
            self._loss_backward_update_sharded()
        else:
            self._forward()
            self._loss_backward_update()

    def step(self):
        if not self.has_bw:
            if self.overlap:
                self._prefetch_x_operand()
            self._forward()
            self._calibrate()
            if self.overlap or self.xx_ride:
                self._xx_tiles()
                self._xx_primed = True
            if self.front_sharded:
                self._loss_backward_update_sharded(all_rows_here=True)
            else:
                self._loss_backward_update()
        elif self.use_graph and self.steps_done > 0:
            if self.graph is None:
                self._capture()
            if self.graph is not None:
                self.graph.replay()
            else:
                self._step_body()
        else:
            if self.overlap and not self._xx_primed:
                self._prefetch_xx()
            self._step_body()
        self.steps_done += 1

    def run_steps(self, count):
        count = int(count)
        if count > 1 and self.noise_mode != "device":
            raise ValueError("run_steps needs the device noise stream: host-provided noise is set per step (set_noise + step)")
        m = self.steps_per_graph
        while count > 0:
            blk = min(count, m)
            if (blk > 1 and self.use_graph and self.has_bw and self.steps_done > 0 and self.noise_mode == "device" and
                    self.graph is not None):
                g = self._block_graph(blk)
                if g is not None:
                    g.replay()
                    self.steps_done += blk
                    count -= blk
                    continue
            self.step()
            count -= 1

    def _block_graph(self, steps):
        g = self.graph_blocks.get(steps)
        if g is None and len(self.graph_blocks) < 4:
            g = self.graph_blocks[steps] = self._capture_graph(steps) or False
        if steps == self.steps_per_graph:
            self.graph_multi = g or None
        return g or None

    def _capture_graph(self, steps):
        torch.cuda.synchronize()
        g = torch.cuda.CUDAGraph()
        try:
            with no_gc_while_capturing(), torch.cuda.graph(g):
                for _ in range(steps):
                    self._step_body()
        except Exception as e:
            import warnings
            warnings.warn(f"vgan_amd: HIP-graph capture of {steps} training step(s) failed ({type(e).__name__}: {e}); running eager launches")
            torch.cuda.synchronize()
            g = None
        if self.exchange and self.world > 1:
            dist = self._collect()
            ok = torch.tensor([1 if g is not None else 0], dtype=torch.int32, device=self.dev)
            dist.all_reduce(ok, op=dist.ReduceOp.MIN, group=self.group)
            if int(ok.item()) == 0:
                g = None
        return g

    def _capture(self):
        self.graph = self._capture_graph(1)
        if self.graph is None:
            self.use_graph = False

    def generator_logits(self, z):
        ops = self.ops
        h = z.to(device=self.dev, dtype=torch.float32).contiguous()
        for k in range(4):
            y = torch.empty(h.shape[0], self.W[k].shape[0], dtype=torch.float32, device=self.dev)
            ops.linear_forward(h, self.W[k], self.b[k], y)
            h = y
        return h
```

Before: 9681 steps/s.

## Stage next step's data rows inside the k-split generator weight-gradient launch

```diff
diff --git a/include/vgan_hip.h b/include/vgan_hip.h
--- a/include/vgan_hip.h
+++ b/include/vgan_hip.h
@@ -33,6 +33,20 @@
 int64_t vgan_linear_backward_params_ksplit_ws_bytes(int in, int out, int parts);
 int vgan_linear_backward_params_ksplit(const float* dy, int lddy, const float* x, int ldx, float* dW, int lddw, int n, int in,
                                        int out, int parts, void* ws, int64_t ws_bytes, vgan_stream_t stream);
+typedef struct vgan_x_rows_job {
+    const float* data;
+    const float* center;
+    const int32_t* rows;
+    const uint64_t* row_cursor;
+    int32_t* xrow;
+    uint16_t* Zh;
+    uint16_t* Zl;
+    float* sq;
+    int32_t ldd, kp, n, d, row_batches, row_stride;
+} vgan_x_rows_job;
+int vgan_linear_backward_params_ksplit_xrows(const float* dy, int lddy, const float* x, int ldx, float* dW, int lddw, int n, int in,
+                                             int out, int parts, void* ws, int64_t ws_bytes, const vgan_x_rows_job* xjob,
+                                             vgan_stream_t stream);
 enum vgan_linear_forward_path_code {
     VGAN_LINEAR_FORWARD_T64_V4 = 0,
     VGAN_LINEAR_FORWARD_T64_V1 = 1,
diff --git a/v-gan_amd/csrc/linear.hip b/v-gan_amd/csrc/linear.hip
--- a/v-gan_amd/csrc/linear.hip
+++ b/v-gan_amd/csrc/linear.hip
@@ -1,5 +1,6 @@
 #include "gemm_core.hpp"
 #include "mmd_xx.hpp"
+#include "x_rows.hpp"
 
 namespace vgan {
 
@@ -129,13 +130,11 @@
         if (row < out && col < in) dW[(long)row * lddw + col] = o[rr];
     }
 }
-__global__ __launch_bounds__(1024, 1) void linear_bwd_params_ks_split_kernel(const float* __restrict__ dy, int lddy,
-                                                                            const float* __restrict__ x, int ldx, float* __restrict__ dW,
-                                                                            int lddw, int n, int in, int out, int kchunk, KSplitWs ws) {
+__device__ __forceinline__ void ks_split_tile(const float* __restrict__ dy, int lddy, const float* __restrict__ x, int ldx,
+                                              float* __restrict__ dW, int lddw, int n, int in, int out, int kchunk, const KSplitWs& ws,
+                                              int bx, int by, int gx, int part, int parts, float* lds) {
     using G = GemmTileKS<KSBK, MC, MC, 4, 16>;
-    __shared__ __attribute__((aligned(16))) float lds[G::kLdsFloats];
-    const int m0 = blockIdx.y * 32, n0 = blockIdx.x * 32;
-    const int part = blockIdx.z, parts = gridDim.z;
+    const int m0 = by * 32, n0 = bx * 32;
     const int k0 = part * kchunk, klen = min(kchunk, n - k0);
     float o[G::NR];
     if (klen > 0) {
@@ -144,7 +143,7 @@
 #pragma unroll
         for (int rr = 0; rr < G::NR; ++rr) o[rr] = 0.f;
     }
-    const int tile = blockIdx.y * gridDim.x + blockIdx.x;
+    const int tile = by * gx + bx;
     if (!ksplit_finish<G::NR, G::NTH>(o, ws, tile, tile * parts * kKSplitSlabBytes, part, parts, lds)) return;
     const int col = n0 + G::col_of();
 #pragma unroll
@@ -152,6 +151,28 @@
         const int row = m0 + G::row_of(rr);
         if (row < out && col < in) dW[(long)row * lddw + col] = o[rr];
     }
+}
+__global__ __launch_bounds__(1024, 1) void linear_bwd_params_ks_split_kernel(const float* __restrict__ dy, int lddy,
+                                                                            const float* __restrict__ x, int ldx, float* __restrict__ dW,
+                                                                            int lddw, int n, int in, int out, int kchunk, KSplitWs ws) {
+    using G = GemmTileKS<KSBK, MC, MC, 4, 16>;
+    __shared__ __attribute__((aligned(16))) float lds[G::kLdsFloats];
+    ks_split_tile(dy, lddy, x, ldx, dW, lddw, n, in, out, kchunk, ws, blockIdx.x, blockIdx.y, gridDim.x, blockIdx.z, gridDim.z, lds);
+}
+__global__ __launch_bounds__(1024, 1) void linear_bwd_params_ks_split_xrows_kernel(const float* __restrict__ dy, int lddy,
+                                                                                  const float* __restrict__ x, int ldx,
+                                                                                  float* __restrict__ dW, int lddw, int n, int in, int out,
+                                                                                  int kchunk, KSplitWs ws, int gx, int gy, int parts,
+                                                                                  XRowsJob xr) {
+    using G = GemmTileKS<KSBK, MC, MC, 4, 16>;
+    __shared__ __attribute__((aligned(16))) float lds[G::kLdsFloats];
+    const int ptiles = gx * gy, b = blockIdx.x;
+    if (b >= ptiles * parts) {
+        x_rows_body(xr, b - ptiles * parts);
+        return;
+    }
+    const int part = b / ptiles, t = b - part * ptiles;
+    ks_split_tile(dy, lddy, x, ldx, dW, lddw, n, in, out, kchunk, ws, t % gx, t / gx, gx, part, parts, lds);
 }
 __global__ __launch_bounds__(1024, 1) void linear_bwd_params_ks_xx_kernel(const float* __restrict__ dy, int lddy, const float* __restrict__ x,
                                                                          int ldx, float* __restrict__ dW, int lddw, int n, int in, int out,
@@ -354,6 +375,32 @@
     return VGAN_OK;
 }
 
+extern "C" int vgan_linear_backward_params_ksplit_xrows(const float* dy, int lddy, const float* x, int ldx, float* dW, int lddw, int n,
+                                                        int in, int out, int parts, void* ws, int64_t ws_bytes, const vgan_x_rows_job* xjob,
+                                                        vgan_stream_t stream) {
+    VGAN_CHECK_ARG(parts >= 2 && parts <= kKSplitMaxParts && xjob != nullptr);
+    VGAN_CHECK_ARG(dy && x && dW && n > 0 && in > 0 && out > 0 && lddy >= out && ldx >= in && lddw >= in);
+    VGAN_CHECK_ARG((out % 4 == 0) && (lddy % 4 == 0) && (in % 4 == 0) && (ldx % 4 == 0) && aligned16(dy) && aligned16(x));
+    const int64_t need = vgan_linear_backward_params_ksplit_ws_bytes(in, out, parts);
+    VGAN_CHECK_ARG(ws != nullptr && aligned16(ws) && ws_bytes >= need && need < (1ll << 31));
+    const vgan_x_rows_job& j = *xjob;
+    VGAN_CHECK_ARG(j.data && j.rows && j.xrow && j.Zh && j.Zl && j.sq && j.n > 0 && j.d > 0 && j.d % 4 == 0 && j.d <= 256 * kXRowsChunks);
+    VGAN_CHECK_ARG(j.ldd >= j.d && j.ldd % 4 == 0 && j.kp >= j.d && j.kp % 4 == 0 && j.row_batches >= 1 && j.row_stride >= 0);
+    VGAN_CHECK_ARG(aligned16(j.data) && aligned16(j.Zh) && aligned16(j.Zl) && (j.center == nullptr || aligned16(j.center)));
+    const int gx = (in + 31) / 32, gy = (out + 31) / 32;
+    const int xrows = x_rows_per_block(1024);
+    const long xblocks = (j.n + xrows - 1) / xrows;
+    VGAN_CHECK_ARG((long)gx * gy * parts + xblocks < (1l << 31));
+    const long tb = ksplit_ticket_bytes((long)gx * gy);
+    const KSplitWs k{reinterpret_cast<float*>(static_cast<char*>(ws) + tb), static_cast<int*>(ws), (int)(need - tb)};
+    const XRowsJob xr{j.data, j.center, RowSel{j.rows, reinterpret_cast<const unsigned long long*>(j.row_cursor), j.row_batches, j.row_stride, 0},
+                      j.xrow, j.Zh, j.Zl, j.sq, j.ldd, j.kp, j.n, j.d};
+    hipLaunchKernelGGL(linear_bwd_params_ks_split_xrows_kernel, dim3((unsigned)(gx * gy * parts + xblocks)), dim3(1024), 0, (hipStream_t)stream,
+                       dy, lddy, x, ldx, dW, lddw, n, in, out, ksplit_kchunk(n, parts, KSBK), k, gx, gy, parts, xr);
+    VGAN_CHECK_LAUNCH();
+    return VGAN_OK;
+}
+
 extern "C" int vgan_linear_backward_params_xx_supported(int n, int in, int out) {
     return (n >= 256 && in > 0 && out > 0 && in % 4 == 0 && out % 4 == 0 && use_ks(out, in, n)) ? 1 : 0;
 }
diff --git a/v-gan_amd/csrc/rows.hip b/v-gan_amd/csrc/rows.hip
--- a/v-gan_amd/csrc/rows.hip
+++ b/v-gan_amd/csrc/rows.hip
@@ -1,20 +1,11 @@
 #include "mmd_xx.hpp"
 #include "vgan_common.hpp"
+#include "x_rows.hpp"
 
 namespace vgan {
 
 constexpr int kRowsPerBlock = kBlock / kWave;
 
-struct RowSel {
-    const int* rows;
-    const unsigned long long* cursor;
-    int row_batches, row_stride, row_offset;
-    __device__ __forceinline__ long operator()(int i) const {
-        if (rows == nullptr) return (long)(row_offset + i);
-        const long b = cursor ? (long)(cursor[0] % (unsigned long long)row_batches) : 0l;
-        return (long)rows[b * row_stride + row_offset + i];
-    }
-};
 
 
 template <bool PROJECT>
@@ -182,7 +173,6 @@
     }
 }
 
-__device__ __forceinline__ float norm_term4(const float (&z)[4]) { return (z[0] * z[0] + z[1] * z[1]) + (z[2] * z[2] + z[3] * z[3]); }
 
 template <int NT, bool XX, bool CHAIN>
 __global__ __launch_bounds__(512) void mask_forward_bf3_kernel(const float* __restrict__ logits, int ldl, const float* __restrict__ data,
@@ -337,23 +327,20 @@
     const float4 xv = reinterpret_cast<const float4*>(data + src * ldd)[qc];
     if (xrow != nullptr && threadIdx.x == 0) xrow[i] = (int)src;
     if (!ok) v = make_float4(-INFINITY, -INFINITY, -INFINITY, -INFINITY);
-    const float4 x4c = make_float4(centred_x(xv.x, cv.x), centred_x(xv.y, cv.y), centred_x(xv.z, cv.z), centred_x(xv.w, cv.w));
-    const float xs[4] = {x4c.x, x4c.y, x4c.z, x4c.w};
+    if (write_x) {
+        float4 x4c;
+        uint2 ph, pl;
+        const float term = x_half_chunk4(xv, cv, x4c, ph, pl);
+        if (ok) {
+            if (write_z) reinterpret_cast<float4*>(Z + (long)i * ldz)[q] = x4c;
+            const long grow = (long)i * kp + 4 * q;
+            *reinterpret_cast<uint2*>(Zh + grow) = ph;
+            *reinterpret_cast<uint2*>(Zl + grow) = pl;
+        }
+        red_nx[wave][lane] = ok ? term : 0.f;
+    }
     unsigned short h[4], l[4];
-    float xn[4];
-#pragma unroll
-    for (int e = 0; e < 4; ++e) {
-        split_bf16(xs[e], h[e], l[e]);
-        xn[e] = bf16_val(h[e]) + bf16_val(l[e]);
-    }
-    if (ok && write_x) {
-        if (write_z) reinterpret_cast<float4*>(Z + (long)i * ldz)[q] = x4c;
-        const long grow = (long)i * kp + 4 * q;
-        *reinterpret_cast<uint2*>(Zh + grow) = make_uint2((unsigned)h[0] | ((unsigned)h[1] << 16), (unsigned)h[2] | ((unsigned)h[3] << 16));
-        *reinterpret_cast<uint2*>(Zl + grow) = make_uint2((unsigned)l[0] | ((unsigned)l[1] << 16), (unsigned)l[2] | ((unsigned)l[3] << 16));
-    }
     red_m[wave][lane] = fmaxf(fmaxf(v.x, v.y), fmaxf(v.z, v.w));
-    red_nx[wave][lane] = ok ? norm_term4(xn) : 0.f;
     __syncthreads();
     float m = -INFINITY;
 #pragma unroll
@@ -390,7 +377,7 @@
         float nx = 0.f, ny = 0.f;
 #pragma unroll
         for (int t = 0; t < NT; ++t) {
-            nx += red_nx[t][lane];
+            if (write_x) nx += red_nx[t][lane];
             ny += red_ny[t][lane];
         }
         nx = wave_sum(nx);
@@ -548,25 +535,17 @@
     const int nq = d >> 2;
     float nx = 0.f;
     for (int q = lane; q < nq; q += 64) {
-        float4 v = x4[q];
-        if (center) {
-            const float4 c = reinterpret_cast<const float4*>(center)[q];
-            v.x -= c.x; v.y -= c.y; v.z -= c.z; v.w -= c.w;
-        }
+        const float4 c = center ? reinterpret_cast<const float4*>(center)[q] : make_float4(0.f, 0.f, 0.f, 0.f);
+        float4 v;
+        uint2 ph, pl;
+        const float term = x_half_chunk4(x4[q], c, v, ph, pl);
         if (out) reinterpret_cast<float4*>(out + (long)i * ldo)[q] = v;
+        if (Zh) {
+            *reinterpret_cast<uint2*>(Zh + (long)i * kp + 4 * q) = ph;
+            *reinterpret_cast<uint2*>(Zl + (long)i * kp + 4 * q) = pl;
+        }
         const float vs[4] = {v.x, v.y, v.z, v.w};
-        unsigned short h[4], l[4];
-        float vn[4];
-#pragma unroll
-        for (int e = 0; e < 4; ++e) {
-            split_bf16(vs[e], h[e], l[e]);
-            vn[e] = norm_split ? bf16_val(h[e]) + bf16_val(l[e]) : vs[e];
-        }
-        if (Zh) {
-            *reinterpret_cast<uint2*>(Zh + (long)i * kp + 4 * q) = make_uint2((unsigned)h[0] | ((unsigned)h[1] << 16), (unsigned)h[2] | ((unsigned)h[3] << 16));
-            *reinterpret_cast<uint2*>(Zl + (long)i * kp + 4 * q) = make_uint2((unsigned)l[0] | ((unsigned)l[1] << 16), (unsigned)l[2] | ((unsigned)l[3] << 16));
-        }
-        nx += (vn[0] * vn[0] + vn[1] * vn[1]) + (vn[2] * vn[2] + vn[3] * vn[3]);
+        nx += norm_split ? term : norm_term4(vs);
     }
     nx = wave_sum(nx);
     if (lane == 0 && sq) sq[i] = nx;
diff --git a/v-gan_amd/csrc/x_rows.hpp b/v-gan_amd/csrc/x_rows.hpp
--- /dev/null
+++ b/v-gan_amd/csrc/x_rows.hpp
@@ -0,0 +1,93 @@
+#pragma once
+#include "vgan_common.hpp"
+
+namespace vgan {
+
+struct RowSel {
+    const int* rows;
+    const unsigned long long* cursor;
+    int row_batches, row_stride, row_offset;
+    __device__ __forceinline__ long operator()(int i) const {
+        if (rows == nullptr) return (long)(row_offset + i);
+        const long b = cursor ? (long)(cursor[0] % (unsigned long long)row_batches) : 0l;
+        return (long)rows[b * row_stride + row_offset + i];
+    }
+};
+
+__device__ __forceinline__ float norm_term4(const float (&z)[4]) {
+    return __fmaf_rn(z[0], z[0], z[1] * z[1]) + __fmaf_rn(z[2], z[2], z[3] * z[3]);
+}
+
+__device__ __forceinline__ uint2 pack_bf16x4(const unsigned short (&b)[4]) {
+    return make_uint2((unsigned)b[0] | ((unsigned)b[1] << 16), (unsigned)b[2] | ((unsigned)b[3] << 16));
+}
+
+__device__ __forceinline__ float x_half_chunk4(const float4& xv, const float4& cv, float4& xc, uint2& ph, uint2& pl) {
+    xc = make_float4(centred_x(xv.x, cv.x), centred_x(xv.y, cv.y), centred_x(xv.z, cv.z), centred_x(xv.w, cv.w));
+    const float xs[4] = {xc.x, xc.y, xc.z, xc.w};
+    unsigned short h[4], l[4];
+    float xn[4];
+#pragma unroll
+    for (int e = 0; e < 4; ++e) {
+        split_bf16(xs[e], h[e], l[e]);
+        xn[e] = bf16_val(h[e]) + bf16_val(l[e]);
+    }
+    ph = pack_bf16x4(h);
+    pl = pack_bf16x4(l);
+    return norm_term4(xn);
+}
+
+struct XRowsJob {
+    const float* data;
+    const float* center;
+    RowSel rows;
+    int* xrow;
+    unsigned short *Zh, *Zl;
+    float* sq;
+    int ldd, kp, n, d;
+};
+constexpr int kXRowsChunks = 4;
+constexpr int kXRowsPerWave = 1;
+__host__ __device__ constexpr int x_rows_per_block(int threads) { return (threads >> 6) * kXRowsPerWave; }
+
+__device__ __forceinline__ void x_rows_body(const XRowsJob& job, int blk) {
+    const int lane = threadIdx.x & 63, waves = (int)(blockDim.x >> 6);
+    const int i0 = blk * waves * kXRowsPerWave + (int)(threadIdx.x >> 6);
+    if (i0 >= job.n) return;
+    const int nq = job.d >> 2;
+    long src[kXRowsPerWave];
+    float4 xv[kXRowsPerWave][kXRowsChunks], cv[kXRowsChunks];
+#pragma unroll
+    for (int r = 0; r < kXRowsPerWave; ++r) {
+        src[r] = job.rows(min(i0 + r * waves, job.n - 1));
+        const float4* xr4 = reinterpret_cast<const float4*>(job.data + src[r] * job.ldd);
+#pragma unroll
+        for (int t = 0; t < kXRowsChunks; ++t) xv[r][t] = xr4[min(lane + 64 * t, nq - 1)];
+    }
+#pragma unroll
+    for (int t = 0; t < kXRowsChunks; ++t)
+        cv[t] = job.center ? reinterpret_cast<const float4*>(job.center)[min(lane + 64 * t, nq - 1)] : make_float4(0.f, 0.f, 0.f, 0.f);
+#pragma unroll
+    for (int r = 0; r < kXRowsPerWave; ++r) {
+        const int i = i0 + r * waves;
+        if (i >= job.n) break;
+        if (lane == 0) job.xrow[i] = (int)src[r];
+        float nx = 0.f;
+#pragma unroll
+        for (int t = 0; t < kXRowsChunks; ++t) {
+            const int q = lane + 64 * t;
+            if (q < nq) {
+                float4 xc;
+                uint2 ph, pl;
+                nx += x_half_chunk4(xv[r][t], cv[t], xc, ph, pl);
+                const long grow = (long)i * job.kp + 4 * q;
+                *reinterpret_cast<uint2*>(job.Zh + grow) = ph;
+                *reinterpret_cast<uint2*>(job.Zl + grow) = pl;
+            }
+        }
+        nx = wave_sum(nx);
+        if (lane == 0) job.sq[i] = nx;
+    }
+}
+
+}
diff --git a/v-gan_amd/lib.py b/v-gan_amd/lib.py
--- a/v-gan_amd/lib.py
+++ b/v-gan_amd/lib.py
@@ -34,6 +34,12 @@
 
 class BwdRebuild(ctypes.Structure):
     _fields_ = [("data", _p), ("xrow", _p), ("S", _p), ("center", _p), ("ldd", ctypes.c_int32), ("lds", ctypes.c_int32)]
+
+
+class XRowsJob(ctypes.Structure):
+    _fields_ = [("data", _p), ("center", _p), ("rows", _p), ("row_cursor", _p), ("xrow", _p), ("Zh", _p), ("Zl", _p), ("sq", _p),
+                ("ldd", ctypes.c_int32), ("kp", ctypes.c_int32), ("n", ctypes.c_int32), ("d", ctypes.c_int32),
+                ("row_batches", ctypes.c_int32), ("row_stride", ctypes.c_int32)]
 
 
 class AdadeltaLayer(ctypes.Structure):
@@ -66,6 +72,7 @@
     "vgan_linear_backward_params": (_i, [_p, _i, _p, _i, _i, _i64, _p, _i, _p, _i, _i, _i, _i, _i64, _p]),
     "vgan_linear_backward_params_ksplit_ws_bytes": (_i64, [_i, _i, _i]),
     "vgan_linear_backward_params_ksplit": (_i, [_p, _i, _p, _i, _p, _i, _i, _i, _i, _i, _p, _i64, _p]),
+    "vgan_linear_backward_params_ksplit_xrows": (_i, [_p, _i, _p, _i, _p, _i, _i, _i, _i, _i, _p, _i64, _p, _p]),
     "vgan_linear_backward_params_xx_supported": (_i, [_i, _i, _i]),
     "vgan_linear_backward_params_xx": (_i, [_p, _i, _p, _i, _p, _i, _i, _i, _i, _p, _p]),
     "vgan_linear_forward_path": (_i, [_p, _i, _i, _i64, _p, _i, _p, _p, _i, _i, _i, _i]),
diff --git a/v-gan_amd/ops.py b/v-gan_amd/ops.py
--- a/v-gan_amd/ops.py
+++ b/v-gan_amd/ops.py
@@ -109,6 +109,23 @@
         _lib.check(self.lib.vgan_linear_backward_params_ksplit(_ptr(dy), dy.stride(0), _ptr(x), x.stride(0), _ptr(dW), dW.stride(0), n, kin, out,
                                                                int(parts), _ptr(ws), 0 if ws is None else ws.numel() * ws.element_size(),
                                                                self._stream()), "vgan_linear_backward_params_ksplit")
+
+    def x_rows_job(self, data, rows, center, xrow, Zh, Zl, sq, row_cursor=None, row_batches=1, row_stride=0):
+        _mat(data, "data"), _vec(rows, "rows", torch.int32), _vec(xrow, "xrow", torch.int32)
+        n = xrow.numel()
+        assert Zh.stride(0) == Zl.stride(0) and Zh.shape[0] >= n and sq.numel() >= n and sq.is_contiguous()
+        return _lib.XRowsJob(_ptr(data), _ptr(center), _ptr(rows), _ptr(row_cursor), _ptr(xrow), _ptr(Zh), _ptr(Zl), _ptr(sq),
+                             data.stride(0), Zh.stride(0), n, data.shape[1], int(row_batches), int(row_stride))
+
+    def linear_backward_params_ksplit_xrows(self, dy, x, dW, parts, ws, xjob):
+        _mat(dy, "dy"), _mat(x, "x"), _mat(dW, "dW")
+        n, out = dy.shape
+        kin = x.shape[1]
+        assert x.shape[0] == n and dW.shape == (out, kin)
+        _lib.check(self.lib.vgan_linear_backward_params_ksplit_xrows(_ptr(dy), dy.stride(0), _ptr(x), x.stride(0), _ptr(dW), dW.stride(0), n,
+                                                                     kin, out, int(parts), _ptr(ws), ws.numel() * ws.element_size(),
+                                                                     ctypes.byref(xjob), self._stream()),
+                   "vgan_linear_backward_params_ksplit_xrows")
 
     def linear_backward_params_xx_supported(self, n, kin, out):
         return bool(self.lib.vgan_linear_backward_params_xx_supported(int(n), int(kin), int(out)))
diff --git a/v-gan_amd/step_plan.py b/v-gan_amd/step_plan.py
--- a/v-gan_amd/step_plan.py
+++ b/v-gan_amd/step_plan.py
@@ -34,6 +34,7 @@
     return best
 
 
+DEFAULT_X_RIDER = False
 CHAIN_KPARTS_AUTO = 4
 
 
@@ -120,6 +121,7 @@
     m4_kparts: int
     tn_kparts: int
     lean: bool
+    x_rider: bool
     col_chunks: int
     nl: int
     lo: int
@@ -130,7 +132,7 @@
 
 
 def plan_step(ops, *, n, d, data_stride, latent, widths, world, rank, force_exchange, generator_mode, mmd_precision,
-              overlap_exchange, fuse_update, front, chain_assoc, knobs, host_tables=None):
+              overlap_exchange, fuse_update, front, chain_assoc, knobs, host_tables=None, x_rider=None):
     assert widths[0] == latent and len(widths) == 5
     exchange = world > 1 or bool(force_exchange)
     if n % world != 0:
@@ -244,6 +246,8 @@
             tn_kparts = chain_kparts(knobs.chain_kparts, tn_tiles, e[4])
     lean = (getattr(ops, "bf3_rebuild", False) and fused_prepare and small_tiles and rm_backward and world == 1 and
             plain_schedule and bwd_edge == 64 and not knobs.z_fp32)
+    can_ride = lean and m4_kparts > 1 and not (xx_in_m4 and not xx_late_in_backward) and not chain_in_mask and not xx_ride
+    x_rider = can_ride and (DEFAULT_X_RIDER if x_rider is None else bool(x_rider))
     col_chunks = (world * ops.colmax_chunks(nl)) if front_sharded else ops.colmax_chunks(n)
     return StepPlan(mode=mode, exchange=exchange, front_sharded=front_sharded, fuse_update=fuse_update, chain_flops=chain_flops,
                     fwd_split=fwd_split, bwd_split=bwd_split, precision=precision, bf3=bf3, bwd_tile=bwd_tile, splits=splits,
@@ -251,5 +255,5 @@
                     two_stage_logits=two_stage_logits, gram_tile=gram_tile, gram_tail=gram_tail, rs_from_gram=rs_from_gram,
                     overlap=overlap, side_stream=side_stream, x_ahead=x_ahead, xx_ride=xx_ride, xx_in_m4=xx_in_m4,
                     xx_late_in_backward=xx_late_in_backward, tile_split=tile_split, n_tiles=n_tiles, n_main=n_main,
-                    cal_shares_tiles=cal_shares_tiles, m4_kparts=m4_kparts, tn_kparts=tn_kparts, lean=lean, col_chunks=col_chunks,
+                    cal_shares_tiles=cal_shares_tiles, m4_kparts=m4_kparts, tn_kparts=tn_kparts, lean=lean, x_rider=x_rider, col_chunks=col_chunks,
                     nl=nl, lo=lo, dp=dp, e=e, kp=(d + 63) // 64 * 64, kn=(2 * n + 63) // 64 * 64)
diff --git a/v-gan_amd/trainer.py b/v-gan_amd/trainer.py
--- a/v-gan_amd/trainer.py
+++ b/v-gan_amd/trainer.py
@@ -52,7 +52,7 @@
     def __init__(self, ops, generator, data, batch_size, batches_per_epoch, lr=0.007, weight_decay=0.04, penalty_weight=10.0,
                  seed=777, noise="device", rank=0, world=1, group=None, use_graph=True, loss_accum_scale=None,
                  generator_mode=None, force_exchange=False, mmd_precision=None, center_operand=True, overlap_exchange=None,
-                 fuse_update=None, front=None, chain_assoc=None):
+                 fuse_update=None, front=None, chain_assoc=None, x_rider=None):
         self.ops = ops
         self.dev = data.device
         self.rank, self.world, self.group = rank, world, group
@@ -67,6 +67,10 @@
         self.graph = None
         self.graph_multi = None
         self.graph_blocks = {}
+        self._x_staged = False
+        self.graph_staged = None
+        self.self_gathers = 0
+        self.last_self_gather = -1
         self.steps_per_graph = max(1, min(16, int(batches_per_epoch)))
         self.steps_done = 0
         self._xx_primed = False
@@ -79,7 +83,7 @@
         self.plan = plan_step(ops, n=n, d=d, data_stride=data.stride(0), latent=L, widths=self.widths, world=world, rank=rank,
                               force_exchange=force_exchange, generator_mode=generator_mode, mmd_precision=mmd_precision,
                               overlap_exchange=overlap_exchange, fuse_update=fuse_update, front=front, chain_assoc=chain_assoc,
-                              knobs=Knobs.from_env(), host_tables=tables)
+                              knobs=Knobs.from_env(), host_tables=tables, x_rider=x_rider)
         vars(self).update(vars(self.plan))
         self._alloc_generator([q for m in lin for q in (m.weight, m.bias)])
         self._alloc_mmd(center_operand)
@@ -193,7 +197,7 @@
         self.gram_tail_ws = ops.gram_tail_workspace(self.dev) if self.gram_tail else None
         self.rs_part = torch.zeros((2 * n + 127) // 128, nl, **f32) if self.rs_from_gram else None
         self._side = torch.cuda.Stream(device=self.dev) if (self.side_stream and self.data.is_cuda) else None
-        self._xx = self._xx_m4 = self._rebuild = None
+        self._xx = self._xx_m4 = self._rebuild = self._xrows = None
         if self.xx_ride:
             i16 = dict(dtype=torch.int16, device=self.dev)
             rows_total = self.data.shape[0]
@@ -228,6 +232,7 @@
         self._after_new_epoch_table()
 
     def _after_new_epoch_table(self):
+        self._x_staged = False
         if self.overlap and self.has_bw:
             self._prefetch_xx()
 
@@ -279,6 +284,7 @@
 
     def set_noise(self, z):
         self.za[:, :self.L].copy_(z.to(dtype=torch.float32), non_blocking=True)
+        self._x_staged = False
 
     def epoch_loss(self):
         v = float(self._sum_over_ranks(self.loss_accum).item())
@@ -365,7 +371,7 @@
     def _slabs(self, splits, like):
         return self.chain_ws[:splits * like.numel()].view(splits, like.shape[0], like.shape[1])
 
-    def _generator_backward_update(self, dist):
+    def _generator_backward_update(self, dist, rider=False):
         ops = self.ops
         adadelta = dict(lr=self.lr, rho=ADADELTA_RHO, eps=ADADELTA_EPS, weight_decay=self.wd, grad_scale=1.0)
         if self.mode == "layered":
@@ -389,6 +395,11 @@
         e, d = self.e, self.d
         if self.xx_in_m4 and not self.xx_late_in_backward:
             ops.linear_backward_params_xx(self.dlogits_pad, self.z_own, self.M[4][:self.dp], self._late_xx_job())
+        elif rider and self.x_rider:
+            if self._xrows is None:
+                self._xrows = ops.x_rows_job(self.data, self.perm, self.center, self.xrow, self.Zh, self.Zl, self.sqn,
+                                             row_cursor=self.step_counter, row_batches=self.nb, row_stride=self.n)
+            ops.linear_backward_params_ksplit_xrows(self.dlogits_pad, self.z_own, self.M[4][:self.dp], self.m4_kparts, self.m4_ws, self._xrows)
         elif self.m4_kparts > 1:
             ops.linear_backward_params_ksplit(self.dlogits_pad, self.z_own, self.M[4][:self.dp], self.m4_kparts, self.m4_ws)
         else:
@@ -430,7 +441,7 @@
         import torch.distributed as dist
         return dist
 
-    def _forward(self):
+    def _forward(self, gather_x=True):
         ops, n, nl, lo = self.ops, self.n, self.nl, self.lo
         if self.noise_mode == "device" and (self.mode == "layered" or self.steps_done == 0):
             ops.noise_normal(self.za, self.seed, self.step_counter, 0, cols=self.L, ones_col=self.L)
@@ -449,7 +460,10 @@
                     ntx = self.tiles.shape[0] - self.n_main
                     self._xx = ops.xx_job(self.Dh, self.Dl, self.dsq, self.tiles[self.n_main:], self.bw, self.partial[self.n_main:self.n_main + ntx])
                 xx = self._xx
-            if self.lean:
+            if self.lean and not gather_x:
+                ops.mask_project_forward_bf3(logits, self.data, self.xrow, self.S, self.Z, self.sqn, self.Zh, self.Zl, None, None,
+                                             center=self.center, write_x=False, write_z=False)
+            elif self.lean:
                 ops.mask_project_forward_bf3(logits, self.data, self.perm, self.S, self.Z, self.sqn, self.Zh, self.Zl, None, None,
                                              center=self.center, xx=xx, write_z=not self.has_bw, xrow=self.xrow, **rowsel)
             else:
@@ -472,7 +486,7 @@
         ops.mmd_set_bandwidth(self.stats, self.n, self.bw)
         self.has_bw = True
 
-    def _loss_backward_update(self):
+    def _loss_backward_update(self, rider=True):
         ops, n, nl, lo, d = self.ops, self.n, self.nl, self.lo, self.d
         dist = self._collect() if self.exchange else None
         gstride = nl * self.dp
@@ -514,7 +528,7 @@
                              mul_shift=self.center)
         self._fork_prefetch()
         ops.mask_backward(self.gU, self.S_own, self.colkey, self.pen, lo, self.dlogits, self.bsplits, gstride)
-        self._generator_backward_update(dist)
+        self._generator_backward_update(dist, rider=rider)
         self._join_prefetch()
 
     def _forward_sharded(self):
@@ -632,13 +646,25 @@
                                           self.partial[self.n_main:self.n_main + ntx])
         return self._xx_m4
 
-    def _step_body(self):
+    def _step_body(self, gather_x=True):
         if self.front_sharded:
             self._forward_sharded()
             self._loss_backward_update_sharded()
         else:
-            self._forward()
+            self._forward(gather_x=gather_x)
             self._loss_backward_update()
+
+    def _gathers_x(self):
+        return not (self.x_rider and self._x_staged)
+
+    def _ran(self, steps, gathered):
+        if gathered:
+            self.self_gathers += 1
+            self.last_self_gather = self.steps_done
+        if not self.x_rider:
+            self.self_gathers += steps - (1 if gathered else 0)
+            self.last_self_gather = self.steps_done + steps - 1
+        self.steps_done += steps
 
     def step(self):
         if not self.has_bw:
@@ -652,19 +678,27 @@
             if self.front_sharded:
                 self._loss_backward_update_sharded(all_rows_here=True)
             else:
-                self._loss_backward_update()
-        elif self.use_graph and self.steps_done > 0:
+                self._loss_backward_update(rider=False)
+            self._x_staged = False
+            self._ran(1, True)
+            return
+        gather_x = self._gathers_x()
+        if self.use_graph and self.steps_done > 0:
             if self.graph is None:
                 self._capture()
-            if self.graph is not None:
-                self.graph.replay()
-            else:
-                self._step_body()
+            if self.graph is not None and not gather_x and self.graph_staged is None:
+                self.graph_staged = self._capture_graph(1, gather_first=False) or False
+            g = self.graph if gather_x else self.graph_staged
+            if g:
+                g.replay()
+            else:
+                self._step_body(gather_x)
         else:
             if self.overlap and not self._xx_primed:
                 self._prefetch_xx()
-            self._step_body()
-        self.steps_done += 1
+            self._step_body(gather_x)
+        self._x_staged = self.x_rider
+        self._ran(1, gather_x)
 
     def run_steps(self, count):
         count = int(count)
@@ -675,30 +709,33 @@
             blk = min(count, m)
             if (blk > 1 and self.use_graph and self.has_bw and self.steps_done > 0 and self.noise_mode == "device" and
                     self.graph is not None):
-                g = self._block_graph(blk)
+                gather_x = self._gathers_x()
+                g = self._block_graph(blk, gather_x)
                 if g is not None:
                     g.replay()
-                    self.steps_done += blk
+                    self._x_staged = self.x_rider
+                    self._ran(blk, gather_x)
                     count -= blk
                     continue
             self.step()
             count -= 1
 
-    def _block_graph(self, steps):
-        g = self.graph_blocks.get(steps)
-        if g is None and len(self.graph_blocks) < 4:
-            g = self.graph_blocks[steps] = self._capture_graph(steps) or False
-        if steps == self.steps_per_graph:
+    def _block_graph(self, steps, gather_first=True):
+        key = steps if gather_first else (steps, False)
+        g = self.graph_blocks.get(key)
+        if g is None and len({k if isinstance(k, int) else k[0] for k in self.graph_blocks} | {steps}) <= 4:
+            g = self.graph_blocks[key] = self._capture_graph(steps, gather_first) or False
+        if steps == self.steps_per_graph and gather_first:
             self.graph_multi = g or None
         return g or None
 
-    def _capture_graph(self, steps):
+    def _capture_graph(self, steps, gather_first=True):
         torch.cuda.synchronize()
         g = torch.cuda.CUDAGraph()
         try:
             with no_gc_while_capturing(), torch.cuda.graph(g):
-                for _ in range(steps):
-                    self._step_body()
+                for k in range(steps):
+                    self._step_body(gather_first if k == 0 else not self.x_rider)
         except Exception as e:
             import warnings
             warnings.warn(f"vgan_amd: HIP-graph capture of {steps} training step(s) failed ({type(e).__name__}: {e}); running eager launches")
```

Result: slower. 9427 steps/s (-2.6%).
